# richardbaihe/a3t

Hardware: AMD Instinct MI355X
Metric: mel-frames/sec (train) (higher is better)
Workload: dtype bf16; 1 GPU; VCTK A3T masked-mel train step: 6+6 Conformer blocks d=384 H=2 ff=1536(k3), B=32/GPU, T_mel=1000, T_phn=120, postnet 5x256x5, fwd+bwd+clip+Adam, dropout 0.2/0.2/0.2 + postnet 0.5 (recipe); global_batch=32, parallelism=dp1, params=100799808

## Files before the change

a3t_amd/_lib.py:

```python
import ctypes
import os
from ctypes import POINTER, c_char_p, c_float, c_int, c_int32, c_int64, c_void_p

import torch

HERE = os.path.dirname(os.path.abspath(__file__))
LIB_PATH = os.environ.get("A3T_LIB_PATH") or os.path.join(HERE, "lib", "liba3t_hip.so")

F32, BF16 = 0, 1
BF16X3 = 2
ACT_NONE, ACT_RELU, ACT_TANH, ACT_SWISH = 0, 1, 2, 3
ACC_STORE, ACC_ADD, ACC_ATOMIC, ACC_SOLE = 0, 1, 2, 3


class GemmDesc(ctypes.Structure):
    _fields_ = [
        ("A", c_void_p), ("B", c_void_p), ("C", c_void_p), ("bias", c_void_p), ("R", c_void_p), ("S", c_void_p),
        ("M", c_int32), ("N", c_int32), ("K", c_int32),
        ("a_rs", c_int64), ("a_cs", c_int64),
        ("b_rs", c_int64), ("b_cs", c_int64), ("b_ts", c_int64),
        ("c_rs", c_int64),
        ("batch", c_int32), ("batch_inner", c_int32),
        ("a_bs0", c_int64), ("a_bs1", c_int64), ("b_bs0", c_int64), ("b_bs1", c_int64),
        ("c_bs0", c_int64), ("c_bs1", c_int64),
        ("taps", c_int32), ("pad", c_int32), ("dil", c_int32), ("Tseq", c_int32), ("kshift", c_int32),
        ("alpha", c_float),
        ("act", c_int32), ("accumulate", c_int32), ("splitk", c_int32),
        ("a_dtype", c_int32), ("b_dtype", c_int32), ("c_dtype", c_int32), ("compute", c_int32),
        ("s_dtype", c_int32), ("colsum_slots", c_int32),
        ("colsum", c_void_p), ("colsum_bs1", c_int64), ("colsum_scale", c_float), ("drop_key", ctypes.c_uint32),
        ("drop_p", c_float), ("colsum_ss", c_int32),
        ("keep_out", c_void_p), ("keep_in", c_void_p),
        ("a_signmask", c_int32), ("keep_layout", c_int32),
        ("A2", c_void_p), ("B2", c_void_p), ("b2_cs", c_int64), ("b2_bs0", c_int64), ("b2_bs1", c_int64), ("colsum2", c_void_p),
        ("a2_rs", c_int64), ("a_unaligned", c_int32),
    ]


_P = c_void_p
_SIGS = {
    "a3t_gemm": [POINTER(GemmDesc), _P],
    "a3t_gemm_plan": [POINTER(GemmDesc), c_char_p, c_int],
    "a3t_layernorm_fwd": [_P, _P, _P, _P, c_int, _P, _P, c_int, c_int, c_float, _P],
    "a3t_layernorm_bwd": [_P, c_int, _P, _P, _P, _P, _P, _P, _P, _P, _P, _P, c_float, c_int, c_int, c_float,
                          ctypes.c_uint32, _P],
    "a3t_col_reduce": [_P, c_int, _P, _P, _P, _P, c_int, c_int, c_int64, c_int, _P],
    "a3t_f64_to_f32_add": [_P, _P, c_int, c_float, _P],
    "a3t_bn_act_fwd": [_P, _P, _P, _P, _P, _P, _P, _P, _P, c_int, c_int, c_int, c_float, c_float, c_int, c_int, _P],
    "a3t_bn_act_bwd_a": [_P, c_int, _P, _P, _P, _P, _P, _P, c_int, c_int, c_int, _P],
    "a3t_bn_act_bwd_b": [_P, c_int, _P, _P, _P, _P, _P, _P, _P, _P, _P, c_int, c_int, c_int, c_int, _P],
    "a3t_glu_dwconv_fwd": [_P, c_int, _P, _P, _P, c_int, _P, c_int, c_int, c_int, c_int, _P],
    "a3t_glu_dwconv_bwd": [_P, _P, c_int, _P, c_int, _P, _P, c_int, _P, _P, _P, c_int, c_int, c_int, c_int, _P],
    "a3t_add_pos_bias": [_P, _P, _P, _P, _P, c_int, c_int, c_int, _P],
    "a3t_add_pos_bias_bwd": [_P, _P, _P, c_int, c_int, c_int, _P],
    "a3t_relpos_softmax_fwd": [_P, _P, c_int, _P, _P, c_int, c_int, c_int, c_int, c_int64, c_int64, c_int64, c_float, _P,
                               c_float, ctypes.c_uint32, _P],
    "a3t_relpos_softmax_bwd": [_P, c_int, _P, c_int, _P, _P, c_int, c_int, c_int, c_int, c_int64, c_int64, c_int64, c_float, _P,
                               c_float, c_int64, c_int64, ctypes.c_uint32, _P, _P],
    "a3t_attn_fwd_train": [_P, _P, _P, _P, _P, _P, _P, _P, _P, _P, _P, c_int, c_int, c_int, c_int, c_int64, c_int64, c_int64,
                           c_int64, c_float, c_float, ctypes.c_uint32, _P, _P, _P],
    "a3t_attn_scale_rows": [_P, _P, _P, c_int, c_int, c_int, c_int, _P],
    "a3t_attn_bwd_ds": [_P, _P, _P, _P, _P, _P, _P, c_int, c_int, c_int, c_int, c_int64, c_int64, c_int64, c_int64, c_float,
                        c_float, ctypes.c_uint32, c_int, c_int64, _P],
    "a3t_attn_fwd": [_P, _P, _P, _P, _P, _P, _P, _P, c_int, c_int, c_int, c_int, c_int64, c_int64, c_int64, c_int64,
                     c_float, c_float, ctypes.c_uint32, _P, _P, _P],
    "a3t_pwg_block": [_P, _P, _P, _P, _P, _P, _P, _P, c_int, c_int, c_int, _P],
    "a3t_mask_fill": [_P, _P, _P, _P, c_int, c_int, c_int, _P],
    "a3t_embed_finish_fwd": [_P, _P, _P, _P, _P, _P, _P, c_int, c_int, c_int, c_int, c_float, c_float, ctypes.c_uint32,
                             _P, _P],
    "a3t_embed_finish_bwd": [_P, _P, _P, _P, _P, _P, _P, _P, c_int, c_int, c_int, c_int, c_int, c_int, c_float, c_float,
                             ctypes.c_uint32, _P],
    "a3t_scale": [_P, _P, c_int64, c_float, _P],
    "a3t_axpy": [_P, _P, c_int64, c_float, _P],
    "a3t_attn_bias_fold": [_P, c_int32, c_int32, _P, _P, _P, _P],
    "a3t_scale_dev": [_P, _P, c_int64, _P, _P],
    "a3t_slice_rows": [_P, _P, c_int, c_int, c_int, c_int, c_int, c_int, _P],
    "a3t_concat_rows": [_P, _P, _P, c_int, c_int, c_int, c_int, _P],
    "a3t_concat_rows_ragged": [_P, _P, _P, _P, _P, c_int, c_int, c_int, c_int, c_int64, c_int64, _P],
    "a3t_split_rows": [_P, _P, _P, c_int, c_int, c_int, c_int, _P],
    "a3t_cast_bf16": [_P, _P, c_int64, _P],
    "a3t_cast_bf16_conv_t": [_P, _P, _P, _P, c_int, c_int, c_int, c_int, _P],
    "a3t_split_bf16": [_P, _P, _P, c_int64, _P],
    "a3t_reflect_pad": [_P, _P, c_int, c_int, c_int, c_int, _P],
    "a3t_reflect_pad_ragged": [_P, _P, _P, c_int, c_int, c_int, c_int, _P],
    "a3t_stft_amp": [_P, _P, c_int64, c_int, c_int, _P],
    "a3t_logmel_finish": [_P, _P, c_int, c_int, c_int, _P],
    "a3t_mlm_loss": [_P, _P, _P, _P, _P, _P, _P, _P, c_int, c_int, c_int, c_float, _P],
    "a3t_mlm_loss_scratch_floats": [c_int],
    "a3t_sumsq": [_P, c_int64, _P, _P],
    "a3t_clip_adam": [_P, _P, _P, _P, _P, _P, c_int64, c_float, c_float, c_float, c_float, c_int, c_float, c_float,
                      _P],
    "a3t_clip_adam_noam": [_P, _P, _P, _P, _P, _P, c_int64, _P, c_float, c_float, c_float, c_float, c_float, c_float,
                           c_float, c_float, _P],
    "a3t_sgd_step": [_P, _P, c_int64, c_float, c_float, _P],
    "a3t_pwg_gate": [_P, _P, _P, c_int64, c_int, _P],
    "a3t_pwg_res_skip": [_P, _P, _P, c_int64, c_int, c_int, _P],
    "a3t_pwg_upsample": [_P, _P, _P, c_int64, c_int64, c_int, c_int, _P],
    "a3t_replicate_pad": [_P, _P, c_int64, c_int64, c_int, c_int, _P],
    "a3t_bias_act": [_P, _P, c_int64, c_int, c_int, c_float, _P],
    "a3t_replicate_pad_ragged": [_P, _P, _P, c_int64, c_int64, c_int, c_int, _P],
    "a3t_pwg_upsample_ragged": [_P, _P, _P, _P, c_int, c_int64, c_int64, c_int, c_int, _P],
    "a3t_zero_tail": [_P, _P, c_int, c_int64, c_int64, c_int, _P],
    "a3t_layernorm_fwd_ragged": [_P, _P, _P, _P, _P, _P, _P, c_int, c_int, c_int, c_float, _P],
    "a3t_glu_dwconv_fwd_ragged": [_P, _P, _P, _P, _P, _P, c_int, c_int, c_int, c_int, _P],
    "a3t_relpos_softmax_fwd_ragged": [_P, _P, c_int, _P, _P, c_int, c_int, c_int, c_int, c_int64, c_int64, c_int64, c_float,
                                      _P],
    "a3t_splice_spans": [_P, _P, _P, _P, _P, _P, c_int, c_int, c_int, c_int, _P],
    "a3t_splice_spans_multi": [_P, _P, _P, _P, _P, _P, _P, c_int, c_int, c_int, c_int, c_int, _P],
    "a3t_gather_windows": [_P, _P, _P, c_int, c_int, c_int, c_int, _P],
    "a3t_pwg_block_ragged": [_P, _P, _P, _P, _P, _P, _P, _P, _P, c_int, c_int, c_int, c_int, _P],
    "a3t_pwg_block_f16": [_P, _P, _P, _P, _P, _P, _P, _P, _P, c_int, c_int, c_int, c_int, _P],
    "a3t_cast_f16_sat": [_P, _P, c_int64, _P],
    "a3t_hfg_conv": [_P, _P, _P, _P, _P, _P, c_float, c_int, c_float, _P, c_int, c_int, c_int, c_int, c_int, c_int, _P],
    "a3t_hfg_conv_f16": [_P, _P, _P, _P, _P, _P, c_float, c_int, c_float, _P, c_int, c_int, c_int, c_int, c_int, c_int, _P],
    "a3t_hfg_out": [_P, _P, _P, _P, c_float, _P, c_int, c_int, c_int, c_int, c_int, _P],
    "a3t_leaky_relu": [_P, _P, c_int64, c_float, _P],
    "a3t_mgan_stack": [_P, _P, _P, _P, c_float, _P, c_int, c_int, c_int, c_int, c_int, c_int, _P],
    "a3t_mgan_out": [_P, _P, _P, _P, c_float, c_int, _P, c_int, c_int, c_int, c_int, c_int, c_int, c_int, _P],
    "a3t_pqmf_synthesis": [_P, _P, _P, _P, c_int, c_int, c_int, c_int, c_int, _P],
    "a3t_reflect_pad_rows": [_P, _P, c_int64, c_int64, c_int, c_int, _P],
    "a3t_reflect_pad_rows_ragged": [_P, _P, _P, c_int, c_int64, c_int64, c_int, c_int, _P],
    "a3t_smg_conv": [_P, _P, _P, _P, _P, _P, _P, c_int, c_int, _P, c_int, c_int, c_int, c_int, c_int, c_int, c_int, c_int, c_int,
                     c_int, _P],
    "a3t_smg_stats": [_P, _P, _P, c_float, _P, c_int, c_int, c_int, c_int, _P],
    "a3t_duration_head": [_P, _P, _P, _P, _P, _P, _P, c_int, c_int, c_float, c_float, _P],
    "a3t_l2_normalize": [_P, _P, c_int, c_int, c_float, _P],
    "a3t_gst_conv_bn_relu": [_P, _P, _P, _P, _P, _P, c_int, c_int, c_int, c_int, c_int, c_int, c_int, _P],
    "a3t_gst_gru_stl": [_P, _P, _P, _P, _P, _P, _P, _P, _P, _P, _P, _P, c_int, c_int, c_int, c_int, c_int, c_int, _P],
    "a3t_gst_add_style": [_P, _P, _P, c_int, c_int, c_int, c_int, _P],
    "a3t_fs2_variance_embed": [_P, _P, _P, _P, _P, _P, _P, _P, c_int, c_int, c_int, c_int, c_int, _P],
    "a3t_length_offsets": [_P, _P, c_float, _P, _P, _P, c_int, c_int, _P],
    "a3t_length_expand": [_P, _P, _P, _P, _P, c_int, c_int, c_int, c_int, c_float, _P],
    "a3t_fs2_finish": [_P, _P, _P, _P, _P, _P, _P, c_int, c_int, c_int, _P],
    "a3t_fs2_mvn": [_P, _P, _P, _P, c_int64, c_int, _P],
    "a3t_dropout": [_P, c_int, _P, c_int, c_int64, c_float, ctypes.c_uint32, c_float, _P],
    "a3t_collate_paint": [_P, _P, _P, _P, _P, _P, _P, _P, _P, _P, _P, _P, _P, c_int, c_int, c_int, c_int, c_int, c_int, _P],
    "a3t_segment_colsum": [_P, _P, c_int, c_int, c_int, _P],
    "a3t_gemm_8p_mode": [c_int],
    "a3t_gemm_8p_supported": [c_int, c_int, c_int, c_int, c_int],
    "a3t_gemm_pn_mode": [c_int],
    "a3t_gemm_tt_mode": [c_int],
    "a3t_gemm_tn3_mode": [c_int],
    "a3t_gemm_tn3_group": [_P, c_int, _P],
    "a3t_attn_split_mode": [c_int],
    "a3t_release_workspaces": [],
    "a3t_gemm_pn_supported": [c_int, c_int, c_int, c_int, c_int],
    "a3t_gemm_tt_supported": [c_int, c_int, c_int, c_int],
    "a3t_dropout_bwd_cast": [_P, _P, c_int, _P, c_float, c_int, c_int, c_float, ctypes.c_uint32, _P],
}
EXPORTS = sorted(list(_SIGS) + ["a3t_version", "a3t_gemm_last_kernel", "a3t_gemm_keep_bytes"])

_lib = None


class A3TLibraryError(RuntimeError):
    pass


def load():
    global _lib
    if _lib is not None:
        return _lib
    if not os.path.exists(LIB_PATH):
        raise A3TLibraryError(
            f"{LIB_PATH} is missing: build it with `python -m a3t_amd.build` (hipcc --offload-arch=gfx950). "
            "a3t_amd has no CPU fallback.")
    lib = ctypes.CDLL(LIB_PATH)
    for name, args in _SIGS.items():
        fn = getattr(lib, name)
        fn.argtypes = args
        fn.restype = c_int
    lib.a3t_version.restype = c_char_p
    lib.a3t_version.argtypes = []
    lib.a3t_gemm_last_kernel.restype = c_char_p
    lib.a3t_gemm_last_kernel.argtypes = []
    lib.a3t_gemm_keep_bytes.restype = c_int64
    lib.a3t_gemm_keep_bytes.argtypes = [c_int, c_int]
    _lib = lib
    return lib


def check(rc, what=""):
    if rc != 0:
        raise A3TLibraryError(f"liba3t_hip call failed ({what}): rc={rc}")
```

a3t_amd/conformer.py:

```python
import math
import os
import zlib
from dataclasses import dataclass

import torch

from . import ops
from ._lib import ACC_ADD, ACC_ATOMIC, ACC_STORE, ACT_RELU, ACT_SWISH, BF16, BF16X3, F32
from .config import A3TConfig
from .params import ParamStore
from .schedule import StepSchedule


def legacy_pe_table(c: A3TConfig) -> torch.Tensor:
    d = c.adim
    position = torch.arange(c.max_len - 1, -1, -1.0, dtype=torch.float32).unsqueeze(1)
    div = torch.exp(torch.arange(0, d, 2, dtype=torch.float32) * -(math.log(10000.0) / d))
    pe = torch.zeros(c.max_len, d)
    pe[:, 0::2] = torch.sin(position * div)
    pe[:, 1::2] = torch.cos(position * div)
    return pe


def score_chunks(lengths, heads, max_score_elems):
    order = sorted(range(len(lengths)), key=lambda i: (lengths[i], i))
    out, cur = [], []
    for i in order:
        if cur and (len(cur) + 1) * heads * lengths[i] ** 2 > max_score_elems:
            out.append(cur)
            cur = []
        cur.append(i)
    if cur:
        out.append(cur)
    return out


@dataclass
class EngineOptions:
    side_stream: bool = True
    side2: bool = True
    side_depth: int = 48
    wgrad_group: bool = True
    post_f32_first: bool = True
    attn_bwd_ds: bool = True
    attn_signed: bool = True
    attn_dq_dual: bool = True
    attn_dbd_view: bool = True
    attn_dk_main: bool = True
    fused_attn: str = "auto"
    fused_attn_train: int = 1
    ffn_8p: bool = True
    ffn_keep4: bool = True
    lin_dgrad_t: bool = True
    fuse_ln_dropout: bool = True

    @classmethod
    def from_env(cls, environ=os.environ):
        fa, ft = environ.get("A3T_FUSED_ATTN", "auto"), environ.get("A3T_FUSED_ATTN_TRAIN", "1")
        if fa not in ("auto", "fwd", "0"):
            raise ValueError(f"A3T_FUSED_ATTN={fa!r}: expected auto, fwd or 0 (the flash backward behind '1' left the library in "
                             "round 5, tools/experiments/attn_flash_backward.patch)")
        on = {f: environ.get("A3T_" + f.upper(), "1") != "0" for f in
              ("side_stream", "side2", "wgrad_group", "post_f32_first", "attn_bwd_ds", "attn_signed", "attn_dq_dual",
               "attn_dbd_view", "attn_dk_main", "ffn_8p", "ffn_keep4", "lin_dgrad_t")}
        return cls(side_depth=max(2, int(environ.get("A3T_SIDE_DEPTH", "48"))), fused_attn=fa,
                   fused_attn_train=0 if ft == "0" else 2 if ft == "2" else 1, **on)


COMPUTE_MODES = {"f32": F32, "bf16": BF16, "bf16x3": BF16X3}


class ConformerStack(StepSchedule):
    def __init__(self, cfg: A3TConfig, store: ParamStore, compute: str = "f32", training: bool = True,
                 dropout: bool = False, options: EngineOptions = None):
        self.opt = opt = options if options is not None else EngineOptions.from_env()
        super().__init__(store.device, opt.side_stream, opt.side2, opt.side_depth)
        self.c = cfg
        self.dropping = bool(dropout and training)
        self.step_seed = 0
        self.store = store
        if compute not in COMPUTE_MODES:
            raise ValueError(f"compute={compute!r}: expected one of {', '.join(map(repr, COMPUTE_MODES))}")
        self.compute = compute
        self.bf16 = (compute == "bf16")
        self.adt = torch.bfloat16 if self.bf16 else torch.float32
        self.cmp = COMPUTE_MODES[compute]
        self.training = training
        self.pe = legacy_pe_table(cfg).to(self.dev)
        self.sv = {}
        self.scratch64 = torch.zeros(4 * max(cfg.ff, 3 * cfg.adim, cfg.postnet_chans, 64), dtype=torch.float64,
                                     device=self.dev)
        self.bn_momentum = 0.1
        self._wg_group = 4 if (self.bf16 and self.side is not None and self._depth >= 8 and opt.wgrad_group) else 1
        self._wg_pending, self._wg_slots = [], set()
        self._gm_ready = None
        self.colsum_slots = 16
        self.fused_attn_fwd_only = self.bf16 and opt.fused_attn == "fwd"
        self.fused_attn_auto = self.bf16 and opt.fused_attn == "auto"
        self.fused_attn_train = self.bf16 and opt.fused_attn == "auto" and opt.fused_attn_train != 0
        self.fused_attn_train_min = 1 if opt.fused_attn_train == 2 else 64
        self._fused_now = self._fused_train_now = False
        self.attn_path, self.block_dims = {}, {}
        self._need_grad = training
        self._mode_tag = None
        if self.bf16:
            for n, v in (("adim", cfg.adim), ("ff", cfg.ff), ("idim", cfg.idim), ("odim", cfg.odim),
                         ("dk", cfg.dk), ("postnet_chans", cfg.postnet_chans or 8)):
                if v % 8:
                    raise ValueError(f"compute='bf16' needs {n} % 8 == 0 (16-byte DMA granules), got {v}")
            self.flat16 = torch.zeros(store.total, dtype=torch.bfloat16, device=self.dev)
            self.p16 = {k: self.flat16[o:o + math.prod(s)].view(s) for k, (o, s) in store.offsets.items()}
        self._ffn_plans = {}
        self._lin_plans = {}
        self._wt = {}
        self._P_ahead, self._pos_ev = {}, None
        self._cast_ev = self._wt_ev = None
        dec = [o for k, (o, _) in store.offsets.items() if k.startswith("dec.")]
        self._cast_split = min(dec) if dec else 0

    def _drop(self, p, tag):
        if not self.dropping or p <= 0.0:
            return None
        h = (zlib.crc32(tag.encode()) ^ ((self.step_seed * 0x9E3779B1) & 0xFFFFFFFF)) & 0xFFFFFFFF
        h = ((h ^ (h >> 16)) * 0x85EBCA6B) & 0xFFFFFFFF
        h = ((h ^ (h >> 13)) * 0xC2B2AE35) & 0xFFFFFFFF
        return (float(p), (h ^ (h >> 16)) & 0xFFFFFFFF)

    def _gm(self, g, tag, p, bias_grad, bias_scale):
        dr = self._drop(p, tag)
        if dr is None:
            return (self._g16(g) if self.bf16 else g)
        gm = self.ws.get(self._t("tmp.gm"), tuple(g.shape), self.adt)
        if self._gm_ready == tag:
            self._gm_ready = None
            return gm
        ops.dropout_bwd_cast(g, gm, dr[0], dr[1], colsum=bias_grad, colsum_scale=bias_scale)
        return gm

    def W(self, name):
        return self.p16[name] if self.bf16 else self.store.p[name]

    def refresh_weights(self):
        self._cast_ev = self._wt_ev = None
        if not self.bf16:
            return
        split = self._cast_split if self.side is not None else 0
        flat, flat16 = self.store.flat, self.flat16
        wt = list(self._wt.values()) if self._need_grad else []

        def transposed():
            for src_off, dst_off, _, tflat, shp in wt:
                ops.cast_bf16_conv_t(flat, tflat, src_off, dst_off, *shp)
        if split <= 0:
            ops.cast_bf16(flat, flat16)
            transposed()
            return
        ops.cast_bf16(flat[:split], flat16[:split])
        self._cast_ev = self._side(lambda: ops.cast_bf16(flat[split:], flat16[split:]), want_event="cast")
        if wt:
            self._wt_ev = self._side(transposed, want_event="wt")

    def _wait_cast(self, which):
        ev = getattr(self, which, None)
        if ev is not None:
            ev.wait_on(torch.cuda.current_stream())
            setattr(self, which, None)

    def _setup_wt(self, suf, shape):
        stored = (tuple(shape), (shape[0], shape[2])) if shape[1] == 1 else (tuple(shape),)
        names = [k for k in self.store.offsets if k.endswith("." + suf) and tuple(self.store.offsets[k][1]) in stored]
        if not names:
            return
        n = math.prod(shape)
        flat = torch.zeros(n * len(names), dtype=torch.bfloat16, device=self.dev)
        src = torch.tensor([self.store.offsets[k][0] for k in names], dtype=torch.int64, device=self.dev)
        dst = torch.arange(len(names), dtype=torch.int64, device=self.dev) * n
        views = {k: flat[i * n:(i + 1) * n].view(shape[2], shape[1], shape[0]) for i, k in enumerate(names)}
        self._wt[suf] = (src, dst, views, flat, tuple(shape))
        ops.cast_bf16_conv_t(self.store.flat, flat, src, dst, *shape)

    def _ffn_plan(self, M):
        key = (M, self._need_grad, self._mode_tag, self.opt.ffn_8p, self.opt.ffn_keep4)
        if key not in self._ffn_plans:
            c = self.c
            keep = d1 = d2 = keep4 = False
            if self._need_grad and self.bf16 and self.dev.type == "cuda" and self.opt.ffn_8p:
                k = c.ff_kernel
                drop = ops.G8_DROP if (self.dropping and c.dropout_rate > 0) else 0
                keep = ops.gemm_8p_supported(M, c.ff, k * c.adim, k, ops.G8_BIAS_ACT | drop | ops.G8_KEEP_OUT) and \
                    ops.gemm_8p_supported(M, c.ff, k * c.adim, k, ops.G8_KEEP_IN | ops.G8_COLSUM)
                d1 = ops.gemm_8p_supported(M, c.adim, k * c.ff, k, 0) or ops.gemm_pn_supported(M, c.adim, k * c.ff, k, 0)
                d2 = (not keep) and \
                    ops.gemm_pn_supported(M, c.ff, k * c.adim, k, ops.G8_SMASK | ops.G8_COLSUM)
                keep4 = (not keep) and self.opt.ffn_keep4 and c.ff % 8 == 0 and \
                    ops.gemm_pn_supported(M, c.ff, k * c.adim, k, ops.G8_KEEP_IN | ops.G8_COLSUM)
                d2 = d2 or keep4
                if (keep or d2) and "w2" not in self._wt:
                    self._setup_wt("w2", (c.adim, k, c.ff))
                if d1 and "w1" not in self._wt:
                    self._setup_wt("w1", (c.ff, k, c.adim))
                keep, d1, d2 = keep and "w2" in self._wt, d1 and "w1" in self._wt, d2 and "w2" in self._wt
                keep4 = keep4 and d2
            self._ffn_plans[key] = (keep, d1, d2, keep4)
        return self._ffn_plans[key]

    def _lin_dgrad(self, dy, name, dx):
        suf = name.rsplit(".", 1)[1]
        M = dy.shape[0]
        key = (suf, M, dx.dtype, self._mode_tag, self.opt.lin_dgrad_t)
        if key not in self._lin_plans:
            use = False
            if self.bf16 and self.dev.type == "cuda" and self.opt.lin_dgrad_t:
                n_out, n_in = self.store.offsets[name][1]
                use = ops.gemm_pn_supported(M, n_in, n_out, 1, ops.G8_F32_OR_RES if dx.dtype == torch.float32 else 0)
                if use and suf not in self._wt:
                    self._setup_wt(suf, (n_out, 1, n_in))
                use = use and suf in self._wt and name in self._wt[suf][2]
            self._lin_plans[key] = use
        if self._lin_plans[key]:
            wt = self._wt[suf][2][name]
            ops.linear_fwd(dy, wt.view(wt.shape[0], wt.shape[2]), dx, compute=self.cmp)
        else:
            ops.linear_bwd_data(dy, self.W(name), dx, compute=self.cmp)

    def _act(self, name, shape):
        return self.ws.get(name, shape, self.adt)

    def _ln_fwd(self, tag, x, pre, eps=1e-12, out_dtype=None, lens=None, T=0):
        p = self.store.p
        M, D = x.shape
        y = self.ws.get(tag + ".y", (M, D), out_dtype or self.adt)
        mean = self.ws.get(tag + ".mean", (M,))
        rstd = self.ws.get(tag + ".rstd", (M,))
        if lens is not None:
            ops.layernorm_fwd_ragged(x, p[pre + ".g"], p[pre + ".b"], y, mean, rstd, lens, M // T, T, eps)
        else:
            ops.layernorm_fwd(x, p[pre + ".g"], p[pre + ".b"], y, mean, rstd, eps)
        self.sv[tag] = (x, y, mean, rstd)
        return y

    def _ln_bwd(self, tag, dy, pre, dres, dx, dx16=None, nb=None, nxt=None):
        p, g = self.store.p, self.store.g
        x, _, mean, rstd = self.sv[tag]
        dropping = self.dropping and self.c.dropout_rate > 0
        if dropping and self.bf16 and self.opt.fuse_ln_dropout and nb is not None and nxt is not None and x.shape[1] % 128 == 0:
            dr = self._drop(self.c.dropout_rate, nxt)
            nx = (self._par + 1) % self._depth
            gm = self.ws.get(f"tmp.gm.{nx}", tuple(dx.shape), self.adt)
            ev = self._side_ev[nx]
            if ev is not None:
                ev.wait_on(torch.cuda.current_stream())
                self._side_ev[nx] = None
            ops.layernorm_bwd(dy, x, p[pre + ".g"], mean, rstd, dres, dx, g[pre + ".g"], g[pre + ".b"], dx16=gm,
                              dxsum=nb[0], dxsum_scale=nb[1], drop=dr)
            self._gm_ready = nxt
            return
        if dropping and nxt is not None:
            nb = None
        fuse = self.bf16 and nb is not None
        ops.layernorm_bwd(dy, x, p[pre + ".g"], mean, rstd, dres, dx, g[pre + ".g"], g[pre + ".b"], dx16=dx16,
                          dxsum=nb[0] if fuse else None, dxsum_scale=nb[1] if fuse else 1.0)
        if nb is not None and not fuse:
            self._bias_grad(dx, nb[0], nb[1])

    def _bias_grad(self, dy, gb, scale=1.0):
        ops.bias_grad(dy, gb, self.scratch64, scale)

    def _g16(self, g):
        return self.ws.get("grad.x16", tuple(g.shape), torch.bfloat16) if self.bf16 else None

    def _lin_wgrad(self, dy, x, dW):
        if self._wg_group > 1:
            self._wg_pending.append((dy, x, dW, 1.0))
            self._wg_slots.add(self._par)
            if len(self._wg_pending) >= self._wg_group:
                self._wg_flush()
            return
        self._side(lambda: ops.linear_bwd_weight(dy, x, dW, compute=self.cmp))

    def _wg_flush(self):
        items, self._wg_pending = self._wg_pending, []
        slots, self._wg_slots = self._wg_slots, set()
        if items:
            cmp = self.cmp
            self._side(lambda: ops.linear_bwd_weight_group(items, compute=cmp))
            if self.side is not None:
                for sl in slots:
                    ev = self._owned_event(("slot", sl))
                    ev.record(self.side)
                    self._side_ev[sl] = ev

    def _pre_ln(self, ga, g, g16):
        if ga is g or ga is g16:
            self._wg_flush()
        if self.side is not None and (ga is g or ga is g16):
            torch.cuda.current_stream().wait_stream(self.side)

    def _ffn_fwd(self, tag, pre, x, T, lens=None):
        p, c = self.store.p, self.c
        M = x.shape[0]
        pad = (c.ff_kernel - 1) // 2
        if lens is not None and pad == 0:
            lens = None
        y = self._ln_fwd(tag + ".ln", x, pre + ".ln", lens=lens, T=T)
        h = self._act(tag + ".h", (M, c.ff))
        keep, lay = None, 0
        if self._ffn_plan(M)[0]:
            keep = self.ws.get(tag + ".keep", (ops.gemm_keep_bytes(M, c.ff),), torch.uint8)
        elif self._ffn_plan(M)[3]:
            keep, lay = self.ws.get(tag + ".keep4", (M * c.ff // 4,), torch.uint8), 1
        ops.conv_fwd(y, self.W(pre + ".w1"), h, T, pad, bias=p[pre + ".b1"], act=ACT_RELU, compute=self.cmp,
                     drop=self._drop(c.dropout_rate, tag + ".h"), keep_out=keep, keep_layout=lay)
        if lens is not None:
            ops.zero_tail(h, lens, 1, M // T, T)
        xo = self.ws.get(tag + ".xo", (M, c.adim))
        ops.conv_fwd(h, self.W(pre + ".w2"), xo, T, pad, bias=p[pre + ".b2"], R=x, alpha=0.5, compute=self.cmp,
                     drop=self._drop(c.dropout_rate, tag + ".o"))
        self.sv[tag] = (y, h, keep, lay)
        return xo

    def _ffn_bwd(self, tag, pre, g, T, nb=None, nxt=None):
        p, gr, c = self.store.p, self.store.g, self.c
        y, h, keep, lay = self.sv[tag]
        M = g.shape[0]
        pad = (c.ff_kernel - 1) // 2
        self._sub_begin()
        g16 = self._g16(g)
        ga = self._gm(g, tag + ".o", c.dropout_rate, gr[pre + ".b2"], 0.5)
        self._side(lambda: ops.conv_bwd_weight(ga, h, gr[pre + ".w2"], T, pad, alpha=0.5, compute=self.cmp))
        dh = self._act(self._t("tmp.dh"), (M, c.ff))
        hd = self._drop(c.dropout_rate, tag + ".h")
        a_dh = 0.5 / (1.0 - hd[0]) if hd else 0.5
        if keep is not None:
            ops.conv_fwd(ga, self._wt["w2"][2][pre + ".w2"], dh, T, c.ff_kernel - 1 - pad, alpha=a_dh, compute=self.cmp,
                         keep_in=keep, keep_layout=lay, colsum=gr[pre + ".b1"])
        elif self._ffn_plan(M)[2]:
            ops.conv_fwd(ga, self._wt["w2"][2][pre + ".w2"], dh, T, c.ff_kernel - 1 - pad, alpha=a_dh, compute=self.cmp,
                         S=h, colsum=gr[pre + ".b1"])
        else:
            ops.conv_bwd_data(ga, self.W(pre + ".w2"), dh, T, pad, S=h, alpha=a_dh,
                              compute=self.cmp, colsum=gr[pre + ".b1"] if self.bf16 else None)
        self._side(lambda: ops.conv_bwd_weight(dh, y, gr[pre + ".w1"], T, pad, compute=self.cmp))
        dy = self._act("tmp.dy", (M, c.adim))
        if self._ffn_plan(M)[1]:
            ops.conv_fwd(dh, self._wt["w1"][2][pre + ".w1"], dy, T, c.ff_kernel - 1 - pad, compute=self.cmp)
        else:
            ops.conv_bwd_data(dh, self.W(pre + ".w1"), dy, T, pad, compute=self.cmp)
        if not self.bf16:
            self._bias_grad(dh, gr[pre + ".b1"])
        self._pre_ln(ga, g, g16)
        self._ln_bwd(tag + ".ln", dy, pre + ".ln", g, g, g16, nb, nxt)
        self._sub_end()
        return g

    def _mha_fwd(self, tag, pre, x, pos, keymask, B, T, lens=None, pos_rows=None):
        p, c = self.store.p, self.c
        d, dk = c.adim, c.dk
        M = B * T
        cmp = self.cmp
        y = self._ln_fwd(tag + ".ln", x, pre + ".ln")
        qkv = self._act(tag + ".qkv", (M, 3 * d))
        ops.linear_fwd(y, self.W(pre + ".wqkv"), qkv, bias=p[pre + ".bqkv"], compute=cmp)
        ragged = lens is not None
        fused = (self._fused_now or self._fused_train_now) and ops.attn_fused_supported(dk, T) and not ragged
        pbias = (p[pre + ".u"], p[pre + ".v"])
        qu = qv = None
        if not fused:
            qu = self._act(tag + ".qu", (M, d))
            qv = self._act(tag + ".qv", (M, d))
            ops.add_pos_bias(qkv, pbias[0], pbias[1], qu, qv)
        P = None if ragged else self._P_ahead.get(tag)
        if P is not None:
            ev = self._pos_ev.get(tag[:3]) if self._pos_ev else None
            if ev is not None:
                ev.wait_on(torch.cuda.current_stream())
                self._pos_ev[tag[:3]] = None
        elif pos_rows is not None:
            Pt = self._act(tag + ".Pt", (pos.shape[0], d))
            ops.linear_fwd(pos, self.W(pre + ".wpos"), Pt, compute=cmp)
            P = self._act(tag + ".Prow", (M, d))
            ops.concat_rows_ragged(Pt, Pt, P, pos_rows[0], pos_rows[1], B, pos_rows[2], pos_rows[3], d, 0, 0)
        else:
            P = self._act(tag + ".P", (T, d))
            ops.linear_fwd(pos, self.W(pre + ".wpos"), P, compute=cmp)
        route = "fwd" if (self._fused_now and fused) else "train" if (self._fused_train_now and fused) else "mat"
        self.attn_path[tag[:-4]] = route
        self.block_dims[tag[:-4]] = (B, T)
        for k in (".fused", ".rs", ".signed"):
            self.sv.pop(tag + k, None)
        ctx = self._act(tag + ".ctx", (M, d))
        q = (qu, qv, qkv, P, keymask, ctx)
        if route == "mat":
            kept = self._attn_fwd_mat(tag, q, B, T, lens, pos_rows is not None)
        else:
            kept = (self._attn_fwd_only if route == "fwd" else self._attn_fwd_train)(tag, q, pbias, B, T)
        xo = self.ws.get(tag + ".xo", (M, d))
        ops.linear_fwd(ctx, self.W(pre + ".wo"), xo, bias=p[pre + ".bo"], R=x, compute=cmp,
                       drop=self._drop(c.dropout_rate, tag + ".o"))
        self.sv[tag] = None if kept is None else (y, qkv, qu, qv, P, kept[0], ctx, pos, kept[1])
        return xo

    def _attn_fwd_only(self, tag, q, pbias, B, T):
        c = self.c
        lse = self.ws.get(tag + ".lse", (B, c.heads, T))
        ops.attn_fwd(*q, lse, B, c.heads, T, 1.0 / math.sqrt(c.dk), drop=self._drop(c.attention_dropout_rate, tag + ".att") or (0.0, 0),
                     pos_bias=pbias if q[0] is None else None)
        self.sv[tag + ".fused"] = True

    def _attn_fwd_train(self, tag, q, pbias, B, T):
        c, H = self.c, self.c.heads
        adr = self._drop(c.attention_dropout_rate, tag + ".att")
        probs = self._act(tag + ".probs", (B, H, T, T))
        signed = bool(adr) and self.bf16 and self.opt.attn_bwd_ds and self.opt.attn_signed and T <= 2048
        pdrop = self._act(tag + ".pdrop", (B, H, T, T)) if adr and not signed else None
        lse = self.ws.get(tag + ".lse", (B, H, T))
        rs = self.ws.get(tag + ".rs", (B, H, T))
        ops.attn_fwd_train(*q, lse, probs, pdrop, rs, B, H, T, 1.0 / math.sqrt(c.dk), drop=adr or (0.0, 0),
                           pos_bias=pbias if q[0] is None else None)
        self.sv[tag + ".signed"] = signed
        self.sv[tag + ".rs"] = rs
        return probs, pdrop

    def _attn_fwd_mat(self, tag, q, B, T, lens, pos_per_row):
        c, H, d, dk, cmp = self.c, self.c.heads, self.c.adim, self.c.dk, self.cmp
        qu, qv, qkv, P, keymask, ctx = q
        sdt = torch.bfloat16 if self.bf16 else torch.float32
        ac = self.ws.get("tmp.ac", (B, H, T, T), sdt)
        bd = self.ws.get("tmp.bd", (B, H, T, T), sdt)
        kk = qkv.view(-1)[d:]
        vv = qkv.view(-1)[2 * d:]
        ops.gemm(qu, kk, ac, T, T, dk, d, 1, 3 * d, 1, T, batch=B * H, batch_inner=H, a_bs=(T * d, dk),
                 b_bs=(T * 3 * d, dk), c_bs=(H * T * T, T * T), compute=cmp)
        ops.gemm(qv, P, bd, T, T, dk, d, 1, d, 1, T, batch=B * H, batch_inner=H, a_bs=(T * d, dk),
                 b_bs=(T * d if pos_per_row else 0, dk), c_bs=(H * T * T, T * T), compute=cmp)
        probs = self._act(tag + ".probs", (B, H, T, T))
        adr = self._drop(c.attention_dropout_rate, tag + ".att")
        pdrop = self._act(tag + ".pdrop", (B, H, T, T)) if adr else None
        if lens is not None:
            ops.relpos_softmax_fwd_ragged(ac, bd, lens, probs, B, H, T, 1.0 / math.sqrt(dk))
        else:
            ops.relpos_softmax_fwd(ac, bd, keymask, probs, B, H, T, 1.0 / math.sqrt(dk), probs_drop=pdrop,
                                   drop=adr or (0.0, 0))
        ops.gemm(pdrop if adr else probs, vv, ctx, T, dk, T, T, 1, 1, 3 * d, d, batch=B * H, batch_inner=H,
                 a_bs=(H * T * T, T * T), b_bs=(T * 3 * d, dk), c_bs=(T * d, dk), compute=cmp)
        return None if lens is not None else (probs, pdrop)

    def _mha_bwd(self, tag, pre, g, B, T, nb=None, nxt=None):
        p, gr, c = self.store.p, self.store.g, self.c
        d, H, dk = c.adim, c.heads, c.dk
        M = B * T
        cmp = self.cmp
        y, qkv, qu, qv, P, probs, ctx, pos, pdrop = self.sv[tag]
        scale = 1.0 / math.sqrt(dk)
        self._sub_begin()
        g16 = self._g16(g)
        ga = self._gm(g, tag + ".o", c.dropout_rate, gr[pre + ".bo"], 1.0)
        self._lin_wgrad(ga, ctx, gr[pre + ".wo"])
        dctx = self._act("tmp.dctx", (M, d))
        self._lin_dgrad(ga, pre + ".wo", dctx)
        kk = qkv.view(-1)[d:]
        vv = qkv.view(-1)[2 * d:]
        dqkv = self._act(self._t("tmp.dqkv"), (M, 3 * d))
        dkk = dqkv.view(-1)[d:]
        dvv = dqkv.view(-1)[2 * d:]
        sdt = torch.bfloat16 if self.bf16 else torch.float32
        rs = self.sv.get(tag + ".rs")
        dctx_v = dctx
        if rs is not None:
            dctx_v = self._act(self._t("tmp.dctxs"), (M, d))
        signed = bool(self.sv.get(tag + ".signed"))
        adr = self._drop(c.attention_dropout_rate, tag + ".att") if (pdrop is not None or signed) else None
        regen = self.bf16 and adr is not None and T % 8 == 0 and T <= 2048
        ds_fused = (rs is not None and self.bf16 and self.opt.attn_bwd_ds and (adr is None or regen) and dk % 32 == 0 and dk <= 192
                    and dk != 160 and T % 8 == 0)
        zb = (H * T * T, T * T)
        assert ds_fused or not signed
        if not ds_fused:
            dpr = self.ws.get("tmp.ac", (B, H, T, T), sdt)
            ops.gemm(dctx, vv, dpr, T, T, dk, d, 1, 3 * d, 1, T, batch=B * H, batch_inner=H, a_bs=(T * d, dk),
                     b_bs=(T * 3 * d, dk), c_bs=zb, compute=cmp)
        fz = self.bf16
        gbq = gr[pre + ".bqkv"]
        S = self.colsum_slots
        sl = self._arena_slot("bwd32", tag + ".bsl", S * 4 * d) if fz else None
        csk = dict(colsum_bs1=dk, colsum_slots=S, colsum_ss=4 * d)
        make_q = qu is None
        if make_q:
            qu = self._act("tmp.qu", (M, d))
            qv = self._act(self._t("tmp.qv"), (M, d))

        def dv_gemm():
            if rs is not None:
                ops.attn_scale_rows(dctx, rs, dctx_v, B, H, T)
            ops.gemm(pdrop if pdrop is not None else probs, dctx_v, dvv, T, dk, T, 1, T, 1, d, 3 * d,
                     batch=B * H, batch_inner=H, a_bs=zb, b_bs=(T * d, dk), c_bs=(T * 3 * d, dk),
                     compute=cmp, colsum=sl[3 * d:] if fz else None, a_signmask=signed,
                     alpha=1.0 / (1.0 - adr[0]) if signed else 1.0, **csk)
            if make_q:
                ops.add_pos_bias(qkv, p[pre + ".u"], p[pre + ".v"], qu, qv)
        qv_ready = self._side(dv_gemm, want_event=make_q, urgent=True)
        zbd = zb
        dual = ds_fused and fz and self.opt.attn_dq_dual and ops.gemm_tt_supported(T, dk, T, B * H)
        dview = ds_fused and fz and self.opt.attn_dbd_view
        if dview:
            bsv = T + T * T
            flat = self.ws.get(self._t("tmp.dsv"), (B * H * bsv,), torch.bfloat16, zero_once=True)
            ds, dbd = flat[T:], flat[1:]
            zbd = (H * bsv, bsv)
        elif self.bf16:
            ds = self.ws.get("tmp.ds16", (B, H, T, T), torch.bfloat16)
            dbd = self.ws.get(self._t("tmp.dbd16"), (B, H, T, T), torch.bfloat16)
        else:
            ds = dpr
            dbd = self.ws.get(self._t("tmp.dbd"), (B, H, T, T), sdt)
        if ds_fused:
            ops.attn_bwd_ds(dctx, ctx, qkv, probs, rs, ds, None if dview else dbd, B, H, T, scale, drop=adr or (0.0, 0),
                            signed_probs=signed, ds_bs=zbd[1] if dview else 0)
        else:
            ops.relpos_softmax_bwd(probs, dpr, ds, dbd, B, H, T, scale, probs_drop=None if regen else pdrop,
                                   drop_p=adr[0] if adr else 0.0, drop_key=adr[1] if regen else 0, rowscale=rs)
        def pos_weight_grad():
            if qv_ready is not None and self.side is not None:
                qv_ready.wait_on(self.side)
            dP = self._arena_slot("bwd32", tag + ".dP", T * d).view(T, d)
            ops.gemm(dbd, qv, dP, T, dk, T, 1, T + 1 if dview else T, 1, d, d, batch=B * H, batch_inner=H, a_bs=zbd, b_bs=(T * d, dk),
                     c_bs=(0, dk), acc=ACC_ATOMIC, compute=cmp, a_view=dview)
            if self.bf16:
                dP16 = self.ws.get("tmp.dP16", (T, d), torch.bfloat16)
                ops.cast_bf16(dP, dP16)
                dP = dP16
            ops.linear_bwd_weight(dP, pos, gr[pre + ".wpos"], compute=cmp)
        self._side(pos_weight_grad)
        dq_acc = fz
        dqu = dqkv if dq_acc else self._act("tmp.dqu", (M, d))
        dqv = dqkv if dq_acc else self._act("tmp.dqv", (M, d))
        ldq, cbq = (3 * d, (T * 3 * d, dk)) if dq_acc else (d, (T * d, dk))
        if dual:
            ops.gemm(ds, kk, dqkv, T, dk, T, T, 1, 1, 3 * d, ldq, batch=B * H, batch_inner=H, a_bs=zbd,
                     b_bs=(T * 3 * d, dk), c_bs=cbq, compute=cmp, colsum=sl,
                     second=(dbd, P, d, (0, dk), sl[d:]) + ((T + 1,) if dview else ()), **csk)
        else:
            ops.gemm(ds, kk, dqu, T, dk, T, T, 1, 1, 3 * d, ldq, batch=B * H, batch_inner=H, a_bs=zbd,
                     b_bs=(T * 3 * d, dk), c_bs=cbq, compute=cmp, colsum=sl if fz else None, **csk)
        dk_fn = lambda: ops.gemm(ds, qu, dkk, T, dk, T, 1, T, 1, d, 3 * d, batch=B * H, batch_inner=H,
                                 a_bs=zbd, b_bs=(T * d, dk), c_bs=(T * 3 * d, dk), compute=cmp,
                                 colsum=sl[2 * d:] if fz else None, **csk)
        if self.opt.attn_dk_main and dual and self.side is not None and make_q and qv_ready is not None:
            qv_ready.wait_on(torch.cuda.current_stream())
            dk_fn()
            dk_done = None
        else:
            dk_done = self._side(dk_fn, want_event=True, urgent=True)
        if not dual:
            ops.gemm(dbd, P, dqv, T, dk, T, T + 1 if dview else T, 1, 1, d, ldq, batch=B * H, batch_inner=H, a_bs=zbd, b_bs=(0, dk),
                     c_bs=cbq, acc=ACC_ADD if dq_acc else ACC_STORE, compute=cmp, colsum=sl[d:] if fz else None, a_view=dview, **csk)
        if not dq_acc:
            ops.add_pos_bias_bwd(dqu, dqv, dqkv)
        if dk_done is not None:
            dk_done.wait_on(torch.cuda.current_stream())
        if fz:
            self._side(
                lambda: ops.attn_bias_fold(sl, S, d, gr[pre + ".u"], gr[pre + ".v"], gbq))
        else:
            self._bias_grad(dqu, gr[pre + ".u"])
            self._bias_grad(dqv, gr[pre + ".v"])
            self._bias_grad(dqkv, gbq)
        self._lin_wgrad(dqkv, y, gr[pre + ".wqkv"])
        dy = self._act("tmp.dy", (M, d))
        self._lin_dgrad(dqkv, pre + ".wqkv", dy)
        self._pre_ln(ga, g, g16)
        self._ln_bwd(tag + ".ln", dy, pre + ".ln", g, g, g16, nb, nxt)
        self._sub_end()
        return g

    def _bn_fwd(self, tag, z, pre, bufpre, act, out):
        p, b = self.store.p, self.store.buf
        M, C = z.shape
        stats = self._arena_slot("fwd64", tag + ".stats", 2 * C)
        if self.training:
            ops.col_reduce(z, stats[:C], stats[C:], mode=1)
        mean = self.ws.get(tag + ".bnmean", (C,))
        rstd = self.ws.get(tag + ".bnrstd", (C,))
        ops.bn_act_fwd(z, stats, p[pre + ".g"], p[pre + ".b"], b[bufpre + ".rm"], b[bufpre + ".rv"], mean, rstd, out,
                       1e-5, self.bn_momentum if self.training else 0.0, self.training, act)
        if self.training:
            self.store.nbt[bufpre] = self.store.nbt.get(bufpre, 0) + 1
        self.sv[tag + ".bn"] = (z, mean, rstd)

    def _bn_bwd(self, tag, dy, pre, act, dz):
        p, gr = self.store.p, self.store.g
        z, mean, rstd = self.sv[tag + ".bn"]
        M, C = z.shape
        sums = self._arena_slot("bwd64", tag + ".bnsums", 2 * C)
        ops.bn_act_bwd(dy, z, mean, rstd, p[pre + ".g"], p[pre + ".b"], sums, dz, gr[pre + ".g"], gr[pre + ".b"],
                       self.training, act, zero=False)

    def _conv_fwd(self, tag, pre, x, T, lens=None):
        p, c = self.store.p, self.c
        M, d = x.shape
        cmp = self.cmp
        y = self._ln_fwd(tag + ".ln", x, pre + ".ln")
        g2 = self._act(tag + ".g", (M, 2 * d))
        ops.linear_fwd(y, self.W(pre + ".pw1"), g2, bias=p[pre + ".pb1"], compute=cmp)
        glu = self._act(tag + ".glu", (M, d))
        z = self.ws.get(tag + ".z", (M, d))
        if lens is not None:
            ops.glu_dwconv_fwd_ragged(g2, p[pre + ".dw"], p[pre + ".db"], glu, z, lens, M // T, T)
        else:
            ops.glu_dwconv_fwd(g2, p[pre + ".dw"], p[pre + ".db"], glu, z, T)
        s = self._act(tag + ".s", (M, d))
        self._bn_fwd(tag, z, pre + ".bn", pre + ".bn", ACT_SWISH, s)
        xo = self.ws.get(tag + ".xo", (M, d))
        ops.linear_fwd(s, self.W(pre + ".pw2"), xo, bias=p[pre + ".pb2"], R=x, compute=cmp,
                       drop=self._drop(c.dropout_rate, tag + ".o"))
        self.sv[tag] = (y, g2, glu, s)
        return xo

    def _conv_bwd(self, tag, pre, g, T, nb=None, nxt=None):
        p, gr, c = self.store.p, self.store.g, self.c
        M, d = g.shape
        cmp = self.cmp
        y, g2, glu, s = self.sv[tag]
        self._sub_begin()
        g16 = self._g16(g)
        ga = self._gm(g, tag + ".o", c.dropout_rate, gr[pre + ".pb2"], 1.0)
        self._lin_wgrad(ga, s, gr[pre + ".pw2"])
        ds = self.ws.get("tmp.ds", (M, d))
        self._lin_dgrad(ga, pre + ".pw2", ds)
        dz = self.ws.get("tmp.dz", (M, d))
        self._bn_bwd(tag, ds, pre + ".bn", ACT_SWISH, dz)
        dg = self._act(self._t("tmp.dg"), (M, 2 * d))
        ops.glu_dwconv_bwd(dz, g2, glu, p[pre + ".dw"], dg, gr[pre + ".dw"], gr[pre + ".db"], T,
                           dgsum=gr[pre + ".pb1"])
        self._lin_wgrad(dg, y, gr[pre + ".pw1"])
        dy = self._act("tmp.dy", (M, d))
        self._lin_dgrad(dg, pre + ".pw1", dy)
        self._pre_ln(ga, g, g16)
        self._ln_bwd(tag + ".ln", dy, pre + ".ln", g, g, g16, nb, nxt)
        self._sub_end()
        return g

    def _check_ragged(self, lens, B):
        if self.bf16 or self.training or self._need_grad:
            raise ValueError("lens: ragged rows need an engine in fp32 compute, eval mode, forward only "
                             f"(compute={self.compute}: 'f32' and 'bf16x3' both count, training={self.training}, "
                             f"need_grad={self._need_grad})")
        if lens.dtype != torch.int32 or lens.numel() != B or lens.device.type != self.dev.type:
            raise ValueError(f"lens must be an int32 tensor of {B} entries on {self.dev}")

    def block_fwd(self, pre, x, pos, keymask, B, T, lens=None, pos_rows=None):
        if lens is not None:
            self._check_ragged(lens, B)
        x = self._ffn_fwd(pre + ".ffm", pre + ".ffm", x, T, lens)
        x = self._mha_fwd(pre + ".mha", pre + ".mha", x, pos, keymask, B, T, lens, pos_rows)
        x = self._conv_fwd(pre + ".cnv", pre + ".cnv", x, T, lens)
        x = self._ffn_fwd(pre + ".ff", pre + ".ff", x, T, lens)
        return self._ln_fwd(pre + ".fin", x, pre + ".fin.ln", out_dtype=torch.float32)

    def block_bwd(self, pre, g, B, T):
        gr = self.store.g
        self._ln_bwd(pre + ".fin", g, pre + ".fin.ln", None, g, self._g16(g), (gr[pre + ".ff.b2"], 0.5), pre + ".ff.o")
        self._ffn_bwd(pre + ".ff", pre + ".ff", g, T, (gr[pre + ".cnv.pb2"], 1.0), pre + ".cnv.o")
        self._conv_bwd(pre + ".cnv", pre + ".cnv", g, T, (gr[pre + ".mha.bo"], 1.0), pre + ".mha.o")
        self._mha_bwd(pre + ".mha", pre + ".mha", g, B, T, (gr[pre + ".ffm.b2"], 0.5), pre + ".ffm.o")
        self._ffn_bwd(pre + ".ffm", pre + ".ffm", g, T, None)
        return g

    def _attn_choice(self, B, T, need_grad):
        nblk = B * self.c.heads * ((T + 127) // 128)
        fused_now = (self.fused_attn_fwd_only and not need_grad) or \
            (self.fused_attn_auto and not need_grad and nblk >= 64)
        fused_train_now = self.fused_attn_train and need_grad and not fused_now and \
            self.fused_attn_train_min <= nblk <= 65536 and T <= 2048
        return fused_now, fused_train_now
```

a3t_amd/csrc/convmod_attn.hip:

```cpp
#include <hip/hip_runtime.h>
#include <stdint.h>
#include "../../include/a3t_hip.h"
#include "dtype_io.h"

#define WAVE 64
__device__ __forceinline__ float sigm(float v) { return 1.f / (1.f + __expf(-v)); }
__device__ __forceinline__ float bf2f_(unsigned int h) { return __uint_as_float(h << 16); }
__device__ __forceinline__ float wsum(float v) {
#pragma unroll
    for (int o = 32; o > 0; o >>= 1) v += __shfl_xor(v, o, WAVE);
    return v;
}
__device__ __forceinline__ float wmax(float v) {
#pragma unroll
    for (int o = 32; o > 0; o >>= 1) v = fmaxf(v, __shfl_xor(v, o, WAVE));
    return v;
}

#define DW_TT 64
#define DW_KMAX 31

template <int KT, bool RAGGED>
__global__ __launch_bounds__(256) void glu_dwconv_fwd_kernel(const void* __restrict__ g, int g_dt,
                                                             const float* __restrict__ wdw,
                                                             const float* __restrict__ bdw, void* __restrict__ glu,
                                                             int glu_dt, float* __restrict__ z, int C, int K, int Tseq,
                                                             int tiles_t, const int32_t* __restrict__ lens) {
    __shared__ float win[DW_TT + DW_KMAX - 1][64];
    const int tx = threadIdx.x & 63, ty = threadIdx.x >> 6;
    const int c = blockIdx.x * 64 + tx;
    const int b = blockIdx.y / tiles_t, t0 = (blockIdx.y % tiles_t) * DW_TT;
    const int pad = (K - 1) / 2;
    const int64_t mbase = (int64_t)b * Tseq;
    int n = Tseq;
    if constexpr (RAGGED) {
        g_dt = glu_dt = A3T_F32;
        n = ragged_len(lens, b, Tseq);
        if (t0 >= n) {
            if (c < C)
                for (int r = ty; r < DW_TT && t0 + r < Tseq; r += 4) {
                    ((float*)glu)[(mbase + t0 + r) * (int64_t)C + c] = 0.f;
                    z[(mbase + t0 + r) * (int64_t)C + c] = 0.f;
                }
            return;
        }
    }
    const int rows = DW_TT + K - 1;
    for (int rb = ty; rb < rows; rb += 32) {
        float ga[8], gb[8];
#pragma unroll
        for (int u = 0; u < 8; ++u) {
            const int r = rb + 4 * u, t = t0 - pad + r;
            const bool ok = (c < C) && (r < rows) && (t >= 0) && (t < n);
            const int64_t gi = ok ? (mbase + t) * (int64_t)(2 * C) + c : 0;
            ga[u] = ldx(g, g_dt, gi);
            gb[u] = ldx(g, g_dt, gi + (ok ? C : 0));
        }
#pragma unroll
        for (int u = 0; u < 8; ++u) {
            const int r = rb + 4 * u, t = t0 - pad + r;
            const bool ok = (c < C) && (r < rows) && (t >= 0) && (t < n);
            const float v = ok ? ga[u] * sigm(gb[u]) : 0.f;
            const bool st = RAGGED ? (c < C) && (t < Tseq) : ok;
            if (st && r >= pad && r < pad + DW_TT) stx(glu, glu_dt, (mbase + t) * (int64_t)C + c, v);
            if (r < rows) win[r][tx] = v;
        }
    }
    __syncthreads();
    if (c >= C) return;
    float w[KT];
#pragma unroll
    for (int k = 0; k < KT; ++k) w[k] = (k < K) ? wdw[(int64_t)c * K + k] : 0.f;
    const float bias = bdw[c];
    if (K == KT) {
        for (int r0 = ty * 4; r0 < DW_TT; r0 += 16) {
            float v[KT + 3];
#pragma unroll
            for (int j = 0; j < KT + 3; ++j) v[j] = win[r0 + j][tx];
#pragma unroll
            for (int tt = 0; tt < 4; ++tt) {
                float acc = bias;
#pragma unroll
                for (int k = 0; k < KT; ++k) acc += w[k] * v[tt + k];
                int t = t0 + r0 + tt;
                if (t < Tseq) z[(mbase + t) * (int64_t)C + c] = (!RAGGED || t < n) ? acc : 0.f;
            }
        }
        return;
    }
    for (int r = ty; r < DW_TT; r += 4) {
        int t = t0 + r;
        if (t >= Tseq) break;
        float acc = bias;
#pragma unroll
        for (int k = 0; k < KT; ++k)
            if (k < K) acc += w[k] * win[r + k][tx];
        z[(mbase + t) * (int64_t)C + c] = (!RAGGED || t < n) ? acc : 0.f;
    }
}

int a3t_glu_dwconv_fwd_vec(const void* g, const float* wdw, const float* bdw, void* glu, float* z, int M, int C, int K,
                           int Tseq, hipStream_t stream);
int a3t_glu_dwconv_bwd_vec(const float* dz, const void* g, const void* glu, const float* wdw, void* dg, float* dwdw,
                           float* dbdw, float* dg_colsum, int M, int C, int K, int Tseq, hipStream_t stream);
static inline bool dw_al16(const void* p) { return ((uintptr_t)p & 15) == 0; }

template <bool RAGGED>
static int glu_dwconv_fwd_launch(const void* g, int g_dtype, const float* wdw, const float* bdw, void* glu, int glu_dtype,
                                 float* z, int B, int C, int K, int Tseq, const int32_t* lens, hipStream_t stream) {
    const int tiles_t = (Tseq + DW_TT - 1) / DW_TT;
    dim3 grid((C + 63) / 64, B * tiles_t);
#define CALL(KT)                                                                                                         \
    hipLaunchKernelGGL((glu_dwconv_fwd_kernel<KT, RAGGED>), grid, dim3(256), 0, stream, g, g_dtype, wdw, bdw, glu, glu_dtype, \
                       z, C, K, Tseq, tiles_t, lens)
    if (K <= 7) CALL(7);
    else if (K <= 15) CALL(15);
    else CALL(DW_KMAX);
#undef CALL
    return (int)hipGetLastError();
}

extern "C" int a3t_glu_dwconv_fwd(const void* g, int g_dtype, const float* wdw, const float* bdw, void* glu,
                                  int glu_dtype, float* z, int M, int C, int K, int Tseq, void* stream) {
    if (K > DW_KMAX || K <= 0 || (K & 1) == 0 || Tseq <= 0 || M <= 0 || C <= 0 || M % Tseq) return A3T_EINVAL;
    if ((int64_t)(M / Tseq) * ((Tseq + DW_TT - 1) / DW_TT) > 65535) return A3T_EINVAL;
    if (g_dtype == A3T_BF16 && glu_dtype == A3T_BF16 && C % 64 == 0 && dw_al16(g) && dw_al16(glu) && dw_al16(z))
        return a3t_glu_dwconv_fwd_vec(g, wdw, bdw, glu, z, M, C, K, Tseq, (hipStream_t)stream);
    return glu_dwconv_fwd_launch<false>(g, g_dtype, wdw, bdw, glu, glu_dtype, z, M / Tseq, C, K, Tseq, nullptr,
                                        (hipStream_t)stream);
}

extern "C" int a3t_glu_dwconv_fwd_ragged(const float* g, const float* wdw, const float* bdw, float* glu, float* z,
                                         const int32_t* lens, int B, int Tseq, int C, int K, void* stream) {
    if (K > DW_KMAX || K <= 0 || (K & 1) == 0 || Tseq <= 0 || B <= 0 || C <= 0 || !lens) return A3T_EINVAL;
    if ((int64_t)B * ((Tseq + DW_TT - 1) / DW_TT) > 65535) return A3T_EINVAL;
    return glu_dwconv_fwd_launch<true>(g, A3T_F32, wdw, bdw, glu, A3T_F32, z, B, C, K, Tseq, lens, (hipStream_t)stream);
}

template <int KT>
__global__ __launch_bounds__(256, 3) void glu_dwconv_bwd_kernel(const float* __restrict__ dz, const void* __restrict__ g,
                                                             int g_dt, const void* __restrict__ glu, int glu_dt,
                                                             const float* __restrict__ wdw, void* __restrict__ dg,
                                                             int dg_dt, float* dwdw, float* dbdw, float* dgsum, int C,
                                                             int K, int Tseq, int tiles_t, int tiles_per_block,
                                                             int chunks) {
    __shared__ float wdz[DW_TT + DW_KMAX - 1][64];
    __shared__ float wgl[DW_TT + DW_KMAX - 1][64];
    __shared__ float red[4][64];
    const int tx = threadIdx.x & 63, ty = threadIdx.x >> 6;
    const int c = blockIdx.x * 64 + tx;
    const int b = blockIdx.y / chunks, tile0 = (blockIdx.y % chunks) * tiles_per_block;
    const int pad = (K - 1) / 2;
    const int64_t mbase = (int64_t)b * Tseq;
    const int rows = DW_TT + K - 1;
    float w[KT], dw[KT];
#pragma unroll
    for (int k = 0; k < KT; ++k) {
        w[k] = (k < K && c < C) ? wdw[(int64_t)c * K + k] : 0.f;
        dw[k] = 0.f;
    }
    float db = 0.f, sga = 0.f, sgb = 0.f;
    for (int tile = tile0; tile < min(tiles_t, tile0 + tiles_per_block); ++tile) {
        const int t0 = tile * DW_TT;
        float gan[4], gbn[4];
        auto prefetch_g = [&](int i) {
#pragma unroll
            for (int tt = 0; tt < 4; ++tt) {
                const int t = t0 + ty * 4 + 16 * i + tt;
                gan[tt] = gbn[tt] = 0.f;
                if (c < C && t < Tseq) {
                    const int64_t gi = (mbase + t) * (int64_t)(2 * C);
                    gan[tt] = ldx(g, g_dt, gi + c);
                    gbn[tt] = ldx(g, g_dt, gi + C + c);
                }
            }
        };
        if (K == KT) prefetch_g(0);
        __syncthreads();
        for (int rb = ty; rb < rows; rb += 32) {
            float a[8], q[8];
#pragma unroll
            for (int u = 0; u < 8; ++u) {
                const int r = rb + 4 * u, t = t0 - pad + r;
                const bool ok = (c < C) && (r < rows) && (t >= 0) && (t < Tseq);
                const int64_t idx = ok ? (mbase + t) * (int64_t)C + c : 0;
                a[u] = dz[idx];
                q[u] = ldx(glu, glu_dt, idx);
                a[u] = ok ? a[u] : 0.f;
                q[u] = ok ? q[u] : 0.f;
            }
#pragma unroll
            for (int u = 0; u < 8; ++u) {
                const int r = rb + 4 * u;
                if (r < rows) wdz[r][tx] = a[u], wgl[r][tx] = q[u];
            }
        }
        __syncthreads();
        if (c < C && K == KT) {
#pragma unroll 1
            for (int i = 0; i < 4; ++i) {
                const int r0 = ty * 4 + 16 * i;
                float ga[4], gb[4];
#pragma unroll
                for (int tt = 0; tt < 4; ++tt) ga[tt] = gan[tt], gb[tt] = gbn[tt];
                if (i < 3) prefetch_g(i + 1);
                float acc[4], dzt[4];
                {
                    float u[KT + 3];
#pragma unroll
                    for (int j = 0; j < KT + 3; ++j) u[j] = wdz[r0 + j][tx];
#pragma unroll
                    for (int tt = 0; tt < 4; ++tt) {
                        float a = 0.f;
#pragma unroll
                        for (int k = 0; k < KT; ++k) a += w[k] * u[tt + KT - 1 - k];
                        acc[tt] = a;
                        dzt[tt] = u[tt + (KT - 1) / 2];
                    }
                }
                __builtin_amdgcn_sched_barrier(0);
                {
                    float q[KT + 3];
#pragma unroll
                    for (int j = 0; j < KT + 3; ++j) q[j] = wgl[r0 + j][tx];
#pragma unroll
                    for (int tt = 0; tt < 4; ++tt) {
#pragma unroll
                        for (int k = 0; k < KT; ++k) dw[k] += dzt[tt] * q[tt + k];
                        db += dzt[tt];
                    }
                }
#pragma unroll
                for (int tt = 0; tt < 4; ++tt) {
                    const int t = t0 + r0 + tt;
                    if (t < Tseq) {
                        const int64_t gi = (mbase + t) * (int64_t)(2 * C);
                        const float sb = sigm(gb[tt]);
                        const float da = acc[tt] * sb, dbb = acc[tt] * ga[tt] * sb * (1.f - sb);
                        stx(dg, dg_dt, gi + c, da);
                        stx(dg, dg_dt, gi + C + c, dbb);
                        sga += da, sgb += dbb;
                    }
                }
            }
        } else if (c < C) {
            for (int r = ty; r < DW_TT; r += 4) {
                int t = t0 + r;
                if (t >= Tseq) break;
                float acc = 0.f;
#pragma unroll
                for (int k = 0; k < KT; ++k)
                    if (k < K) acc += w[k] * wdz[r + 2 * pad - k][tx];
                const int64_t gi = (mbase + t) * (int64_t)(2 * C);
                float ga = ldx(g, g_dt, gi + c), sb = sigm(ldx(g, g_dt, gi + C + c));
                const float da = acc * sb, dbb = acc * ga * sb * (1.f - sb);
                stx(dg, dg_dt, gi + c, da);
                stx(dg, dg_dt, gi + C + c, dbb);
                sga += da, sgb += dbb;
                float dzt = wdz[r + pad][tx];
                db += dzt;
#pragma unroll
                for (int k = 0; k < KT; ++k)
                    if (k < K) dw[k] += dzt * wgl[r + k][tx];
            }
        }
    }
#pragma unroll
    for (int k = 0; k < KT; ++k) {
        if (k >= K) break;
        __syncthreads();
        red[ty][tx] = dw[k];
        __syncthreads();
        if (ty == 0 && c < C) atomicAdd(&dwdw[(int64_t)c * K + k], red[0][tx] + red[1][tx] + red[2][tx] + red[3][tx]);
    }
    __syncthreads();
    red[ty][tx] = db;
    __syncthreads();
    if (ty == 0 && c < C) atomicAdd(&dbdw[c], red[0][tx] + red[1][tx] + red[2][tx] + red[3][tx]);
    if (dgsum) {
        __syncthreads();
        red[ty][tx] = sga;
        __syncthreads();
        if (ty == 0 && c < C) atomicAdd(&dgsum[c], red[0][tx] + red[1][tx] + red[2][tx] + red[3][tx]);
        __syncthreads();
        red[ty][tx] = sgb;
        __syncthreads();
        if (ty == 0 && c < C) atomicAdd(&dgsum[C + c], red[0][tx] + red[1][tx] + red[2][tx] + red[3][tx]);
    }
}

extern "C" int a3t_glu_dwconv_bwd(const float* dz, const void* g, int g_dtype, const void* glu, int glu_dtype,
                                  const float* wdw, void* dg, int dg_dtype, float* dwdw, float* dbdw, float* dg_colsum,
                                  int M, int C, int K, int Tseq, void* stream) {
    if (K > DW_KMAX || K <= 0 || (K & 1) == 0 || Tseq <= 0 || M <= 0 || C <= 0 || M % Tseq) return A3T_EINVAL;
    if (g_dtype == A3T_BF16 && glu_dtype == A3T_BF16 && dg_dtype == A3T_BF16 && C % 64 == 0 && dw_al16(g) &&
        dw_al16(glu) && dw_al16(dg) && dw_al16(dz))
        return a3t_glu_dwconv_bwd_vec(dz, g, glu, wdw, dg, dwdw, dbdw, dg_colsum, M, C, K, Tseq, (hipStream_t)stream);
    int B = M / Tseq, tiles_t = (Tseq + DW_TT - 1) / DW_TT;
    int cb = (C + 63) / 64;
    int chunks = 1;
    while (cb * B * chunks < 1024 && chunks < tiles_t) ++chunks;
    int tpb = (tiles_t + chunks - 1) / chunks;
    chunks = (tiles_t + tpb - 1) / tpb;
    if ((int64_t)B * chunks > 65535) return A3T_EINVAL;
    dim3 grid(cb, B * chunks);
#define DWB(KT)                                                                                                       \
    hipLaunchKernelGGL(glu_dwconv_bwd_kernel<KT>, grid, dim3(256), 0, (hipStream_t)stream, dz, g, g_dtype, glu, glu_dtype, \
                       wdw, dg, dg_dtype, dwdw, dbdw, dg_colsum, C, K, Tseq, tiles_t, tpb, chunks)
    if (K <= 7)
        DWB(7);
    else if (K <= 15)
        DWB(15);
    else
        DWB(DW_KMAX);
#undef DWB
    return (int)hipGetLastError();
}

__global__ void add_pos_bias_kernel(const void* __restrict__ qkv, const float* __restrict__ bu,
                                    const float* __restrict__ bv, void* __restrict__ qu, void* __restrict__ qv,
                                    int dt, int64_t n, int d) {
    for (int64_t i = (int64_t)blockIdx.x * blockDim.x + threadIdx.x; i < n; i += (int64_t)gridDim.x * blockDim.x) {
        int64_t m = i / d;
        int c = (int)(i - m * d);
        float q = ldx(qkv, dt, m * 3 * d + c);
        stx(qu, dt, i, q + bu[c]);
        stx(qv, dt, i, q + bv[c]);
    }
}
__device__ __forceinline__ void apb_unpack8(const uint4& u, float* f) {
    f[0] = bf2f_(u.x & 0xffff), f[1] = bf2f_(u.x >> 16), f[2] = bf2f_(u.y & 0xffff), f[3] = bf2f_(u.y >> 16);
    f[4] = bf2f_(u.z & 0xffff), f[5] = bf2f_(u.z >> 16), f[6] = bf2f_(u.w & 0xffff), f[7] = bf2f_(u.w >> 16);
}
__device__ __forceinline__ uint4 apb_pack8(const float* f) {
    uint4 u;
    u.x = io_pack2(f[0], f[1]), u.y = io_pack2(f[2], f[3]);
    u.z = io_pack2(f[4], f[5]), u.w = io_pack2(f[6], f[7]);
    return u;
}
__global__ void add_pos_bias_bf16_kernel(const unsigned short* __restrict__ qkv, const float* __restrict__ bu,
                                         const float* __restrict__ bv, unsigned short* __restrict__ qu,
                                         unsigned short* __restrict__ qv, int64_t n8, int d8) {
    for (int64_t i = (int64_t)blockIdx.x * blockDim.x + threadIdx.x; i < n8; i += (int64_t)gridDim.x * blockDim.x) {
        const int64_t m = i / d8;
        const int c = (int)(i - m * d8) * 8;
        float q[8], o[8];
        apb_unpack8(*(const uint4*)(qkv + m * 3 * d8 * 8 + c), q);
        const float4 u0 = *(const float4*)(bu + c), u1 = *(const float4*)(bu + c + 4);
        const float4 v0 = *(const float4*)(bv + c), v1 = *(const float4*)(bv + c + 4);
        const float uu[8] = {u0.x, u0.y, u0.z, u0.w, u1.x, u1.y, u1.z, u1.w};
        const float vv[8] = {v0.x, v0.y, v0.z, v0.w, v1.x, v1.y, v1.z, v1.w};
#pragma unroll
        for (int e = 0; e < 8; ++e) o[e] = q[e] + uu[e];
        *(uint4*)(qu + i * 8) = apb_pack8(o);
#pragma unroll
        for (int e = 0; e < 8; ++e) o[e] = q[e] + vv[e];
        *(uint4*)(qv + i * 8) = apb_pack8(o);
    }
}
static inline bool apb_al16(const void* p) { return ((uintptr_t)p & 15) == 0; }
extern "C" int a3t_add_pos_bias(const void* qkv, const float* bias_u, const float* bias_v, void* qu, void* qv,
                                int dtype, int M, int d, void* stream) {
    int64_t n = (int64_t)M * d;
    if (dtype == A3T_BF16 && d % 8 == 0 && apb_al16(qkv) && apb_al16(qu) && apb_al16(qv) && apb_al16(bias_u) &&
        apb_al16(bias_v)) {
        int64_t n8 = n / 8;
        int blocks = (int)((n8 + 255) / 256);
        if (blocks > 4096) blocks = 4096;
        hipLaunchKernelGGL(add_pos_bias_bf16_kernel, dim3(blocks), dim3(256), 0, (hipStream_t)stream,
                           (const unsigned short*)qkv, bias_u, bias_v, (unsigned short*)qu, (unsigned short*)qv, n8, d / 8);
        return (int)hipGetLastError();
    }
    int blocks = (int)((n + 255) / 256);
    if (blocks > 4096) blocks = 4096;
    hipLaunchKernelGGL(add_pos_bias_kernel, dim3(blocks), dim3(256), 0, (hipStream_t)stream, qkv, bias_u, bias_v, qu,
                       qv, dtype, n, d);
    return (int)hipGetLastError();
}
__global__ void add_pos_bias_bwd_kernel(const void* __restrict__ dqu, const void* __restrict__ dqv,
                                        void* __restrict__ dqkv, int dt, int64_t n, int d) {
    for (int64_t i = (int64_t)blockIdx.x * blockDim.x + threadIdx.x; i < n; i += (int64_t)gridDim.x * blockDim.x) {
        int64_t m = i / d;
        int c = (int)(i - m * d);
        stx(dqkv, dt, m * 3 * d + c, ldx(dqu, dt, i) + ldx(dqv, dt, i));
    }
}
__global__ void add_pos_bias_bwd_bf16_kernel(const unsigned short* __restrict__ dqu, const unsigned short* __restrict__ dqv,
                                             unsigned short* __restrict__ dqkv, int64_t n8, int d8) {
    for (int64_t i = (int64_t)blockIdx.x * blockDim.x + threadIdx.x; i < n8; i += (int64_t)gridDim.x * blockDim.x) {
        const int64_t m = i / d8;
        const int c = (int)(i - m * d8) * 8;
        float a[8], b[8], o[8];
        apb_unpack8(*(const uint4*)(dqu + i * 8), a);
        apb_unpack8(*(const uint4*)(dqv + i * 8), b);
#pragma unroll
        for (int e = 0; e < 8; ++e) o[e] = a[e] + b[e];
        *(uint4*)(dqkv + m * 3 * d8 * 8 + c) = apb_pack8(o);
    }
}
extern "C" int a3t_add_pos_bias_bwd(const void* dqu, const void* dqv, void* dqkv, int dtype, int M, int d,
                                    void* stream) {
    int64_t n = (int64_t)M * d;
    if (dtype == A3T_BF16 && d % 8 == 0 && apb_al16(dqu) && apb_al16(dqv) && apb_al16(dqkv)) {
        int64_t n8 = n / 8;
        int blocks = (int)((n8 + 255) / 256);
        if (blocks > 4096) blocks = 4096;
        hipLaunchKernelGGL(add_pos_bias_bwd_bf16_kernel, dim3(blocks), dim3(256), 0, (hipStream_t)stream,
                           (const unsigned short*)dqu, (const unsigned short*)dqv, (unsigned short*)dqkv, n8, d / 8);
        return (int)hipGetLastError();
    }
    int blocks = (int)((n + 255) / 256);
    if (blocks > 4096) blocks = 4096;
    hipLaunchKernelGGL(add_pos_bias_bwd_kernel, dim3(blocks), dim3(256), 0, (hipStream_t)stream, dqu, dqv, dqkv, dtype,
                       n, d);
    return (int)hipGetLastError();
}

__device__ __forceinline__ float bd_shift(const void* __restrict__ BDz, int dt, int T, int n, int i, int j) {
    if (j <= i) return ldx(BDz, dt, (int64_t)i * T + (n - 1 - i + j));
    if (j == i + 1) return 0.f;
    return ldx(BDz, dt, (int64_t)(i + 1) * T + (j - i - 2));
}

template <int NV, bool RAGGED>
__global__ __launch_bounds__(256) void relpos_softmax_fwd_kernel(const void* __restrict__ ac,
                                                                 const void* __restrict__ bd, int s_dt,
                                                                 const uint8_t* __restrict__ keymask,
                                                                 void* __restrict__ probs, int p_dt, int H, int T,
                                                                 int64_t ac_bs, int64_t bd_bs, int64_t p_bs,
                                                                 float scale, int64_t nrows, void* __restrict__ pdrop,
                                                                 unsigned int thr, float inv, unsigned int key,
                                                                 const int32_t* __restrict__ lens) {
    const int lane = threadIdx.x & 63;
    const int64_t row = (int64_t)blockIdx.x * 4 + (threadIdx.x >> 6);
    if (row >= nrows) return;
    const int64_t zz = row / T;
    const int i = (int)(row - zz * T);
    const int b = (int)(zz / H);
    int n = T;
    if constexpr (RAGGED) {
        s_dt = p_dt = A3T_F32;
        pdrop = nullptr;
        n = ragged_len(lens, b, T);
        if (i >= n) {
            for (int j = lane; j < T; j += 64) ((float*)probs)[zz * p_bs + (int64_t)i * T + j] = 0.f;
            return;
        }
    }
    const int64_t ao = zz * ac_bs + (int64_t)i * T;
    const void* bz = (s_dt == A3T_BF16) ? (const void*)((const unsigned short*)bd + zz * bd_bs)
                                        : (const void*)((const float*)bd + zz * bd_bs);
    const uint8_t* mk = keymask + (int64_t)b * T;
    auto valid = [&](const int j) -> bool {
        if constexpr (RAGGED) return j < n;
        else return mk[j];
    };
    const int64_t po = zz * p_bs + (int64_t)i * T;
    const float NEG = -3.4028235e38f;
    if (NV > 0) {
        float v[NV > 0 ? NV : 1];
        float mx = NEG;
#pragma unroll
        for (int q = 0; q < NV; ++q) {
            int j = lane + q * 64;
            v[q] = NEG;
            if (j < T && valid(j)) v[q] = (ldx(ac, s_dt, ao + j) + bd_shift(bz, s_dt, T, n, i, j)) * scale;
            mx = fmaxf(mx, v[q]);
        }
        mx = wmax(mx);
        float s = 0.f;
#pragma unroll
        for (int q = 0; q < NV; ++q) {
            v[q] = (v[q] > NEG) ? expf(v[q] - mx) : 0.f;
            s += v[q];
        }
        s = wsum(s);
        const float inv_s = s > 0.f ? 1.f / s : 0.f;
#pragma unroll
        for (int q = 0; q < NV; ++q) {
            int j = lane + q * 64;
            if (j < T) {
                const float pj = v[q] * inv_s;
                stx(probs, p_dt, po + j, pj);
                if (pdrop) stx(pdrop, p_dt, po + j, rng_keep(key, (unsigned int)(po + j), thr) ? pj * inv : 0.f);
            }
        }
        return;
    }
    float mx = NEG;
    int any = 0;
    for (int j = lane; j < T; j += 64)
        if (valid(j)) {
            mx = fmaxf(mx, (ldx(ac, s_dt, ao + j) + bd_shift(bz, s_dt, T, n, i, j)) * scale);
            any = 1;
        }
    mx = wmax(mx);
    any = __any(any);
    if (!any) {
        for (int j = lane; j < T; j += 64) {
            stx(probs, p_dt, po + j, 0.f);
            if (pdrop) stx(pdrop, p_dt, po + j, 0.f);
        }
        return;
    }
    float s = 0.f;
    for (int j = lane; j < T; j += 64)
        if (valid(j)) s += expf((ldx(ac, s_dt, ao + j) + bd_shift(bz, s_dt, T, n, i, j)) * scale - mx);
    s = wsum(s);
    const float inv_s = 1.f / s;
    for (int j = lane; j < T; j += 64) {
        const float pj = valid(j) ? expf((ldx(ac, s_dt, ao + j) + bd_shift(bz, s_dt, T, n, i, j)) * scale - mx) * inv_s : 0.f;
        stx(probs, p_dt, po + j, pj);
        if (pdrop) stx(pdrop, p_dt, po + j, rng_keep(key, (unsigned int)(po + j), thr) ? pj * inv : 0.f);
    }
}

__device__ __forceinline__ void unpack8(const uint4& u, float* f) {
    f[0] = bf2f_(u.x & 0xffff), f[1] = bf2f_(u.x >> 16), f[2] = bf2f_(u.y & 0xffff), f[3] = bf2f_(u.y >> 16);
    f[4] = bf2f_(u.z & 0xffff), f[5] = bf2f_(u.z >> 16), f[6] = bf2f_(u.w & 0xffff), f[7] = bf2f_(u.w >> 16);
}
__device__ __forceinline__ uint4 pack8(const float* f) {
    uint4 u;
    u.x = io_pack2(f[0], f[1]), u.y = io_pack2(f[2], f[3]);
    u.z = io_pack2(f[4], f[5]), u.w = io_pack2(f[6], f[7]);
    return u;
}

template <int NC>
__global__ __launch_bounds__(256) void relpos_softmax_fwd_bf16_kernel(
    const unsigned short* __restrict__ ac, const unsigned short* __restrict__ bd, const uint8_t* __restrict__ keymask,
    unsigned short* __restrict__ probs, int H, int T, int64_t ac_bs, int64_t bd_bs, int64_t p_bs, float scale,
    int64_t nrows, unsigned short* __restrict__ pdrop, unsigned int thr, float inv, unsigned int key) {
    const int lane = threadIdx.x & 63;
    const int64_t row = (int64_t)blockIdx.x * 4 + (threadIdx.x >> 6);
    if (row >= nrows) return;
    const int64_t zz = row / T;
    const int i = (int)(row - zz * T);
    const int b = (int)(zz / H);
    const unsigned short* ar = ac + zz * ac_bs + (int64_t)i * T;
    const unsigned short* b0 = bd + zz * bd_bs + (int64_t)i * T + (T - 1 - i);
    const unsigned short* b1 = bd + zz * bd_bs + (int64_t)(i + 1) * T - i - 2;
    const uint8_t* mk = keymask + (int64_t)b * T;
    const int64_t po = zz * p_bs + (int64_t)i * T;
    const float NEG = -3.4028235e38f;
    const int nch = T >> 3;
    float v[NC][8];
    float mx = NEG;
#pragma unroll
    for (int q = 0; q < NC; ++q) {
        const int c = lane + q * 64, j0 = c * 8;
#pragma unroll
        for (int e = 0; e < 8; ++e) v[q][e] = NEG;
        if (c < nch) {
            float a[8];
            unpack8(*(const uint4*)(ar + j0), a);
            const uint2 m2 = *(const uint2*)(mk + j0);
            float bv[8];
            if (j0 + 7 <= i) {
#pragma unroll
                for (int e = 0; e < 8; ++e) bv[e] = bf2f_(b0[j0 + e]);
            } else if (j0 >= i + 2) {
#pragma unroll
                for (int e = 0; e < 8; ++e) bv[e] = bf2f_(b1[j0 + e]);
            } else {
#pragma unroll
                for (int e = 0; e < 8; ++e) {
                    const int j = j0 + e;
                    bv[e] = (j <= i) ? bf2f_(b0[j]) : (j == i + 1 ? 0.f : bf2f_(b1[j]));
                }
            }
#pragma unroll
            for (int e = 0; e < 8; ++e) {
                const unsigned int mb = ((e < 4 ? m2.x : m2.y) >> (8 * (e & 3))) & 0xff;
                if (mb) v[q][e] = (a[e] + bv[e]) * scale;
                mx = fmaxf(mx, v[q][e]);
            }
        }
    }
    mx = wmax(mx);
    float s = 0.f;
#pragma unroll
    for (int q = 0; q < NC; ++q)
#pragma unroll
        for (int e = 0; e < 8; ++e) {
            v[q][e] = (v[q][e] > NEG) ? __expf(v[q][e] - mx) : 0.f;
            s += v[q][e];
        }
    s = wsum(s);
    const float inv_s = s > 0.f ? 1.f / s : 0.f;
#pragma unroll
    for (int q = 0; q < NC; ++q) {
        const int c = lane + q * 64, j0 = c * 8;
        if (c < nch) {
            float o[8];
#pragma unroll
            for (int e = 0; e < 8; ++e) o[e] = v[q][e] * inv_s;
            *(uint4*)(probs + po + j0) = pack8(o);
            if (pdrop) {
#pragma unroll
                for (int e = 0; e < 8; e += 4) {
                    bool kp[4];
                    rng_keep4(key, (unsigned int)(po + j0 + e), thr, kp);
#pragma unroll
                    for (int u = 0; u < 4; ++u) o[e + u] = kp[u] ? o[e + u] * inv : 0.f;
                }
                *(uint4*)(pdrop + po + j0) = pack8(o);
            }
        }
    }
}

#define SM_DISPATCH(T, CALL)               \
    do {                                   \
        if ((T) <= 128) { CALL(2); }       \
        else if ((T) <= 256) { CALL(4); }  \
        else if ((T) <= 512) { CALL(8); }  \
        else if ((T) <= 1152) { CALL(18); } \
        else if ((T) <= 2048) { CALL(32); } \
        else { CALL(0); }                  \
    } while (0)
#define SM_DISPATCH_VEC(T, CALL)            \
    do {                                    \
        if ((T) <= 512) { CALL(1); }        \
        else if ((T) <= 1024) { CALL(2); }  \
        else if ((T) <= 1536) { CALL(3); }  \
        else { CALL(4); }                   \
    } while (0)
static inline bool sm_al16(const void* p) { return ((uintptr_t)p & 15) == 0; }

template <bool RAGGED>
static int relpos_softmax_fwd_launch(const void* ac, const void* bd, int scores_dtype, const uint8_t* keymask, void* probs,
                                     int probs_dtype, int H, int T, int64_t ac_bs, int64_t bd_bs, int64_t p_bs, float scale,
                                     int64_t nrows, void* probs_drop, unsigned int thr, float dinv, uint32_t drop_key,
                                     const int32_t* lens, hipStream_t stream) {
#define CALL(NV)                                                                                                       \
    hipLaunchKernelGGL((relpos_softmax_fwd_kernel<NV, RAGGED>), dim3((unsigned)((nrows + 3) / 4)), dim3(256), 0, stream, ac, \
                       bd, scores_dtype, keymask, probs, probs_dtype, H, T, ac_bs, bd_bs, p_bs, scale, nrows, probs_drop,  \
                       thr, dinv, drop_key, lens)
    SM_DISPATCH(T, CALL);
#undef CALL
    return (int)hipGetLastError();
}

extern "C" int a3t_relpos_softmax_fwd(const void* ac, const void* bd, int scores_dtype, const uint8_t* keymask,
                                      void* probs, int probs_dtype, int B, int H, int T, int64_t ac_bs, int64_t bd_bs,
                                      int64_t p_bs, float scale, void* probs_drop, float drop_p, uint32_t drop_key,
                                      void* stream) {
    int64_t nrows = (int64_t)B * H * T;
    if (drop_p < 0.f || drop_p >= 1.f) return A3T_EINVAL;
    if (drop_p == 0.f) probs_drop = nullptr;
    const unsigned int thr = (unsigned int)((double)drop_p * 4294967296.0);
    const float dinv = 1.f / (1.f - drop_p);
    if (scores_dtype == A3T_BF16 && probs_dtype == A3T_BF16 && T % 8 == 0 && T <= 2048 && ac_bs % 8 == 0 &&
        p_bs % 8 == 0 && sm_al16(ac) && sm_al16(probs) && sm_al16(keymask) && (!probs_drop || sm_al16(probs_drop))) {
#define CALLV(NC)                                                                                                     \
    hipLaunchKernelGGL(relpos_softmax_fwd_bf16_kernel<NC>, dim3((unsigned)((nrows + 3) / 4)), dim3(256), 0,           \
                       (hipStream_t)stream, (const unsigned short*)ac, (const unsigned short*)bd, keymask,            \
                       (unsigned short*)probs, H, T, ac_bs, bd_bs, p_bs, scale, nrows, (unsigned short*)probs_drop, \
                       thr, dinv, drop_key)
        SM_DISPATCH_VEC(T, CALLV);
#undef CALLV
        return (int)hipGetLastError();
    }
    return relpos_softmax_fwd_launch<false>(ac, bd, scores_dtype, keymask, probs, probs_dtype, H, T, ac_bs, bd_bs, p_bs, scale,
                                            nrows, probs_drop, thr, dinv, drop_key, nullptr, (hipStream_t)stream);
}
// ... 189 lines not shown
```

a3t_amd/csrc/gemm.hip:

```cpp
#include <hip/hip_runtime.h>
#include <stdint.h>
#include "../../include/a3t_hip.h"

typedef float f32x16 __attribute__((ext_vector_type(16)));
typedef __bf16 bf16x8 __attribute__((ext_vector_type(8)));

#include "gemm_common.h"

#include <stdio.h>
#include <stdlib.h>
static thread_local char g_last_kernel[128] = "";
void a3t_note_kernel(const char* name) { snprintf(g_last_kernel, sizeof(g_last_kernel), "%s", name); }
extern "C" const char* a3t_gemm_last_kernel(void) { return g_last_kernel; }

template <bool AK, bool BKC, bool VEC>
__global__ __launch_bounds__(256) void gemm_f32_kernel(GP p) {
    constexpr int BM = 128, BN = 128, BK = 16, LD = 132;
    __shared__ __attribute__((aligned(16))) float smem[4 * BK * LD];
    float(*As)[BK][LD] = (float(*)[BK][LD])smem;
    float(*Bs)[BK][LD] = (float(*)[BK][LD])(smem + 2 * BK * LD);

    const int tid = threadIdx.x, lane = tid & 63, w = tid >> 6;
    const int tn = blockIdx.x % p.tiles_n, tm = blockIdx.x / p.tiles_n;
    const int ks = blockIdx.y % p.splitk, bz = blockIdx.y / p.splitk;
// ... 511 lines not shown
    store_tiles(0);
    __syncthreads();
    int buf = 0;
    for (int kt = kt0; kt < kt1; ++kt) {
        const bool more = (kt + 1 < kt1);
        if (more) load_tiles((kt + 1) * BK);
#pragma unroll
        for (int kk = 0; kk < BK / 16; ++kk) {
            bf16x8 ah[2], al[2], bh[2], bl[2];
#pragma unroll
            for (int i = 0; i < 2; ++i) {
                ah[i] = *(const bf16x8*)&Ts[buf][0][wm + i * 32 + lr][kk * 16 + lk * 8];
                al[i] = *(const bf16x8*)&Ts[buf][1][wm + i * 32 + lr][kk * 16 + lk * 8];
                bh[i] = *(const bf16x8*)&Ts[buf][2][wn + i * 32 + lr][kk * 16 + lk * 8];
                bl[i] = *(const bf16x8*)&Ts[buf][3][wn + i * 32 + lr][kk * 16 + lk * 8];
            }
#pragma unroll
            for (int i = 0; i < 2; ++i)
#pragma unroll
                for (int j = 0; j < 2; ++j) acc[i][j] = __builtin_amdgcn_mfma_f32_32x32x16_bf16(al[i], bh[j], acc[i][j], 0, 0, 0);
#pragma unroll
            for (int i = 0; i < 2; ++i)
#pragma unroll
                for (int j = 0; j < 2; ++j) acc[i][j] = __builtin_amdgcn_mfma_f32_32x32x16_bf16(ah[i], bl[j], acc[i][j], 0, 0, 0);
#pragma unroll
            for (int i = 0; i < 2; ++i)
#pragma unroll
                for (int j = 0; j < 2; ++j) acc[i][j] = __builtin_amdgcn_mfma_f32_32x32x16_bf16(ah[i], bh[j], acc[i][j], 0, 0, 0);
        }
        if (more) store_tiles(buf ^ 1);
        __syncthreads();
        buf ^= 1;
    }
#pragma unroll
    for (int i = 0; i < 2; ++i)
#pragma unroll
        for (int j = 0; j < 2; ++j)
#pragma unroll
            for (int r = 0; r < 16; ++r) {
                int row = tm * BM + wm + i * 32 + (r & 3) + 8 * (r >> 2) + 4 * lk;
                int col = tn * BN + wn + j * 32 + lr;
                epilogue_store(p, zoff, row, col, acc[i][j][r], ks);
            }
}

static int sw_mode(const char* e) { return e ? atoi(e) : 2; }
static int sw_stages(const char* e) { return e ? (e[0] == '1' ? 1 : 2) : 0; }
static int sw_wn3(const char* e) { return e ? (e[0] == '0' ? 0 : 2) : 1; }
static const struct {
    const char* env;
    int (*read)(const char*);
} k_switch[] = {{"A3T_GEMM_8P", sw_mode},     {"A3T_GEMM_PN", sw_mode},         {"A3T_GEMM_TT", sw_mode}, {"A3T_GEMM_8P_TN", sw_mode},
                {"A3T_GEMM_8P_TN3", sw_mode}, {"A3T_GEMM_STAGES", sw_stages}, {"A3T_GEMM_WN3", sw_wn3}};
static int g_switch[] = {-1, -1, -1, -1, -1, -1, -1};
int gemm_switch(int s) {
    if (g_switch[s] < 0) g_switch[s] = k_switch[s].read(getenv(k_switch[s].env));
    return g_switch[s];
}
int gemm_switch_set(int s, int v) {
    const int old = gemm_switch(s);
    g_switch[s] = v;
    return old;
}
extern "C" int a3t_gemm_8p_mode(int mode) { return gemm_switch_set(SW_8P, mode); }
extern "C" int a3t_gemm_pn_mode(int mode) { return gemm_switch_set(SW_PN, mode); }
extern "C" int a3t_gemm_tt_mode(int mode) { return gemm_switch_set(SW_TT, mode); }
extern "C" int a3t_gemm_tn3_mode(int mode) { return gemm_switch_set(SW_8P_TN3, mode); }

GP gemm_rep(int M, int N, int K, int taps, int flags, int keep_layout) {
    static float dummy[4] __attribute__((aligned(16)));
    GP p = {};
    p.M = M, p.N = N, p.K = K, p.taps = taps < 1 ? 1 : taps, p.Kc = K / p.taps, p.b_ts = p.Kc;
    p.a_rs = p.Kc, p.a_cs = 1, p.b_rs = K, p.b_cs = 1, p.c_rs = N, p.splitk = 1, p.accumulate = A3T_ACC_STORE;
    p.Tseq = 1, p.colsum_slots = 1, p.c_dtype = (flags & 16) ? A3T_F32 : A3T_BF16;
    if (flags & 1) p.bias = dummy, p.act = A3T_ACT_RELU;
    if (flags & 2) p.drop_inv = 1.25f;
    if (flags & 4) p.keep_out = (unsigned char*)dummy;
    if (flags & 8) p.keep_in = (const unsigned char*)dummy, p.keep_layout = keep_layout;
    if (flags & 32) p.colsum = dummy;
    if (flags & 64) p.S = dummy, p.s_dtype = A3T_BF16;
    return p;
}

static inline bool al(const void* p, int b) { return ((uintptr_t)p % b) == 0; }
static inline bool m4(int64_t v, int m) { return (v % m) == 0; }

static bool glds_routes(GP& p, int batch, bool AK, bool BKC, GemmPlan* pl) {
    const bool aview = (p.a_unaligned & 1) != 0;
    bool ok = (aview || al(p.A, 16)) && al(p.B, 16) && m4(p.a_bs0, 8) && m4(p.a_bs1, 8) && m4(p.b_bs0, 8) && m4(p.b_bs1, 8);
    if (AK || BKC) ok = ok && m4(p.Kc, 8);
    if (AK)
        ok = ok && (aview || m4(p.a_rs, 8)) && m4(p.K, 8);
    else
        ok = ok && (aview || m4(p.a_cs, 8)) && m4(p.M, 8);
    if (BKC)
        ok = ok && m4(p.b_rs, 8) && m4(p.K, 8) && m4(p.b_ts, 8);
    else
        ok = ok && m4(p.b_cs, 8) && m4(p.b_ts, 8) && m4(p.N, 8);
    if (!AK && p.taps > 1) ok = ok && ((p.N / p.taps) % 128 == 0) && (p.N % p.taps == 0) && p.Tseq > 0;
    if (!ok || (p.colsum && p.accumulate == A3T_ACC_ATOMIC)) return false;
    const int epi_vec = (p.N % 4 == 0) && (p.c_rs % 4 == 0) && (p.c_bs0 % 4 == 0) && (p.c_bs1 % 4 == 0) && al(p.C, 16) &&
                        (!p.R || al(p.R, 16)) && (!p.S || al(p.S, 8)) && (!p.bias || al(p.bias, 16));
    if (p.colsum && !epi_vec) return false;
    const bool keep = p.keep_in || p.keep_out;
    const bool keep_rm = p.keep_layout == 1 && keep;
    if (keep_rm && (!epi_vec || p.c_rs != p.N || batch != 1 || p.splitk != 1 || p.accumulate != A3T_ACC_STORE || p.N % 8 ||
                    (p.keep_out && p.R) || (p.keep_in && p.S)))
        return false;
    if (p.a_signmask && (AK || BKC || p.taps > 1 || p.kshift_mode)) return false;
    p.epi_vec = epi_vec;
    const int ly = (AK && BKC) ? L_NT : (AK ? L_NN : L_TN);
    if (!(p.keep_out || (p.keep_in && !keep_rm) || p.a_signmask || p.A2 || aview) && pn_plan(p, batch, ly, pl)) return true;
    if (!p.a_signmask && !keep_rm && !p.A2 && !aview) {
        if (g8_plan(p, batch, ly, pl)) return true;
        if (keep) return false;
    }
    if (!BKC && !keep && !aview && tt_plan(p, batch, AK ? L_NN : L_TN, pl)) return true;
    if (p.A2) return false;
    glds_plan(p, batch, ly, pl);
    return true;
}

static bool staged_aligned(const GP& p, bool AK, bool BKC) {
    bool ok = al(p.A, 16) && al(p.B, 16);
    if (AK)
        ok = ok && m4(p.a_rs, 8) && m4(p.K, 8) && m4(p.Kc, 8) && m4(p.a_bs0, 8) && m4(p.a_bs1, 8);
    else
        ok = ok && m4(p.a_cs, 4) && m4(p.a_bs0, 4) && m4(p.a_bs1, 4);
    if (BKC)
        ok = ok && m4(p.b_rs, 8) && m4(p.K, 8) && m4(p.Kc, 8) && m4(p.b_ts, 8) && m4(p.b_bs0, 8) && m4(p.b_bs1, 8);
    else
        ok = ok && m4(p.b_cs, 4) && m4(p.b_ts, 4) && m4(p.b_bs0, 4) && m4(p.b_bs1, 4);
    return ok;
}

static int gemm_plan(const a3t_gemm_desc* d, GP* gp, GemmPlan* pl) {
    if (!d || !d->A || !d->B || !d->C || d->M <= 0 || d->N <= 0 || d->K <= 0) return A3T_EINVAL;
    GP& p = *gp;
    p = GP{};
    *pl = GemmPlan{};
    p.A = d->A, p.B = d->B, p.C = d->C, p.bias = d->bias, p.R = d->R, p.S = d->S;
    p.M = d->M, p.N = d->N, p.K = d->K;
    p.taps = d->taps < 1 ? 1 : d->taps;
    const bool wgrad_fused = (d->taps > 1 && d->a_cs != 1);
    if (!wgrad_fused && (p.K % p.taps)) return A3T_EINVAL;
    p.Kc = wgrad_fused ? p.K : p.K / p.taps;
    p.a_rs = d->a_rs, p.a_cs = d->a_cs, p.b_rs = d->b_rs, p.b_cs = d->b_cs, p.b_ts = d->b_ts, p.c_rs = d->c_rs;
    int batch = d->batch < 1 ? 1 : d->batch;
    p.batch_inner = d->batch_inner < 1 ? 1 : d->batch_inner;
    p.a_bs0 = d->a_bs0, p.a_bs1 = d->a_bs1, p.b_bs0 = d->b_bs0, p.b_bs1 = d->b_bs1;
    p.c_bs0 = d->c_bs0, p.c_bs1 = d->c_bs1;
    p.pad = d->pad, p.dil = d->dil < 1 ? 1 : d->dil, p.Tseq = d->Tseq, p.kshift = d->kshift;
    p.kshift_mode = (p.taps == 1 && d->Tseq > 0) ? 1 : 0;
    if (p.taps > 1 && p.Tseq <= 0) return A3T_EINVAL;
    p.alpha = d->alpha, p.act = d->act, p.accumulate = d->accumulate;
    p.sole_writer = 0;
    if (p.accumulate == A3T_ACC_SOLE) p.accumulate = A3T_ACC_ATOMIC, p.sole_writer = 1;
    p.splitk = d->splitk < 1 ? 1 : d->splitk;
    if (p.splitk > 1 && p.accumulate != A3T_ACC_ATOMIC) return A3T_EINVAL;
    if (p.splitk > 1 && p.act != A3T_ACT_NONE) return A3T_EINVAL;
    p.c_dtype = d->c_dtype;
    p.s_dtype = d->s_dtype;
    p.colsum = d->colsum, p.colsum_bs1 = d->colsum_bs1, p.colsum_scale = d->colsum_scale;
    p.colsum_slots = d->colsum_slots > 1 ? d->colsum_slots : 1, p.colsum_ss = d->colsum_ss;
    if (d->drop_p < 0.f || d->drop_p >= 1.f) return A3T_EINVAL;
    p.drop_key = d->drop_key;
    p.drop_thr = (unsigned int)((double)d->drop_p * 4294967296.0);
    p.drop_inv = d->drop_p > 0.f ? 1.f / (1.f - d->drop_p) : 0.f;
    p.keep_out = (unsigned char*)d->keep_out, p.keep_in = (const unsigned char*)d->keep_in;
    p.a_signmask = d->a_signmask ? 1 : 0;
    p.A2 = d->A2, p.B2 = d->B2, p.b2_cs = d->b2_cs, p.b2_bs0 = d->b2_bs0, p.b2_bs1 = d->b2_bs1, p.colsum2 = d->colsum2;
    p.a2_rs = d->a2_rs, p.a_unaligned = d->a_unaligned;
    if ((p.A2 == nullptr) != (p.B2 == nullptr) || (!p.A2 && (p.colsum2 || p.a2_rs || (p.a_unaligned & 2))) || (p.a_unaligned & ~3)) return A3T_EINVAL;
    if ((p.a_unaligned & 1) && (d->compute != A3T_BF16 || d->a_dtype != A3T_BF16 || d->b_dtype != A3T_BF16 || p.taps > 1 || d->Tseq > 0 ||
                                ((uintptr_t)p.A & 1)))
        return A3T_EINVAL;
    p.keep_layout = (p.keep_out || p.keep_in) ? d->keep_layout : 0;
    if (p.keep_layout != 0 && p.keep_layout != 1) return A3T_EINVAL;
    const bool keep = p.keep_out || p.keep_in;
    if (keep && (d->compute != A3T_BF16 || d->a_dtype != A3T_BF16 || d->b_dtype != A3T_BF16)) return A3T_EINVAL;
    if (p.c_dtype == A3T_BF16 && p.accumulate != A3T_ACC_STORE && (p.accumulate != A3T_ACC_ADD || p.splitk > 1)) return A3T_EINVAL;
    const bool AK = (d->a_cs == 1), BKC = (d->b_cs == 1);
    if (!AK && d->a_rs != 1) return A3T_EINVAL;
    if (!BKC && d->b_rs != 1) return A3T_EINVAL;
    p.tiles_n = (p.N + 127) / 128;
    if (p.taps > 1 && !AK) {
        if (d->compute != A3T_BF16 || d->a_dtype != A3T_BF16 || d->b_dtype != A3T_BF16 || d->b_cs == 1 || p.a_signmask || p.A2) return A3T_EINVAL;
        return glds_routes(p, batch, false, false, pl) ? 0 : A3T_EINVAL;
    }
    if (!AK && BKC) return A3T_EINVAL;
    const int tiles_m = (p.M + 127) / 128;
    const dim3 grid((unsigned)(p.tiles_n * tiles_m), (unsigned)(batch * p.splitk));

    if (d->compute == A3T_F32 || d->compute == A3T_BF16X3) {
        if (d->a_dtype != A3T_F32 || d->b_dtype != A3T_F32 || d->colsum || p.a_signmask || p.A2) return A3T_EINVAL;
        if (d->compute == A3T_BF16X3 && staged_aligned(p, AK, BKC)) {
            pl->route = GR_BF16X3, pl->ak = AK, pl->bkc = BKC, pl->grid = grid;
            snprintf(pl->name, sizeof(pl->name), "gemm_bf16x3_kernel<%s, %s>", tf(AK), tf(BKC));
            return 0;
        }
        bool vec = al(p.A, 16) && al(p.B, 16) && m4(p.a_bs0, 4) && m4(p.a_bs1, 4) && m4(p.b_bs0, 4) && m4(p.b_bs1, 4);
        if (AK)
            vec = vec && m4(p.a_rs, 4) && m4(p.K, 4) && m4(p.Kc, 4);
        else
            vec = vec && m4(p.a_cs, 4);
        if (BKC)
            vec = vec && m4(p.b_rs, 4) && m4(p.K, 4) && m4(p.Kc, 4) && m4(p.b_ts, 4);
        else
            vec = vec && m4(p.b_cs, 4) && m4(p.b_ts, 4);
        pl->route = GR_F32, pl->ak = AK, pl->bkc = BKC, pl->vec = vec, pl->grid = grid;
        snprintf(pl->name, sizeof(pl->name), "gemm_f32_kernel<%s, %s, %s>", tf(AK), tf(BKC), tf(vec));
        return 0;
    }
    if (d->compute != A3T_BF16) return A3T_EINVAL;
    if (d->a_dtype == A3T_BF16 && d->b_dtype == A3T_BF16 && glds_routes(p, batch, AK, BKC, pl)) return 0;
    if (keep || p.a_signmask || p.A2 || p.a_unaligned) return A3T_EINVAL;
    if (d->colsum) return A3T_EINVAL;
    if (!staged_aligned(p, AK, BKC)) return A3T_EINVAL;
    pl->route = GR_BF16_LEGACY, pl->ak = AK, pl->bkc = BKC, pl->grid = grid;
    pl->a_f32 = d->a_dtype == A3T_F32, pl->b_f32 = d->b_dtype == A3T_F32;
    snprintf(pl->name, sizeof(pl->name), "gemm_bf16_kernel<%s, %s, %s, %s>", pl->a_f32 ? "float" : "unsigned short",
             pl->b_f32 ? "float" : "unsigned short", tf(AK), tf(BKC));
    return 0;
}

static int f32_launch(const GP& p, const GemmPlan& pl, hipStream_t stream) {
#define LAUNCH_F32(ak, bk)                                                                          \
    do {                                                                                            \
        if (pl.vec)                                                                                 \
            hipLaunchKernelGGL((gemm_f32_kernel<ak, bk, true>), pl.grid, dim3(256), 0, stream, p);  \
        else                                                                                        \
            hipLaunchKernelGGL((gemm_f32_kernel<ak, bk, false>), pl.grid, dim3(256), 0, stream, p); \
    } while (0)
    if (pl.ak && pl.bkc)
        LAUNCH_F32(true, true);
    else if (pl.ak)
        LAUNCH_F32(true, false);
    else
        LAUNCH_F32(false, false);
#undef LAUNCH_F32
    return (int)hipGetLastError();
}

static int legacy_launch(const GP& p, const GemmPlan& pl, hipStream_t stream) {
#define LAUNCH_BF(TA, TB)                                                                                   \
    do {                                                                                                    \
        if (pl.ak && pl.bkc)                                                                                \
            hipLaunchKernelGGL((gemm_bf16_kernel<TA, TB, true, true>), pl.grid, dim3(256), 0, stream, p);   \
        else if (pl.ak)                                                                                     \
            hipLaunchKernelGGL((gemm_bf16_kernel<TA, TB, true, false>), pl.grid, dim3(256), 0, stream, p);  \
        else                                                                                                \
            hipLaunchKernelGGL((gemm_bf16_kernel<TA, TB, false, false>), pl.grid, dim3(256), 0, stream, p); \
    } while (0)
    if (pl.a_f32 && pl.b_f32)
        LAUNCH_BF(float, float);
    else if (pl.a_f32)
        LAUNCH_BF(float, unsigned short);
    else if (pl.b_f32)
        LAUNCH_BF(unsigned short, float);
    else
        LAUNCH_BF(unsigned short, unsigned short);
#undef LAUNCH_BF
    return (int)hipGetLastError();
}

static int x3_launch(const GP& p, const GemmPlan& pl, hipStream_t stream) {
#define LAUNCH_X3(ak, bk)                                                                                                   \
    do {                                                                                                                    \
        const hipError_t opt_in =                                                                                           \
            hipFuncSetAttribute((const void*)gemm_bf16x3_kernel<ak, bk>, hipFuncAttributeMaxDynamicSharedMemorySize, X3_LDS); \
        if (opt_in != hipSuccess) return (int)opt_in;                                                                       \
        hipLaunchKernelGGL((gemm_bf16x3_kernel<ak, bk>), pl.grid, dim3(256), X3_LDS, stream, p);                            \
    } while (0)
    if (pl.ak && pl.bkc)
        LAUNCH_X3(true, true);
    else if (pl.ak)
        LAUNCH_X3(true, false);
    else
        LAUNCH_X3(false, false);
#undef LAUNCH_X3
    return (int)hipGetLastError();
}

extern "C" int a3t_gemm(const a3t_gemm_desc* d, void* stream_) {
    hipStream_t stream = (hipStream_t)stream_;
    GP p;
    GemmPlan pl;
    const int rc = gemm_plan(d, &p, &pl);
    if (rc) return rc;
    int r;
    switch (pl.route) {
        case GR_F32: r = f32_launch(p, pl, stream); break;
        case GR_BF16_LEGACY: r = legacy_launch(p, pl, stream); break;
        case GR_BF16X3: r = x3_launch(p, pl, stream); break;
        case GR_GLDS_128: r = glds_launch(p, pl, stream); break;
        case GR_PN: r = pn_launch(p, pl, stream); break;
        case GR_TT: r = tt_launch(p, pl, stream); break;
        default: r = g8_launch(p, pl, stream); break;
    }
    a3t_note_kernel(pl.name);
    return r;
}

extern "C" int a3t_gemm_plan(const a3t_gemm_desc* d, char* name, int len) {
    GP p;
    GemmPlan pl;
    const int rc = gemm_plan(d, &p, &pl);
    if (!rc && name && len > 0) snprintf(name, (size_t)len, "%s", pl.name);
    return rc;
}
```

a3t_amd/csrc/gemm_bf16_tt.hip:

```cpp
#include <hip/hip_runtime.h>
#include <stdint.h>
#include <stdlib.h>
#include "../../include/a3t_hip.h"
#include "gemm_common.h"
#include "mfma_kit.h"

typedef short s16x4 __attribute__((ext_vector_type(4)));
typedef short s16x8 __attribute__((ext_vector_type(8)));
typedef unsigned short u16;

namespace {
constexpr int TT_MAX_ROWS = 320, TT_BK = 32, TT_STAGES = 4;
constexpr int TT_A_BYTES = TT_MAX_ROWS * TT_BK * 2, TT_B_BYTES = 192 * TT_BK * 2, TT_STAGE = TT_A_BYTES + TT_B_BYTES;
constexpr int TT_LDS = TT_STAGES * TT_STAGE;
}

#ifdef TT_TIMING
__device__ unsigned long long tt_stamps[1024 * 4];
extern "C" int a3t_debug_read_tt(void* dst, size_t bytes) { return (int)hipMemcpyFromSymbol(dst, HIP_SYMBOL(tt_stamps), bytes); }
#define TT_STAMP(k) do { if (tid == 0 && blockIdx.x < 1024) tt_stamps[blockIdx.x * 4 + (k)] = wall_clock64(); } while (0)
#else
#define TT_STAMP(k)
#endif

template <bool ATN, int NJ, bool ASGN = false, bool DUAL = false>
__global__ __launch_bounds__(512, 2) void gemm_bf16_tt_kernel(GP p, int TR) {
    extern __shared__ __attribute__((aligned(16))) unsigned char smem[];
    const int tid = threadIdx.x, lane = tid & 63;
    const int w = __builtin_amdgcn_readfirstlane(tid >> 6);
    const int wr = w >> 2, wc = w & 3;
    TT_STAMP(0);
    const int wi = xcd_contiguous(blockIdx.x, gridDim.x);
    const int tm = wi % p.ntiles, bz = wi / p.ntiles;
    const int z0 = bz / p.batch_inner, z1 = bz % p.batch_inner;
    const u16* A = (const u16*)p.A + z0 * p.a_bs0 + z1 * p.a_bs1;
    const u16* B = (const u16*)p.B + z0 * p.b_bs0 + z1 * p.b_bs1;
    const int64_t zoff = z0 * p.c_bs0 + z1 * p.c_bs1;
    const int m0 = tm * TR;
    const int HR = TR >> 1, nbi = HR >> 4;
    const int nkt = (p.K + TT_BK - 1) / TT_BK;

    const unsigned a_ld = (unsigned)(ATN ? p.a_cs : p.a_rs) * 2u, b_ld = (unsigned)p.b_cs * 2u;
    const unsigned a_ext = ATN ? (unsigned)(p.K - 1) * a_ld + (unsigned)p.M * 2u : (unsigned)(p.M - 1) * a_ld + (unsigned)p.K * 2u;
    const unsigned b_ext = (unsigned)(p.K - 1) * b_ld + (unsigned)p.N * 2u;
    const bool is_a = w < 5;
    const __amdgpu_buffer_rsrc_t rX = __builtin_amdgcn_make_buffer_rsrc((void*)(is_a ? A : B), 0, (int)(is_a ? a_ext : b_ext), 0x00020000);
    const unsigned b2_ld = DUAL ? (unsigned)p.b2_cs * 2u : 0u;
    const void* X2 = DUAL ? (is_a ? (const void*)((const u16*)p.A2 + z0 * p.a_bs0 + z1 * p.a_bs1) : (const void*)((const u16*)p.B2 + z0 * p.b2_bs0 + z1 * p.b2_bs1)) : (const void*)A;
    const unsigned a2_ld = (DUAL && p.a2_rs) ? (unsigned)p.a2_rs * 2u : a_ld;
    const __amdgpu_buffer_rsrc_t rX2 = __builtin_amdgcn_make_buffer_rsrc((void*)X2, 0, (int)(is_a ? (unsigned)(p.M - 1) * a2_ld + (unsigned)p.K * 2u : (unsigned)(p.K - 1) * b2_ld + (unsigned)p.N * 2u), 0x00020000);
    const unsigned lds0 = __builtin_amdgcn_readfirstlane((unsigned)(uintptr_t)LDS_AS(smem));

    unsigned voff[4];
    unsigned voff2[4];
    int kq[4];
    const unsigned ld = is_a ? a_ld : b_ld;
#pragma unroll
    for (int q = 0; q < 4; ++q) {
        if (is_a && !ATN) {
            const int R = (w * 4 + q) * 16 + (lane >> 2);
            const int g = (lane & 3) ^ ((4 - ((lane >> 4) & 3)) & 3);
            const bool ok = R < TR && m0 + R < p.M;
            voff[q] = ok ? (unsigned)(m0 + R) * a_ld + (unsigned)g * 16u : OOB;
            voff2[q] = ok ? (unsigned)(m0 + R) * a2_ld + (unsigned)g * 16u : OOB;
            kq[q] = g * 8;
        } else {
            const int s = is_a ? w * 4 + q : (w - 5) * 4 + q;
            const int r = (s & 3) * 8 + (lane >> 3);
            const int sw = ((r >> 1) & 1) | (((r >> 3) & 1) << 1);
            const int col = (s >> 2) * 64 + (((lane & 7) ^ (sw << 1)) << 3);
            const bool ok = is_a ? (col < TR && m0 + col < p.M) : (col < p.N && col < 64 * NJ);
            voff[q] = ok ? (unsigned)r * ld + (unsigned)((is_a ? m0 : 0) + col) * 2u : OOB;
            voff2[q] = ok ? (unsigned)r * (is_a ? ld : b2_ld) + (unsigned)((is_a ? m0 : 0) + col) * 2u : OOB;
            kq[q] = r;
        }
    }
    const unsigned kstep = (is_a && !ATN) ? 64u : 32u * ld;
    const unsigned kstep2 = (is_a && !ATN) ? 64u : 32u * (is_a ? ld : b2_ld);
    const unsigned dst0 = lds0 + (is_a ? (unsigned)(w * 4) * 1024u : (unsigned)TT_A_BYTES + (unsigned)((w - 5) * 4) * 1024u);
    auto issue = [&](const int kt) __attribute__((always_inline)) {
        const unsigned dst = dst0 + (unsigned)(kt & 3) * (unsigned)TT_STAGE;
        if (DUAL && kt >= nkt) {
            const int k2 = kt - nkt;
            const unsigned so = (unsigned)k2 * kstep2;
            const int krem = p.K - k2 * TT_BK;
#pragma unroll
            for (int q = 0; q < 4; ++q) dma16(rX2, dst + q * 1024, kq[q] < krem ? voff2[q] : OOB, so);
            return;
        }
        const unsigned so = (unsigned)kt * kstep;
        const int krem = p.K - kt * TT_BK;
#pragma unroll
        for (int q = 0; q < 4; ++q) dma16(rX, dst + q * 1024, kq[q] < krem ? voff[q] : OOB, so);
    };

    const int g = lane >> 4, pp = lane & 15;
    const unsigned offkc = (unsigned)pp * 64u + (unsigned)((g ^ ((4 - (pp >> 2)) & 3)) << 4);
    const unsigned swr = (unsigned)((((pp >> 3) & 1) | ((g & 1) << 1)) << 1);
    const unsigned kbyte = (unsigned)(g * 8 + (pp >> 2)) * 128u + (unsigned)(pp & 1) * 8u;
    auto frag_rc = [&](const unsigned char* img, const int c0) __attribute__((always_inline)) -> bf16x8 {
        const unsigned cb = (unsigned)((c0 & 63) >> 3) + (unsigned)((pp >> 1) & 1);
        const unsigned char* a0 = img + (c0 >> 6) * 4096 + kbyte + ((cb ^ swr) << 4);
        s16x4 lo = __builtin_amdgcn_ds_read_tr16_b64_v4i16((__attribute__((address_space(3))) s16x4*)LDS_AS(a0));
        s16x4 hi = __builtin_amdgcn_ds_read_tr16_b64_v4i16((__attribute__((address_space(3))) s16x4*)LDS_AS(a0 + 512));
        s16x8 v = {lo[0], lo[1], lo[2], lo[3], hi[0], hi[1], hi[2], hi[3]};
        return __builtin_bit_cast(bf16x8, v);
    };

    f32x4 acc[10][NJ];
#pragma unroll
    for (int i = 0; i < 10; ++i)
#pragma unroll
        for (int j = 0; j < NJ; ++j) acc[i][j] = f32x4{0.f, 0.f, 0.f, 0.f};

    issue(0), issue(1), issue(2);
    const int rb0 = wr * nbi;
    const int nkt_all = DUAL ? 2 * nkt : nkt;
    float cs1[NJ][4];
#pragma unroll
    for (int j = 0; j < NJ; ++j)
#pragma unroll
        for (int r = 0; r < 4; ++r) cs1[j][r] = 0.f;
    for (int kt = 0; kt < nkt_all; ++kt) {
        WAIT_VM(8);
        BAR();
#ifdef TT_TIMING
        if (kt == 0) TT_STAMP(1);
#endif
        issue(kt + 3);
        const unsigned char* sA = smem + (kt & 3) * TT_STAGE;
        const unsigned char* sB = sA + TT_A_BYTES;
        bf16x8 fb[NJ];
#pragma unroll
        for (int j = 0; j < NJ; ++j) fb[j] = frag_rc(sB, wc * (16 * NJ) + j * 16);
        bf16x8 fa[10];
#pragma unroll
        for (int i = 0; i < 10; ++i) {
            if (ATN)
                fa[i] = ASGN ? a3t_sign_floor(frag_rc(sA, (rb0 + i) * 16), 0) : frag_rc(sA, (rb0 + i) * 16);
            else
                fa[i] = *(const bf16x8*)(sA + (rb0 + i) * 1024 + offkc);
        }
        SB();
#pragma unroll
        for (int i = 0; i < 10; ++i)
#pragma unroll
            for (int j = 0; j < NJ; ++j) acc[i][j] = __builtin_amdgcn_mfma_f32_16x16x32_bf16(fb[j], fa[i], acc[i][j], 0, 0, 0);
        if (DUAL && kt == nkt - 1 && p.colsum) {
#pragma unroll
            for (int i = 0; i < 10; ++i)
                if (i < nbi) {
#pragma unroll
                    for (int j = 0; j < NJ; ++j)
#pragma unroll
                        for (int r = 0; r < 4; ++r) cs1[j][r] += acc[i][j][r];
                }
        }
    }
    WAIT_VM(0);
    __syncthreads();
    TT_STAMP(2);

    const int crow = m0 + rb0 * 16 + pp;
    const int ccol = wc * (16 * NJ) + g * 4;
    u16* Cb = (u16*)p.C + zoff + ccol;
    float cs[NJ][4];
#pragma unroll
    for (int j = 0; j < NJ; ++j)
#pragma unroll
        for (int r = 0; r < 4; ++r) cs[j][r] = 0.f;
    const bool add = p.accumulate != A3T_ACC_STORE;
    const float alpha = p.alpha;
#pragma unroll
    for (int i = 0; i < 10; ++i) {
        const int row = crow + i * 16;
        const bool rok = i < nbi && row < p.M;
        uint2 old[NJ];
        if (add) {
#pragma unroll
            for (int j = 0; j < NJ; ++j)
                old[j] = (rok && ccol + j * 16 < p.N) ? *(const uint2*)(Cb + (int64_t)row * p.c_rs + j * 16) : make_uint2(0u, 0u);
        }
#pragma unroll
        for (int j = 0; j < NJ; ++j) {
            if (!rok || ccol + j * 16 >= p.N) continue;
            float v0 = acc[i][j][0] * alpha, v1 = acc[i][j][1] * alpha, v2 = acc[i][j][2] * alpha, v3 = acc[i][j][3] * alpha;
            cs[j][0] += v0, cs[j][1] += v1, cs[j][2] += v2, cs[j][3] += v3;
            if (add) v0 += bf2f(old[j].x & 0xffff), v1 += bf2f(old[j].x >> 16), v2 += bf2f(old[j].y & 0xffff), v3 += bf2f(old[j].y >> 16);
            uint2 o;
            o.x = io_pack2(v0, v1), o.y = io_pack2(v2, v3);
            *(uint2*)(Cb + (int64_t)row * p.c_rs + j * 16) = o;
        }
    }
    if (p.colsum) {
        float* o = p.colsum + z1 * p.colsum_bs1 + ccol;
        if (p.colsum_slots > 1) o += (int64_t)((tm + z0) % p.colsum_slots) * p.colsum_ss;
#pragma unroll
        for (int j = 0; j < NJ; ++j)
#pragma unroll
            for (int r = 0; r < 4; ++r) {
                const float t = row16_sum(cs[j][r]);
                if (DUAL) {
                    const float t1 = row16_sum(cs1[j][r] * alpha);
                    if (pp == 0 && ccol + j * 16 < p.N) {
                        atomicAdd(o + j * 16 + r, p.colsum_scale * t1);
                        atomicAdd(o + (p.colsum2 - p.colsum) + j * 16 + r, p.colsum_scale * (t - t1));
                    }
                } else if (pp == 0 && ccol + j * 16 < p.N) {
                    atomicAdd(o + j * 16 + r, p.colsum_scale * t);
                }
            }
    }
#ifdef TT_TIMING
    __syncthreads();
    TT_STAMP(3);
#endif
}

template <bool ATN, int NJ, bool ASGN = false, bool DUAL = false>
static void launch_tt(const GP& pv, int TR, int grid, hipStream_t stream) {
    (void)hipFuncSetAttribute((const void*)gemm_bf16_tt_kernel<ATN, NJ, ASGN, DUAL>, hipFuncAttributeMaxDynamicSharedMemorySize, TT_LDS);
    hipLaunchKernelGGL((gemm_bf16_tt_kernel<ATN, NJ, ASGN, DUAL>), dim3(grid), dim3(512), TT_LDS, stream, pv, TR);
}

static bool tt_tiling(int M, int N, int K, int batch, int mode, int& tiles, int& TR) {
    const int cus = device_cus();
    tiles = 0, TR = 0;
    long best = 0;
    for (int t = (M + TT_MAX_ROWS - 1) / TT_MAX_ROWS, n = 0; n < 6; ++t, ++n) {
        const int tr = (((M + t - 1) / t) + 31) / 32 * 32;
        if (tr > TT_MAX_ROWS || (long)tr * (t - 1) >= M) continue;
        const long cost = (((long)t * batch + cus - 1) / cus) * (tr + 64);
        if (!tiles || cost < best) tiles = t, TR = tr, best = cost;
    }
    if (!tiles) return false;
    const long units = (long)tiles * batch;
    if (mode == 2) {
        if (K < 512 || M < 256 || N < 96 || units > cus || units * TR * 4 > (long)M * batch * 5 || units * 10 < cus * 7) return false;
    }
    return true;
}

bool tt_plan(const GP& p, int batch, int ly, GemmPlan* pl) {
    const int mode = gemm_switch(SW_TT);
    if (mode == 0 || (ly != L_NN && ly != L_TN) || p.splitk != 1 || p.accumulate == A3T_ACC_ATOMIC) return false;
    if (p.a_signmask && ly != L_TN) return false;
    if (p.A2) {
        const bool v2 = (p.a_unaligned & 2) != 0;
        const int64_t a2 = p.a2_rs ? p.a2_rs : p.a_rs;
        if (ly != L_NN || p.accumulate != A3T_ACC_STORE || !p.B2 || p.b2_cs % 8 || (p.b2_bs0 | p.b2_bs1) % 8 || ((uintptr_t)p.B2 & 15) ||
            ((uintptr_t)p.A2 & (v2 ? 1 : 15)) || (!v2 && a2 % 8) || a2 < p.K || a2 * 2 * (int64_t)p.M >= (1ll << 31) ||
            p.b2_cs * 2 * (int64_t)p.K >= (1ll << 31) || (p.colsum != nullptr) != (p.colsum2 != nullptr))
            return false;
    }
    if (p.taps > 1 || p.kshift_mode || p.keep_in || p.keep_out || !p.epi_vec) return false;
    if (p.b_rs != 1 || p.N > 192 || p.N % 8 || p.M % 8 || p.K % 8) return false;
    if (ly == L_NN ? (p.a_cs != 1 || p.a_rs % 8) : (p.a_rs != 1 || p.a_cs % 8)) return false;
    if (p.b_cs % 8 || (p.a_bs0 | p.a_bs1 | p.b_bs0 | p.b_bs1) % 8) return false;
    if (p.bias || p.R || p.S || p.act != A3T_ACT_NONE || p.drop_inv > 0.f || p.c_dtype != A3T_BF16) return false;
    const int64_t a_ld = ly == L_NN ? p.a_rs : p.a_cs;
    if (a_ld * 2 * (int64_t)(ly == L_NN ? p.M : p.K) >= (1ll << 31) || p.b_cs * 2 * (int64_t)p.K >= (1ll << 31)) return false;
    int tiles = 0, TR = 0;
    if (!tt_tiling(p.M, p.N, p.K, batch, mode, tiles, TR)) return false;
    pl->route = GR_TT, pl->ly = ly, pl->ntiles = tiles, pl->TR = TR, pl->grid = dim3((unsigned)((long)tiles * batch));
    pl->nj = p.N <= 128 ? 2 : 3;
    pl->atn = ly == L_TN, pl->asgn = pl->atn && p.a_signmask, pl->dual = !pl->atn && p.A2;
    snprintf(pl->name, sizeof(pl->name), "gemm_bf16_tt_kernel<%s, %d, %s, %s>", tf(pl->atn), pl->nj, tf(pl->asgn), tf(pl->dual));
    return true;
}

extern "C" int a3t_gemm_tt_supported(int M, int N, int K, int batch) {
    static float dummy[4] __attribute__((aligned(16)));
    GP p = {};
    p.A = dummy, p.B = dummy, p.C = dummy;
    p.M = M, p.N = N, p.K = K, p.Kc = K, p.taps = 1, p.alpha = 1.f, p.colsum_slots = 1;
    p.a_rs = K, p.a_cs = 1, p.b_rs = 1, p.b_cs = N, p.c_rs = N;
    p.batch_inner = 1, p.a_bs0 = (int64_t)M * K, p.b_bs0 = (int64_t)K * N, p.c_bs0 = (int64_t)M * N;
    p.splitk = 1, p.accumulate = A3T_ACC_STORE, p.c_dtype = A3T_BF16, p.epi_vec = 1;
    GemmPlan pl;
    return tt_plan(p, batch, L_NN, &pl) ? 1 : 0;
}

int tt_launch(const GP& p, const GemmPlan& pl, hipStream_t stream) {
    GP pv = p;
    pv.ntiles = pl.ntiles;
    const int TR = pl.TR, grid = (int)pl.grid.x;
    const bool nj3 = pl.nj == 3;
    if (pl.asgn) {
        if (nj3)
            launch_tt<true, 3, true>(pv, TR, grid, stream);
        else
            launch_tt<true, 2, true>(pv, TR, grid, stream);
    } else if (pl.atn) {
        if (nj3)
            launch_tt<true, 3>(pv, TR, grid, stream);
        else
            launch_tt<true, 2>(pv, TR, grid, stream);
    } else if (pl.dual) {
        if (nj3)
            launch_tt<false, 3, false, true>(pv, TR, grid, stream);
        else
            launch_tt<false, 2, false, true>(pv, TR, grid, stream);
    } else {
        if (nj3)
            launch_tt<false, 3>(pv, TR, grid, stream);
        else
            launch_tt<false, 2>(pv, TR, grid, stream);
    }
    return (int)hipGetLastError();
}
```

a3t_amd/csrc/gemm_common.h:

```cpp
#pragma once
#include <hip/hip_runtime.h>
#include <stdint.h>
#include <stdio.h>
#include "../../include/a3t_hip.h"
#include "dtype_io.h"
#include "device_cus.h"

void a3t_note_kernel(const char* name);

enum { L_NT = 0, L_NN = 1, L_TN = 2 };

struct GP {
    const void* A;
    const void* B;
    void* C;
    const float* bias;
    const float* R;
    const float* S;
    int M, N, K, Kc;
    int64_t a_rs, a_cs, b_rs, b_cs, b_ts, c_rs;
    int batch_inner;
    int64_t a_bs0, a_bs1, b_bs0, b_bs1, c_bs0, c_bs1;
    int taps, pad, dil, Tseq, kshift, kshift_mode;
    float alpha;
    int act, accumulate, splitk, c_dtype, tiles_n, s_dtype, epi_vec;
    int ntiles;
    float* colsum;
    int64_t colsum_bs1;
    float colsum_scale;
    int colsum_slots, colsum_ss;
    unsigned int drop_key, drop_thr;
    float drop_inv;
    unsigned char* keep_out;
    const unsigned char* keep_in;
    unsigned int a_bytes, b_bytes;
    float* slab;
    int sole_writer;
    const void* A2;
    const void* B2;
    int64_t b2_cs, b2_bs0, b2_bs1;
    float* colsum2;
    int64_t a2_rs;
    int a_unaligned;
    int keep_layout;
    int a_signmask;
};

__device__ __forceinline__ unsigned short f2bf(float f) { return io_f2bf(f); }

template <typename V>
__device__ __forceinline__ V a3t_sign_floor(V v, short fl) {
    typedef short s16x8_ __attribute__((ext_vector_type(8)));
    const s16x8_ f = {fl, fl, fl, fl, fl, fl, fl, fl};
    return __builtin_bit_cast(V, __builtin_elementwise_max(__builtin_bit_cast(s16x8_, v), f));
}
__device__ __forceinline__ float bf2f(unsigned short h) { return __uint_as_float(((unsigned int)h) << 16); }

template <typename T>
__device__ __forceinline__ float ldf(const T* p);
template <>
__device__ __forceinline__ float ldf<float>(const float* p) {
    return *p;
}
template <>
__device__ __forceinline__ float ldf<unsigned short>(const unsigned short* p) {
    return bf2f(*p);
}

template <typename T>
__device__ __forceinline__ const T* a_ptr_k(const GP& p, const T* A, int m, int tpos, int kg) {
    if (p.taps > 1) {
        int tap = kg / p.Kc;
        int c = kg - tap * p.Kc;
        int off = (tap - p.pad) * p.dil;
        int tt = tpos + off;
        if (tt < 0 || tt >= p.Tseq) return nullptr;
        return A + (int64_t)(m + off) * p.a_rs + c;
    }
    return A + (int64_t)m * p.a_rs + kg;
}
__device__ __forceinline__ bool b_koff(const GP& p, int k, int64_t& koff) {
    if (p.taps > 1) {
        int tap = k / p.Kc;
        int c = k - tap * p.Kc;
        koff = (int64_t)tap * p.b_ts + (int64_t)c * p.b_cs;
        return true;
    }
    if (p.kshift_mode) {
        int tt = (k % p.Tseq) + p.kshift;
        koff = (int64_t)(k + p.kshift) * p.b_cs;
        return tt >= 0 && tt < p.Tseq;
    }
    koff = (int64_t)k * p.b_cs;
    return true;
}

__device__ __forceinline__ float apply_act(float v, int act) {
    if (act == A3T_ACT_RELU) return fmaxf(v, 0.f);
    if (act == A3T_ACT_TANH) return tanhf(v);
    if (act == A3T_ACT_SWISH) return v / (1.f + __expf(-v));
    return v;
}

__device__ __forceinline__ void epilogue_store(const GP& p, int64_t zoff, int row, int col, float v, int ks) {
    if (row >= p.M || col >= p.N) return;
    int64_t idx = zoff + (int64_t)row * p.c_rs + col;
    if (p.bias && ks == 0) v += p.bias[col];
    v = apply_act(v, p.act);
    if (p.S) {
        float sv = (p.s_dtype == A3T_BF16) ? bf2f(((const unsigned short*)p.S)[idx]) : p.S[idx];
        v = (sv > 0.f) ? v : 0.f;
    }
    if (p.drop_inv > 0.f) v = rng_keep(p.drop_key, (unsigned int)idx, p.drop_thr) ? v * p.drop_inv : 0.f;
    v *= p.alpha;
    if (p.R && ks == 0) v += p.R[idx];
    if (p.c_dtype == A3T_BF16) {
        unsigned short* c = (unsigned short*)p.C + idx;
        *c = f2bf(p.accumulate == A3T_ACC_STORE ? v : v + bf2f(*c));
        return;
    }
    float* C = (float*)p.C;
    if (p.accumulate == A3T_ACC_STORE)
        C[idx] = v;
    else if (p.accumulate == A3T_ACC_ADD)
        C[idx] += v;
    else
#ifdef A3T_EXPERIMENT_NOATOMIC
        C[idx] = v;
#else
        atomicAdd(&C[idx], v);
#endif
}


__device__ __forceinline__ void epilogue_vec4(const GP& p, float4 v, int64_t idx, const float4& bias4, int ks, float4& cs) {
    v.x += bias4.x, v.y += bias4.y, v.z += bias4.z, v.w += bias4.w;
    if (p.act != A3T_ACT_NONE) {
        v.x = apply_act(v.x, p.act), v.y = apply_act(v.y, p.act);
        v.z = apply_act(v.z, p.act), v.w = apply_act(v.w, p.act);
    }
    if (p.S) {
        float4 sv;
        if (p.s_dtype == A3T_BF16) {
            uint2 t = *(const uint2*)((const unsigned short*)p.S + idx);
            sv = make_float4(bf2f(t.x & 0xffff), bf2f(t.x >> 16), bf2f(t.y & 0xffff), bf2f(t.y >> 16));
        } else {
            sv = *(const float4*)(p.S + idx);
        }
        v.x = sv.x > 0.f ? v.x : 0.f, v.y = sv.y > 0.f ? v.y : 0.f;
        v.z = sv.z > 0.f ? v.z : 0.f, v.w = sv.w > 0.f ? v.w : 0.f;
    }
    if (p.keep_layout == 1 && p.keep_in) {
        const unsigned kb = p.keep_in[idx >> 2];
        v.x = (kb & 1u) ? v.x : 0.f, v.y = (kb & 2u) ? v.y : 0.f, v.z = (kb & 4u) ? v.z : 0.f, v.w = (kb & 8u) ? v.w : 0.f;
    }
    if (p.drop_inv > 0.f) {
        const unsigned int i0 = (unsigned int)idx;
        bool kp[4];
        rng_keep4(p.drop_key, i0, p.drop_thr, kp);
        v.x = kp[0] ? v.x * p.drop_inv : 0.f, v.y = kp[1] ? v.y * p.drop_inv : 0.f;
        v.z = kp[2] ? v.z * p.drop_inv : 0.f, v.w = kp[3] ? v.w * p.drop_inv : 0.f;
    }
    v.x *= p.alpha, v.y *= p.alpha, v.z *= p.alpha, v.w *= p.alpha;
    if (p.keep_layout == 1 && p.keep_out)
        p.keep_out[idx >> 2] = (unsigned char)((v.x > 0.f ? 1u : 0u) | (v.y > 0.f ? 2u : 0u) | (v.z > 0.f ? 4u : 0u) | (v.w > 0.f ? 8u : 0u));
    if (p.R && ks == 0) {
        float4 rv = *(const float4*)(p.R + idx);
        v.x += rv.x, v.y += rv.y, v.z += rv.z, v.w += rv.w;
    }
    cs.x += v.x, cs.y += v.y, cs.z += v.z, cs.w += v.w;
    if (p.c_dtype == A3T_BF16) {
        uint2* c = (uint2*)((unsigned short*)p.C + idx);
        if (p.accumulate != A3T_ACC_STORE) {
            const uint2 t = *c;
            v.x += bf2f(t.x & 0xffff), v.y += bf2f(t.x >> 16), v.z += bf2f(t.y & 0xffff), v.w += bf2f(t.y >> 16);
        }
        uint2 o;
        o.x = io_pack2(v.x, v.y);
        o.y = io_pack2(v.z, v.w);
        *c = o;
    } else {
        float* C = (float*)p.C + idx;
        if (p.accumulate == A3T_ACC_STORE) {
            *(float4*)C = v;
        } else {
            float4 o = *(const float4*)C;
            o.x += v.x, o.y += v.y, o.z += v.z, o.w += v.w;
            *(float4*)C = o;
        }
    }
}
template <int LR = 16>
__device__ __forceinline__ void colsum_flush(const GP& p, float4 cs, int lane, bool col_ok, int z1, int col, int spread = 0) {
#pragma unroll
    for (int o = LR; o < 64; o <<= 1) {
        cs.x += __shfl_xor(cs.x, o, 64), cs.y += __shfl_xor(cs.y, o, 64);
        cs.z += __shfl_xor(cs.z, o, 64), cs.w += __shfl_xor(cs.w, o, 64);
    }
    if (lane < LR && col_ok) {
        float* o = p.colsum + z1 * p.colsum_bs1 + col;
        if (p.colsum_slots > 1) o += (int64_t)(spread % p.colsum_slots) * p.colsum_ss;
        atomicAdd(o + 0, p.colsum_scale * cs.x), atomicAdd(o + 1, p.colsum_scale * cs.y);
        atomicAdd(o + 2, p.colsum_scale * cs.z), atomicAdd(o + 3, p.colsum_scale * cs.w);
    }
}

enum GemmRoute { GR_F32, GR_BF16_LEGACY, GR_GLDS_128, GR_PN, GR_G8, GR_G8_TN, GR_G8_TN3, GR_TT, GR_BF16X3 };
struct GemmPlan {
    GemmRoute route;
    bool ak, bkc, vec;
    bool a_f32, b_f32;
    int ly, stages, wn, conv;
    bool cv;
    int nj;
    bool atn, asgn, dual;
    dim3 grid;
    int tiles_n, ntiles, splits, folds, TR;
    size_t slab_floats;
    char name[96];
};

enum GemmSwitch { SW_8P, SW_PN, SW_TT, SW_8P_TN, SW_8P_TN3, SW_STAGES, SW_WN3 };
int gemm_switch(int s);
int gemm_switch_set(int s, int v);
GP gemm_rep(int M, int N, int K, int taps, int flags, int keep_layout);
static inline const char* tf(bool b) { return b ? "true" : "false"; }

void glds_plan(const GP& p, int batch, int ly, GemmPlan* pl);
int glds_launch(const GP& p, const GemmPlan& pl, hipStream_t stream);
bool pn_plan(const GP& p, int batch, int ly, GemmPlan* pl);
int pn_launch(const GP& p, const GemmPlan& pl, hipStream_t stream);
bool g8_plan(const GP& p, int batch, int ly, GemmPlan* pl);
int g8_launch(const GP& p, const GemmPlan& pl, hipStream_t stream);
bool g8_tn_plan(const GP& p, int batch, GemmPlan* pl);
int g8_tn_launch(const GP& p, const GemmPlan& pl, hipStream_t stream);
bool tt_plan(const GP& p, int batch, int ly, GemmPlan* pl);
int tt_launch(const GP& p, const GemmPlan& pl, hipStream_t stream);
```

a3t_amd/csrc/mfma_kit.h:

```cpp
#pragma once
#include <hip/hip_runtime.h>
#include <stdint.h>

typedef __bf16 bf16x8 __attribute__((ext_vector_type(8)));
typedef float f32x4 __attribute__((ext_vector_type(4)));

#define LDS_AS(p) ((__attribute__((address_space(3))) void*)(p))
#define SB() __builtin_amdgcn_sched_barrier(0)
#define BAR()                                   \
    do {                                        \
        SB();                                   \
        asm volatile("s_barrier" ::: "memory"); \
        SB();                                   \
    } while (0)
#define WAIT_VM(n) asm volatile("s_waitcnt vmcnt(" #n ")" ::: "memory")
#define WAIT_LGKM(n) asm volatile("s_waitcnt lgkmcnt(" #n ")" ::: "memory")

constexpr unsigned OOB = 0x80000000u;

#if defined(__HIP_DEVICE_COMPILE__) && !defined(__gfx950__)
#error "buffer_load_dwordx4 ... lds (16-byte LDS-DMA) exists on gfx950 only: build with --offload-arch=gfx950"
#endif
__device__ __forceinline__ void dma16(const __amdgpu_buffer_rsrc_t& r, unsigned lds_addr, unsigned voff, unsigned soff) {
    asm volatile("s_mov_b32 m0, %0\n\ts_nop 0\n\tbuffer_load_dwordx4 %1, %2, %3 offen lds" ::"s"(lds_addr), "v"(voff), "s"(r), "s"(soff) : "memory");
}

__device__ __forceinline__ float row16_sum(float v) {
    v += __builtin_bit_cast(float, __builtin_amdgcn_update_dpp(0, __builtin_bit_cast(int, v), 0xB1, 0xf, 0xf, true));
    v += __builtin_bit_cast(float, __builtin_amdgcn_update_dpp(0, __builtin_bit_cast(int, v), 0x4E, 0xf, 0xf, true));
    v += __builtin_bit_cast(float, __builtin_amdgcn_update_dpp(0, __builtin_bit_cast(int, v), 0x141, 0xf, 0xf, true));
    v += __builtin_bit_cast(float, __builtin_amdgcn_update_dpp(0, __builtin_bit_cast(int, v), 0x140, 0xf, 0xf, true));
    return v;
}

__device__ __forceinline__ int xcd_contiguous(int wi, int nwg) {
    const int q = nwg >> 3, r = nwg & 7, xcd = wi & 7;
    return (xcd < r ? xcd * (q + 1) : r * (q + 1) + (xcd - r) * q) + (wi >> 3);
}
```

a3t_amd/ops.py:

```python
import ctypes
import os

import torch

from . import _lib as L
from ._lib import ACC_ADD, ACC_ATOMIC, ACC_SOLE, ACC_STORE, ACT_NONE, ACT_RELU, ACT_SWISH, ACT_TANH, BF16, F32

__all__ = ["gemm", "gemm_plan", "linear_fwd", "linear_bwd_data", "linear_bwd_weight", "conv_fwd", "conv_bwd_data",
           "conv_bwd_weight"]


PROFILE = None


def _stream():
    return ctypes.c_void_p(torch.cuda.current_stream().cuda_stream)


def _ptr(t):
    if t is None:
        return None
    return ctypes.c_void_p(t.data_ptr())


def _dt(t):
    if t.dtype == torch.float32:
        return F32
    if t.dtype == torch.bfloat16:
        return BF16
    raise TypeError(f"unsupported dtype {t.dtype}")


def _gemm_desc(A, B, C, M, N, K, a_rs, a_cs, b_rs, b_cs, c_rs, *, b_ts=0, bias=None, R=None, S=None, batch=1,
               batch_inner=1, a_bs=(0, 0), b_bs=(0, 0), c_bs=(0, 0), taps=1, pad=0, dil=1, Tseq=0, kshift=0, alpha=1.0,
               act=ACT_NONE, acc=ACC_STORE, splitk=1, compute=F32, colsum=None, colsum_bs1=0, colsum_scale=1.0,
               drop=None, colsum_slots=1, colsum_ss=0, keep_out=None, keep_in=None, a_signmask=False, keep_layout=0, second=None,
               a_view=False):
    d = L.GemmDesc()
    d.A, d.B, d.C = A.data_ptr(), B.data_ptr(), C.data_ptr()
    d.bias = bias.data_ptr() if bias is not None else None
    d.R = R.data_ptr() if R is not None else None
    d.S = S.data_ptr() if S is not None else None
    d.M, d.N, d.K = M, N, K
    d.a_rs, d.a_cs, d.b_rs, d.b_cs, d.b_ts, d.c_rs = a_rs, a_cs, b_rs, b_cs, b_ts, c_rs
    d.batch, d.batch_inner = batch, batch_inner
    d.a_bs0, d.a_bs1 = a_bs
    d.b_bs0, d.b_bs1 = b_bs
    d.c_bs0, d.c_bs1 = c_bs
    d.taps, d.pad, d.dil, d.Tseq, d.kshift = taps, pad, dil, Tseq, kshift
    d.alpha, d.act, d.accumulate, d.splitk = alpha, act, acc, splitk
    d.a_dtype, d.b_dtype, d.c_dtype, d.compute = _dt(A), _dt(B), _dt(C), compute
    d.s_dtype = _dt(S) if S is not None else F32
    d.colsum = colsum.data_ptr() if colsum is not None else None
    d.colsum_bs1, d.colsum_scale = colsum_bs1, colsum_scale
    d.colsum_slots, d.colsum_ss = colsum_slots, colsum_ss
    d.drop_p, d.drop_key = (drop if drop is not None else (0.0, 0))
    d.keep_out = keep_out.data_ptr() if keep_out is not None else None
    d.keep_in = keep_in.data_ptr() if keep_in is not None else None
    d.a_signmask = 1 if a_signmask else 0
    d.keep_layout = keep_layout
    d.a_unaligned = 1 if a_view else 0
    if second is not None:
        A2, B2, b2_cs, b2_bs, cs2 = second[:5]
        d.A2, d.B2, d.b2_cs = A2.data_ptr(), B2.data_ptr(), b2_cs
        d.b2_bs0, d.b2_bs1 = b2_bs
        d.colsum2 = cs2.data_ptr() if cs2 is not None else None
        if len(second) > 5:
            d.a2_rs = second[5]
            d.a_unaligned |= 2
    return d


def gemm(*args, **kw):
    lib = L.load()
    d = _gemm_desc(*args, **kw)
    if PROFILE is not None:
        e0, e1 = torch.cuda.Event(enable_timing=True), torch.cuda.Event(enable_timing=True)
        e0.record()
        L.check(lib.a3t_gemm(ctypes.byref(d), _stream()), "a3t_gemm")
        e1.record()
        PROFILE.append((lib.a3t_gemm_last_kernel().decode(), (4.0 if d.A2 else 2.0) * d.M * d.N * d.K * d.batch, e0, e1,
                        (d.M, d.N, d.K, d.batch, d.taps, d.splitk)))
        return
    L.check(lib.a3t_gemm(ctypes.byref(d), _stream()), "a3t_gemm")


def gemm_plan(*args, **kw):
    name = ctypes.create_string_buffer(128)
    rc = L.load().a3t_gemm_plan(ctypes.byref(_gemm_desc(*args, **kw)), name, len(name))
    return name.value.decode() if rc == 0 else None


_SPLITK_TARGET = 1000


def _splitk_for(n_tiles, K, ktile=64):
    target = _SPLITK_TARGET if n_tiles >= 64 else 440
    s = max(1, target // max(n_tiles, 1))
    s = min(s, max(1, K // (ktile * 8)))
    return int(s)


def linear_fwd(x, W, out, bias=None, R=None, alpha=1.0, act=ACT_NONE, compute=F32, drop=None):
    M, K = x.shape
    N = W.shape[0]
    gemm(x, W, out, M, N, K, K, 1, K, 1, N, bias=bias, R=R, alpha=alpha, act=act, compute=compute, drop=drop)


def linear_bwd_data(dy, W, dx, S=None, alpha=1.0, acc=ACC_STORE, compute=F32, colsum=None):
    M, N = dy.shape
    K = W.shape[1]
    gemm(dy, W, dx, M, K, N, N, 1, 1, K, K, S=S, alpha=alpha, acc=acc, compute=compute, colsum=colsum)


def linear_bwd_weight(dy, x, dW, alpha=1.0, compute=F32):
    M, N = dy.shape
    K = x.shape[1]
    tiles = ((N + 127) // 128) * ((K + 127) // 128)
    gemm(dy, x, dW, N, K, M, 1, N, 1, K, K, alpha=alpha, acc=ACC_SOLE, splitk=_splitk_for(tiles, M),
         compute=compute)


def linear_bwd_weight_group(items, compute=F32):
    if compute == BF16 and len(items) > 1 and len(items) <= 8:
        lib = L.load()
        arr = (L.GemmDesc * len(items))()
        for d, (dy, x, dW, alpha) in zip(arr, items):
            M, N = dy.shape
            K = x.shape[1]
            d.A, d.B, d.C = dy.data_ptr(), x.data_ptr(), dW.data_ptr()
            d.M, d.N, d.K = N, K, M
            d.a_rs, d.a_cs, d.b_rs, d.b_cs, d.b_ts, d.c_rs = 1, N, 1, K, 0, K
            d.batch, d.batch_inner, d.taps, d.dil = 1, 1, 1, 1
            d.alpha, d.act, d.accumulate, d.splitk = alpha, ACT_NONE, ACC_SOLE, 1
            d.a_dtype, d.b_dtype, d.c_dtype, d.compute, d.s_dtype = _dt(dy), _dt(x), _dt(dW), compute, F32
            d.colsum_slots = 1
        if PROFILE is not None:
            e0, e1 = torch.cuda.Event(enable_timing=True), torch.cuda.Event(enable_timing=True)
            e0.record()
        rc = lib.a3t_gemm_tn3_group(ctypes.cast(arr, ctypes.c_void_p), len(items), _stream())
        if rc == 0:
            if PROFILE is not None:
                e1.record()
                tok, cin = items[0][0].shape[0], items[0][1].shape[1]
                cout = sum(dy.shape[1] for dy, _, _, _ in items)
                PROFILE.append((lib.a3t_gemm_last_kernel().decode() + f" x{len(items)} grouped", 2.0 * tok * cout * cin, e0, e1,
                                (cout, cin, tok, 1, 1, 1)))
            return True
        if rc != -1:
            L.check(rc, "a3t_gemm_tn3_group")
    for dy, x, dW, alpha in items:
        linear_bwd_weight(dy, x, dW, alpha=alpha, compute=compute)
    return False


def conv_fwd(x, Wk, out, Tseq, pad, dil=1, bias=None, R=None, alpha=1.0, act=ACT_NONE, compute=F32, drop=None,
             keep_out=None, keep_in=None, colsum=None, S=None, keep_layout=0):
    M, Cin = x.shape
    N, taps, _ = Wk.shape
    gemm(x, Wk, out, M, N, taps * Cin, Cin, 1, taps * Cin, 1, N, b_ts=Cin, bias=bias, R=R, taps=taps, pad=pad,
         dil=dil, Tseq=Tseq, alpha=alpha, act=act, compute=compute, drop=drop, keep_out=keep_out, keep_in=keep_in,
         colsum=colsum, S=S, keep_layout=keep_layout)


G8_BIAS_ACT, G8_DROP, G8_KEEP_OUT, G8_KEEP_IN, G8_F32_OR_RES, G8_COLSUM, G8_SMASK = 1, 2, 4, 8, 16, 32, 64


def gemm_8p_supported(M, N, K, taps=1, flags=0):
    return bool(L.load().a3t_gemm_8p_supported(int(M), int(N), int(K), int(taps), int(flags)))


def gemm_pn_supported(M, N, K, taps=1, flags=0):
    return bool(L.load().a3t_gemm_pn_supported(int(M), int(N), int(K), int(taps), int(flags)))


def gemm_tt_supported(M, N, K, batch):
    return bool(L.load().a3t_gemm_tt_supported(int(M), int(N), int(K), int(batch)))


def gemm_mode_tag():
    lib = L.load()
    m8 = lib.a3t_gemm_8p_mode(2)
    lib.a3t_gemm_8p_mode(m8)
    mp = lib.a3t_gemm_pn_mode(2)
    lib.a3t_gemm_pn_mode(mp)
    return (m8, mp)


def collate_paint(fs, fe, alen, sel, mspan, nms, flen, tlen, masked, speech_mask, text_mask, sp, tp, sega_emb):
    B, P = fs.shape
    Tm, Tp, S = masked.shape[1], text_mask.shape[1], mspan.shape[1]
    L.check(L.load().a3t_collate_paint(_ptr(fs), _ptr(fe), _ptr(alen), _ptr(sel), _ptr(mspan), _ptr(nms), _ptr(flen), _ptr(tlen),
                                       _ptr(masked), _ptr(speech_mask), _ptr(text_mask), _ptr(sp), _ptr(tp), B, Tm, Tp, P, S,
                                       int(bool(sega_emb)), _stream()), "collate_paint")


def segment_colsum(x, out, B, T):
    L.check(L.load().a3t_segment_colsum(_ptr(x), _ptr(out), B, T, x.shape[1], _stream()), "segment_colsum")


def gemm_keep_bytes(M, N):
    return int(L.load().a3t_gemm_keep_bytes(int(M), int(N)))


def conv_bwd_data(dy, Wk, dx, Tseq, pad, dil=1, S=None, alpha=1.0, compute=F32, colsum=None):
    M, N = dy.shape
    _, taps, Cin = Wk.shape
    Wv = Wk.view(-1)[(taps - 1) * Cin:]
    gemm(dy, Wv, dx, M, Cin, taps * N, N, 1, 1, taps * Cin, Cin, b_ts=-Cin, S=S, taps=taps, pad=taps - 1 - pad,
         dil=dil, Tseq=Tseq, alpha=alpha, compute=compute, colsum=colsum)


def conv_bwd_weight(dy, x, dWk, Tseq, pad, dil=1, alpha=1.0, compute=F32):
    M, N = dy.shape
    Cin = x.shape[1]
    taps = dWk.shape[1]
    if compute == BF16 and dy.dtype == torch.bfloat16 and x.dtype == torch.bfloat16 and Cin % 128 == 0 \
            and N % 8 == 0 and taps > 1:
        tiles = ((N + 127) // 128) * (taps * Cin // 128)
        gemm(dy, x, dWk, N, taps * Cin, M, 1, N, 1, Cin, taps * Cin, taps=taps, pad=pad, dil=dil, Tseq=Tseq,
             alpha=alpha, acc=ACC_SOLE, splitk=_splitk_for(tiles, M), compute=compute)
        return
    tiles = ((N + 127) // 128) * ((Cin + 127) // 128)
    sk = _splitk_for(tiles, M)
    flat = dWk.view(-1)
    for tap in range(taps):
        gemm(dy, x, flat[tap * Cin:], N, Cin, M, 1, N, 1, Cin, taps * Cin, Tseq=Tseq, kshift=(tap - pad) * dil,
             alpha=alpha, acc=ACC_ATOMIC, splitk=sk, compute=compute)


def _dto(t):
    return _dt(t) if t is not None else F32


def layernorm_fwd(x, g, b, y, mean, rstd, eps):
    M, D = x.shape
    L.check(L.load().a3t_layernorm_fwd(_ptr(x), _ptr(g), _ptr(b), _ptr(y), _dt(y), _ptr(mean), _ptr(rstd), M, D, eps,
                                       _stream()), "ln_fwd")


def layernorm_bwd(dy, x, g, mean, rstd, dres, dx, dg, db, dx16=None, dxsum=None, dxsum_scale=1.0, drop=(0.0, 0)):
    M, D = x.shape
    L.check(L.load().a3t_layernorm_bwd(_ptr(dy), _dt(dy), _ptr(x), _ptr(g), _ptr(mean), _ptr(rstd), _ptr(dres),
                                       _ptr(dx), _ptr(dx16), _ptr(dg), _ptr(db), _ptr(dxsum), dxsum_scale, M, D,
                                       drop[0], drop[1], _stream()), "ln_bwd")


def col_reduce(x, out0, out1=None, y=None, rowmask=None, mode=0, ld=None):
    M, C = x.shape
    L.check(L.load().a3t_col_reduce(_ptr(x), _dt(x), _ptr(y), _ptr(rowmask), _ptr(out0), _ptr(out1), M, C,
                                    ld if ld is not None else x.stride(0), mode, _stream()), "col_reduce")


def f64_to_f32_add(src, dst, scale=1.0):
    L.check(L.load().a3t_f64_to_f32_add(_ptr(src), _ptr(dst), dst.numel(), scale, _stream()), "f64_to_f32_add")


def bias_grad(dy, dbias, scratch64, scale=1.0):
    n = dy.shape[1]
    s = scratch64[:n]
    s.zero_()
    col_reduce(dy, s, mode=0)
    f64_to_f32_add(s, dbias, scale)


def bn_act_fwd(z, stats, g, b, rmean, rvar, mean_out, rstd_out, y, eps, momentum, training, act):
    M, C = z.shape
    L.check(L.load().a3t_bn_act_fwd(_ptr(z), _ptr(stats), _ptr(g), _ptr(b), _ptr(rmean), _ptr(rvar), _ptr(mean_out),
                                    _ptr(rstd_out), _ptr(y), _dt(y), M, C, eps, momentum, int(training), act,
                                    _stream()), "bn_act_fwd")


def bn_act_bwd(dy, z, mean, rstd, g, b, sums, dz, dg, db, training, act, zero=True):
    M, C = z.shape
    lib = L.load()
    if zero:
        sums.zero_()
    L.check(lib.a3t_bn_act_bwd_a(_ptr(dy), _dt(dy), _ptr(z), _ptr(mean), _ptr(rstd), _ptr(g), _ptr(b), _ptr(sums), M, C,
                                 act, _stream()), "bn_bwd_a")
    L.check(lib.a3t_bn_act_bwd_b(_ptr(dy), _dt(dy), _ptr(z), _ptr(mean), _ptr(rstd), _ptr(g), _ptr(b), _ptr(sums),
                                 _ptr(dz), _ptr(dg), _ptr(db), M, C, int(training), act, _stream()), "bn_bwd_b")


def glu_dwconv_fwd(g, wdw, bdw, glu, z, Tseq):
    M, C = glu.shape
    L.check(L.load().a3t_glu_dwconv_fwd(_ptr(g), _dt(g), _ptr(wdw), _ptr(bdw), _ptr(glu), _dt(glu), _ptr(z), M, C,
                                        wdw.shape[1], Tseq, _stream()), "glu_dwconv_fwd")


def glu_dwconv_bwd(dz, g, glu, wdw, dg, dwdw, dbdw, Tseq, dgsum=None):
    M, C = glu.shape
    L.check(L.load().a3t_glu_dwconv_bwd(_ptr(dz), _ptr(g), _dt(g), _ptr(glu), _dt(glu), _ptr(wdw), _ptr(dg), _dt(dg),
                                        _ptr(dwdw), _ptr(dbdw), _ptr(dgsum), M, C, wdw.shape[1], Tseq, _stream()),
            "glu_dwconv_bwd")


def add_pos_bias(qkv, u, v, qu, qv):
    M, d = qu.shape
    L.check(L.load().a3t_add_pos_bias(_ptr(qkv), _ptr(u), _ptr(v), _ptr(qu), _ptr(qv), _dt(qkv), M, d, _stream()),
            "pos_bias")


def add_pos_bias_bwd(dqu, dqv, dqkv):
    M, d = dqu.shape
    L.check(L.load().a3t_add_pos_bias_bwd(_ptr(dqu), _ptr(dqv), _ptr(dqkv), _dt(dqu), M, d, _stream()),
            "pos_bias_bwd")


def relpos_softmax_fwd(ac, bd, keymask, probs, B, H, T, scale, probs_drop=None, drop=(0.0, 0)):
    L.check(L.load().a3t_relpos_softmax_fwd(_ptr(ac), _ptr(bd), _dt(ac), _ptr(keymask), _ptr(probs), _dt(probs), B, H, T,
                                            T * T, T * T, T * T, scale, _ptr(probs_drop), drop[0], drop[1],
                                            _stream()), "softmax_fwd")


def relpos_softmax_bwd(probs, dprobs, ds, dbd, B, H, T, scale, probs_drop=None, drop_p=0.0, dbd_head_major=False,
                       drop_key=0, rowscale=None):
    bsb, bsh = (T * T, B * T * T) if dbd_head_major else (0, 0)
    L.check(L.load().a3t_relpos_softmax_bwd(_ptr(probs), _dt(probs), _ptr(dprobs), _dt(dprobs), _ptr(ds), _ptr(dbd), _dt(dbd), B, H,
                                            T, T * T, T * T, T * T, scale, _ptr(probs_drop), drop_p, bsb, bsh, drop_key,
                                            _ptr(rowscale), _stream()), "softmax_bwd")


def attn_fused_supported(dk, T):
    return dk % 32 == 0 and dk <= 192 and dk != 160 and T % 8 == 0 and 8 <= T <= 4096


def _attn_q_operands(qu, qv, qkv, pos_bias):
    d = qkv.shape[1] // 3
    if pos_bias is None:
        return _ptr(qu), _ptr(qv), d, None, None
    return _ptr(qkv), _ptr(qkv), 3 * d, _ptr(pos_bias[0]), _ptr(pos_bias[1])


def attn_fwd(qu, qv, qkv, P, keymask, ctx, lse, B, H, T, scale, drop=(0.0, 0), pos_bias=None):
    d = qkv.shape[1] // 3
    dk = d // H
    kk = qkv.view(-1)[d:]
    vv = qkv.view(-1)[2 * d:]
    pqu, pqv, ldq, pbu, pbv = _attn_q_operands(qu, qv, qkv, pos_bias)
    L.check(L.load().a3t_attn_fwd(pqu, pqv, _ptr(kk), _ptr(vv), _ptr(P), _ptr(keymask), _ptr(ctx), _ptr(lse),
                                  B, H, T, dk, ldq, 3 * d, d, d, scale, drop[0], drop[1], pbu, pbv, _stream()), "attn_fwd")


def attn_fwd_train(qu, qv, qkv, P, keymask, ctx, lse, probs, probs_drop, rowscale, B, H, T, scale, drop=(0.0, 0), pos_bias=None):
    d = qkv.shape[1] // 3
    dk = d // H
    kk = qkv.view(-1)[d:]
    vv = qkv.view(-1)[2 * d:]
    pqu, pqv, ldq, pbu, pbv = _attn_q_operands(qu, qv, qkv, pos_bias)
    e0 = None
    if PROFILE is not None:
        e0, e1 = torch.cuda.Event(enable_timing=True), torch.cuda.Event(enable_timing=True)
        e0.record()
    L.check(L.load().a3t_attn_fwd_train(pqu, pqv, _ptr(kk), _ptr(vv), _ptr(P), _ptr(keymask), _ptr(ctx), _ptr(lse),
                                        _ptr(probs), _ptr(probs_drop), _ptr(rowscale), B, H, T, dk, ldq, 3 * d, d, d, scale,
                                        drop[0], drop[1], pbu, pbv, _stream()), "attn_fwd_train")
    if e0 is not None:
        e1.record()
        PROFILE.append((f"attn_fwd32_kernel<{dk // 32}, {'true' if drop[0] > 0 else 'false'}, true, false, false, {'true' if (drop[0] > 0 and probs_drop is None) else 'false'}>", 3 * 2.0 * B * H * T * T * dk, e0, e1,
                        (T, T, dk, B * H, 1, 1)))


def attn_scale_rows(x, rowscale, y, B, H, T):
    d = x.shape[1]
    L.check(L.load().a3t_attn_scale_rows(_ptr(x), _ptr(rowscale), _ptr(y), B, H, T, d // H, _stream()), "attn_scale_rows")


def attn_bwd_ds(dctx, ctx, qkv, probs, rowscale, ds, dbd, B, H, T, scale, drop=(0.0, 0), dbd_head_major=False, signed_probs=False,
                ds_bs=0):
    d = dctx.shape[1]
    v = qkv.view(-1)[2 * d:]
    bsb, bsh = ((T * T, B * T * T) if dbd_head_major else (0, 0))
    L.check(L.load().a3t_attn_bwd_ds(_ptr(dctx), _ptr(ctx), _ptr(v), _ptr(probs), _ptr(rowscale), _ptr(ds), _ptr(dbd), B, H, T,
                                     d // H, d, 3 * d, bsb, bsh, scale, drop[0], drop[1], 1 if signed_probs else 0, ds_bs, _stream()), "attn_bwd_ds")


def mask_fill(speech, masked, mask_feature, out):
    M, C = out.shape
    L.check(L.load().a3t_mask_fill(_ptr(speech), _ptr(masked), _ptr(mask_feature), _ptr(out), _dt(out), M, C,
                                   _stream()), "mask_fill")


def embed_finish_fwd(e, emb, seg, text, spos, tpos, xs, B, Tm, Tp, D, xscale, drop=(0.0, 0), spk=None):
    L.check(L.load().a3t_embed_finish_fwd(_ptr(e), _ptr(emb), _ptr(seg), _ptr(text), _ptr(spos), _ptr(tpos), _ptr(xs),
                                          B, Tm, Tp, D, xscale, drop[0], drop[1], _ptr(spk), _stream()), "embed_fwd")


def embed_finish_bwd(dxs, e, text, spos, tpos, de, demb, dseg, B, Tm, Tp, D, V, nseg, xscale, drop=(0.0, 0)):
    L.check(L.load().a3t_embed_finish_bwd(_ptr(dxs), _ptr(e), _ptr(text), _ptr(spos), _ptr(tpos), _ptr(de),
                                          _ptr(demb), _ptr(dseg), B, Tm, Tp, D, V, nseg, xscale, drop[0], drop[1],
                                          _stream()), "embed_bwd")


def scale(x, y, s):
    L.check(L.load().a3t_scale(_ptr(x), _ptr(y), x.numel(), s, _stream()), "scale")


def scale_dev(x, y, s):
    L.check(L.load().a3t_scale_dev(_ptr(x), _ptr(y), x.numel(), _ptr(s), _stream()), "scale_dev")


def axpy(x, y, a=1.0):
    L.check(L.load().a3t_axpy(_ptr(x), _ptr(y), x.numel(), a, _stream()), "axpy")


def attn_bias_fold(slots, S, d, gu, gv, gbqkv):
    L.check(L.load().a3t_attn_bias_fold(_ptr(slots), S, d, _ptr(gu), _ptr(gv), _ptr(gbqkv), _stream()), "attn_bias_fold")


def cast_bf16(x, y):
    L.check(L.load().a3t_cast_bf16(_ptr(x), _ptr(y), x.numel(), _stream()), "cast_bf16")


def cast_bf16_conv_t(src_flat, dst, src_off, dst_off, N, taps, C):
    L.check(L.load().a3t_cast_bf16_conv_t(_ptr(src_flat), _ptr(dst), _ptr(src_off), _ptr(dst_off), src_off.numel(), N, taps, C,
                                          _stream()), "cast_bf16_conv_t")


def split_bf16(x, hi, lo):
    L.check(L.load().a3t_split_bf16(_ptr(x), _ptr(hi), _ptr(lo), x.numel(), _stream()), "split_bf16")


def slice_rows(x, y, B, T, Tm, D, reverse_add=False):
    L.check(L.load().a3t_slice_rows(_ptr(x), _ptr(y), _dt(y), B, T, Tm, D, int(reverse_add), _stream()), "slice_rows")


def concat_rows(speech, text, xs, B, Tm, Tp, D):
    L.check(L.load().a3t_concat_rows(_ptr(speech), _ptr(text), _ptr(xs), B, Tm, Tp, D, _stream()), "concat_rows")


def concat_rows_ragged(speech, text, xs, slens, tlens, B, Tm, Tp, D, speech_bs=None, text_bs=None):
    L.check(L.load().a3t_concat_rows_ragged(_ptr(speech), _ptr(text), _ptr(xs), _ptr(_i32(slens, "slens")),
                                            _ptr(_i32(tlens, "tlens")), B, Tm, Tp, D, Tm * D if speech_bs is None else speech_bs,
                                            Tp * D if text_bs is None else text_bs, _stream()), "concat_rows_ragged")


def split_rows(dxs, dspeech, dtext, B, Tm, Tp, D):
    L.check(L.load().a3t_split_rows(_ptr(dxs), _ptr(dspeech), _ptr(dtext), B, Tm, Tp, D, _stream()), "split_rows")


def reflect_pad(x, out, pad):
    B, N = x.shape
    L.check(L.load().a3t_reflect_pad(_ptr(x), _ptr(out), B, N, pad, out.shape[1], _stream()), "reflect_pad")


def reflect_pad_ragged(x, out, pad, lens, host_lens):
    B, N = x.shape
    host_lens = [int(n) for n in host_lens]
    if len(host_lens) != B or lens.numel() != B:
        raise ValueError(f"reflect_pad_ragged: {B} rows, {len(host_lens)} host lengths, {lens.numel()} device lengths")
    for b, n in enumerate(host_lens):
        if n <= pad or n > N:
            raise ValueError(f"reflect_pad_ragged: row {b} has {n} samples; reflection by {pad} needs {pad} < n <= {N}")
    L.check(L.load().a3t_reflect_pad_ragged(_ptr(x), _ptr(out), _ptr(_i32(lens, "lens")), B, N, pad, out.shape[1], _stream()),
            "reflect_pad_ragged")


def stft_amp(S, amp, nbins):
    L.check(L.load().a3t_stft_amp(_ptr(S), _ptr(amp), amp.shape[0], nbins, amp.shape[1], _stream()), "stft_amp")


def logmel_finish(mel, olens, B, F, C):
    L.check(L.load().a3t_logmel_finish(_ptr(mel), _ptr(olens), B, F, C, _stream()), "logmel_finish")


def mlm_loss(before, after, target, masked, loss_out, d_before, d_after, scratch, l2=False, gscale=1.0):
    M, C = before.shape
    L.check(L.load().a3t_mlm_loss(_ptr(before), _ptr(after), _ptr(target), _ptr(masked), _ptr(loss_out),
                                  _ptr(d_before), _ptr(d_after), _ptr(scratch), M, C, int(l2), gscale, _stream()),
            "mlm_loss")


def loss_scratch_floats(M):
    return L.load().a3t_mlm_loss_scratch_floats(M)


def sumsq(g, partial):
    L.check(L.load().a3t_sumsq(_ptr(g), g.numel(), _ptr(partial), _stream()), "sumsq")


def clip_adam(p, g, m, v, partial, norm_out, lr, step, clip=1.0, gscale=1.0, betas=(0.9, 0.999), eps=1e-8):
    L.check(L.load().a3t_clip_adam(_ptr(p), _ptr(g), _ptr(m), _ptr(v), _ptr(partial), _ptr(norm_out), p.numel(), lr,
                                   betas[0], betas[1], eps, step, clip, gscale, _stream()), "clip_adam")


def clip_adam_noam(p, g, m, v, partial, norm_out, state, base_lr, model_size, warmup, clip=1.0, gscale=1.0,
                   betas=(0.9, 0.999), eps=1e-8):
    L.check(L.load().a3t_clip_adam_noam(_ptr(p), _ptr(g), _ptr(m), _ptr(v), _ptr(partial), _ptr(norm_out), p.numel(),
                                        _ptr(state), base_lr, float(model_size), float(warmup), betas[0], betas[1], eps,
                                        clip, gscale, _stream()), "clip_adam_noam")


def sgd_step(p, g, lr, gscale=1.0):
    if p.dtype != torch.float32 or g.dtype != torch.float32 or p.numel() != g.numel() or not (p.is_contiguous() and g.is_contiguous()):
        raise ValueError("sgd_step: p and g must be contiguous fp32 buffers of one size")
    L.check(L.load().a3t_sgd_step(_ptr(p), _ptr(g), p.numel(), float(lr), float(gscale), _stream()), "sgd_step")


def pwg_gate(y, c, out):
    T, H = out.shape
    L.check(L.load().a3t_pwg_gate(_ptr(y), _ptr(c), _ptr(out), T, H, _stream()), "pwg_gate")


def pwg_res_skip(o, x, skips):
    T, R = x.shape
    L.check(L.load().a3t_pwg_res_skip(_ptr(o), _ptr(x), _ptr(skips), T, R, skips.shape[1], _stream()), "pwg_res_skip")


def _i32(t, what):
    if t.dtype != torch.int32 or not t.is_contiguous():
        raise ValueError(f"{what} must be a contiguous int32 tensor")
    return t


def _rows_lens(what, x, lens):
    B = x.shape[0] if x.dim() == 3 else 1
    if lens is not None and _i32(lens, "lens").numel() != B:
        raise ValueError(f"{what}: {lens.numel()} lengths for {B} rows")
    return (B, *x.shape[-2:])


def pwg_upsample(c, w, out, scale_, lens=None, mul=1):
    B, Tin, C = _rows_lens("pwg_upsample", c, lens)
    if lens is None:
        rc = L.load().a3t_pwg_upsample(_ptr(c), _ptr(w), _ptr(out), B, Tin, C, scale_, _stream())
    else:
        rc = L.load().a3t_pwg_upsample_ragged(_ptr(c), _ptr(w), _ptr(out), _ptr(lens), mul, B, Tin, C, scale_, _stream())
    L.check(rc, "pwg_upsample")


def replicate_pad(x, y, pad, lens=None):
    B, T, C = _rows_lens("replicate_pad", x, lens)
    if lens is None:
        rc = L.load().a3t_replicate_pad(_ptr(x), _ptr(y), B, T, C, pad, _stream())
    else:
        rc = L.load().a3t_replicate_pad_ragged(_ptr(x), _ptr(y), _ptr(lens), B, T, C, pad, _stream())
    L.check(rc, "replicate_pad")


def zero_tail(x, lens, mul, B, T):
    C = x.shape[-1]
    L.check(L.load().a3t_zero_tail(_ptr(x), _ptr(_i32(lens, "lens")), mul, B, T, C, _stream()), "zero_tail")


def _ragged_f32(what, *ts):
    for t in ts:
        if t is not None and (t.dtype != torch.float32 or not t.is_contiguous()):
            raise TypeError(f"{what}: tensors must be contiguous fp32")


def layernorm_fwd_ragged(x, g, b, y, mean, rstd, lens, B, T, eps):
    M, D = x.shape
    _ragged_f32("layernorm_fwd_ragged", x, y, mean, rstd)
    if M != B * T or y.shape != x.shape or lens.numel() != B:
        raise ValueError("layernorm_fwd_ragged: shapes do not fit")
    L.check(L.load().a3t_layernorm_fwd_ragged(_ptr(x), _ptr(g), _ptr(b), _ptr(y), _ptr(mean), _ptr(rstd),
                                              _ptr(_i32(lens, "lens")), B, T, D, eps, _stream()), "ln_fwd_ragged")


def glu_dwconv_fwd_ragged(g, wdw, bdw, glu, z, lens, B, Tseq):
    M, C = glu.shape
    _ragged_f32("glu_dwconv_fwd_ragged", g, glu, z)
    if M != B * Tseq or g.shape != (M, 2 * C) or z.shape != glu.shape or lens.numel() != B:
        raise ValueError("glu_dwconv_fwd_ragged: shapes do not fit")
    L.check(L.load().a3t_glu_dwconv_fwd_ragged(_ptr(g), _ptr(wdw), _ptr(bdw), _ptr(glu), _ptr(z), _ptr(_i32(lens, "lens")),
                                               B, Tseq, C, wdw.shape[1], _stream()), "glu_dwconv_fwd_ragged")


def relpos_softmax_fwd_ragged(ac, bd, lens, probs, B, H, T, scale):
    if min(ac.numel(), bd.numel(), probs.numel()) < B * H * T * T or lens.numel() != B:
        raise ValueError("relpos_softmax_fwd_ragged: shapes do not fit")
    L.check(L.load().a3t_relpos_softmax_fwd_ragged(_ptr(ac), _ptr(bd), _dt(ac), _ptr(_i32(lens, "lens")), _ptr(probs),
                                                   _dt(probs), B, H, T, T * T, T * T, T * T, scale, _stream()),
            "softmax_fwd_ragged")


def _tile_list(what, tiles, B, Tw):
    if tiles is None:
        return None, 0
    if tiles.dim() != 2 or tiles.shape[1] != 4:
        raise ValueError(f"{what}: tiles must be (ntiles, 4), got {tuple(tiles.shape)}")
    if tiles.shape[0] > B * ((Tw + 255) // 256):
        raise ValueError(f"{what}: {tiles.shape[0]} tiles do not fit {B} rows of {Tw} samples")
    _i32(tiles, "tiles")
    if tiles.shape[0] == 0:
        return None, -1
    return _ptr(tiles), tiles.shape[0]


def pwg_block(x, cu, wt0, b0, wt1, b1, g, skips, B, Tw, dil, tiles=None):
    for name, t, C in (("x", x, 64), ("cu", cu, 80), ("g", g, 64), ("skips", skips, 64)):
        if t.dtype != torch.float32 or not t.is_contiguous() or t.numel() != B * Tw * C:
            raise ValueError(f"pwg_block: {name} must be a contiguous fp32 [{B * Tw}][{C}] tensor")
    args = (_ptr(x), _ptr(cu), _ptr(wt0), _ptr(b0), _ptr(wt1), _ptr(b1), _ptr(g), _ptr(skips))
    tp, nt = _tile_list("pwg_block", tiles, B, Tw)
    if tiles is None:
        L.check(L.load().a3t_pwg_block(*args, B, Tw, dil, _stream()), "pwg_block")
    elif nt > 0:
        L.check(L.load().a3t_pwg_block_ragged(*args, tp, nt, B, Tw, dil, _stream()), "pwg_block")


# ... 355 lines not shown
```

include/a3t_hip.h:

```cpp
#ifndef A3T_HIP_H
#define A3T_HIP_H
#include <stdint.h>

#ifdef __cplusplus
extern "C" {
#endif

#define A3T_F32 0
#define A3T_BF16 1
#define A3T_BF16X3 2

#define A3T_EINVAL (-22)

#define A3T_ACT_NONE 0
#define A3T_ACT_RELU 1
#define A3T_ACT_TANH 2
#define A3T_ACT_SWISH 3

#define A3T_ACC_STORE 0
#define A3T_ACC_ADD 1
#define A3T_ACC_ATOMIC 2
#define A3T_ACC_SOLE 3

typedef struct a3t_gemm_desc {
    const void* A;
    const void* B;
    void* C;
    const float* bias;
    const float* R;
    const float* S;
    int32_t M, N, K;
    int64_t a_rs, a_cs;
    int64_t b_rs, b_cs, b_ts;
    int64_t c_rs;
    int32_t batch, batch_inner;
    int64_t a_bs0, a_bs1, b_bs0, b_bs1, c_bs0, c_bs1;
    int32_t taps, pad, dil, Tseq, kshift;
    float alpha;
    int32_t act;
    int32_t accumulate;
    int32_t splitk;
    int32_t a_dtype, b_dtype, c_dtype;
    int32_t compute;
    int32_t s_dtype;
    int32_t colsum_slots;
    float* colsum;
    int64_t colsum_bs1;
    float colsum_scale;
    uint32_t drop_key;
    float drop_p;
    int32_t colsum_ss;
    void* keep_out;
    const void* keep_in;
    int32_t a_signmask;
    int32_t keep_layout;
    const void* A2;
    const void* B2;
    int64_t b2_cs, b2_bs0, b2_bs1;
    float* colsum2;
    int64_t a2_rs;
    int32_t a_unaligned;
} a3t_gemm_desc;

int a3t_gemm(const a3t_gemm_desc* d, void* stream);
int a3t_gemm_plan(const a3t_gemm_desc* d, char* name, int len);
int a3t_gemm_8p_supported(int M, int N, int K, int taps, int flags);
int64_t a3t_gemm_keep_bytes(int M, int N);
int a3t_gemm_pn_supported(int M, int N, int K, int taps, int flags);
int a3t_gemm_tt_supported(int M, int N, int K, int batch);

int a3t_layernorm_fwd(const float* x, const float* gamma, const float* beta, void* y, int y_dtype,
                      float* mean, float* rstd, int M, int D, float eps, void* stream);
int a3t_layernorm_bwd(const void* dy, int dy_dtype, const float* x, const float* gamma, const float* mean,
                      const float* rstd, const float* dres, float* dx, void* dx_bf16, float* dgamma,
                      float* dbeta, float* dx_colsum, float dx_colsum_scale, int M, int D, float drop_p,
                      uint32_t drop_key, void* stream);

int a3t_col_reduce(const void* x, int x_dtype, const float* y, const uint8_t* rowmask, double* out0,
                   double* out1, int M, int C, int64_t ld, int mode, void* stream);
int a3t_f64_to_f32_add(const double* src, float* dst, int n, float scale, void* stream);

int a3t_bn_act_fwd(const float* z, const double* stats, const float* gamma, const float* beta,
                   float* running_mean, float* running_var, float* mean_out, float* rstd_out, void* y,
                   int y_dtype, int M, int C, float eps, float momentum, int training, int act, void* stream);
int a3t_bn_act_bwd_a(const void* dy, int dy_dtype, const float* z, const float* mean, const float* rstd,
                     const float* gamma, const float* beta, double* sums, int M, int C, int act, void* stream);
int a3t_bn_act_bwd_b(const void* dy, int dy_dtype, const float* z, const float* mean, const float* rstd,
                     const float* gamma, const float* beta, const double* sums, float* dz, float* dgamma,
                     float* dbeta, int M, int C, int training, int act, void* stream);

int a3t_glu_dwconv_fwd(const void* g, int g_dtype, const float* wdw, const float* bdw, void* glu,
                       int glu_dtype, float* z, int M, int C, int K, int Tseq, void* stream);
int a3t_glu_dwconv_bwd(const float* dz, const void* g, int g_dtype, const void* glu, int glu_dtype,
                       const float* wdw, void* dg, int dg_dtype, float* dwdw, float* dbdw, float* dg_colsum,
                       int M, int C, int K, int Tseq, void* stream);

int a3t_add_pos_bias(const void* qkv, const float* bias_u, const float* bias_v, void* qu, void* qv, int dtype,
                     int M, int d, void* stream);
int a3t_add_pos_bias_bwd(const void* dqu, const void* dqv, void* dqkv, int dtype, int M, int d, void* stream);
int a3t_relpos_softmax_fwd(const void* ac, const void* bd, int scores_dtype, const uint8_t* keymask, void* probs,
                           int probs_dtype, int B, int H, int T, int64_t ac_bs, int64_t bd_bs, int64_t p_bs,
                           float scale, void* probs_drop, float drop_p, uint32_t drop_key, void* stream);
int a3t_relpos_softmax_bwd(const void* probs, int probs_dtype, const void* dprobs, int dprobs_dtype, void* ds,
                           void* dbd, int out_dtype, int B, int H, int T, int64_t p_bs, int64_t dp_bs, int64_t o_bs,
                           float scale, const void* probs_drop, float drop_p, int64_t dbd_bs_b, int64_t dbd_bs_h,
                           uint32_t drop_key, const float* rowscale, void* stream);

int a3t_attn_fwd(const void* qu, const void* qv, const void* k, const void* v, const void* pos, const uint8_t* keymask,
                 void* ctx, float* lse, int B, int H, int T, int dk, int64_t ldq, int64_t ldkv, int64_t ldp, int64_t ldo,
                 float scale, float drop_p, uint32_t drop_key, const float* bias_u, const float* bias_v, void* stream);

int a3t_attn_fwd_train(const void* qu, const void* qv, const void* k, const void* v, const void* pos,
                       const uint8_t* keymask, void* ctx, float* lse, void* probs, void* probs_drop, float* rowscale,
                       int B, int H, int T, int dk, int64_t ldq, int64_t ldkv, int64_t ldp, int64_t ldo, float scale,
                       float drop_p, uint32_t drop_key, const float* bias_u, const float* bias_v, void* stream);
int a3t_attn_scale_rows(const void* x, const float* rowscale, void* y, int B, int H, int T, int dk, void* stream);
int a3t_attn_bwd_ds(const void* dctx, const void* ctx, const void* v, const void* probs, const float* rowscale, void* ds,
                    void* dbd, int B, int H, int T, int dk, int64_t ldo, int64_t ldkv, int64_t dbd_bsb, int64_t dbd_bsh,
                    float scale, float drop_p, uint32_t drop_key, int signed_probs, int64_t ds_bs, void* stream);

int a3t_mask_fill(const float* speech, const uint8_t* masked, const float* mask_feature, void* out,
                  int out_dtype, int M, int C, void* stream);
int a3t_embed_finish_fwd(const float* e, const float* emb, const float* seg, const int64_t* text,
                         const int64_t* spos, const int64_t* tpos, float* xs, int B, int Tm, int Tp, int D,
                         float xscale, float drop_p, uint32_t drop_key, const float* spk, void* stream);
int a3t_embed_finish_bwd(const float* dxs, const float* e, const int64_t* text, const int64_t* spos,
                         const int64_t* tpos, float* de, float* demb, float* dseg, int B, int Tm, int Tp,
                         int D, int V, int nseg, float xscale, float drop_p, uint32_t drop_key, void* stream);
int a3t_scale(const float* x, float* y, int64_t n, float s, void* stream);
int a3t_axpy(const float* x, float* y, int64_t n, float a, void* stream);
int a3t_attn_bias_fold(const float* slots, int S, int d, float* gu, float* gv, float* gbqkv, void* stream);
int a3t_scale_dev(const float* x, float* y, int64_t n, const float* s, void* stream);
int a3t_slice_rows(const float* x, void* y, int y_dtype, int B, int T, int Tm, int D, int reverse_add,
                   void* stream);
int a3t_concat_rows(const float* speech, const float* text, float* xs, int B, int Tm, int Tp, int D, void* stream);
int a3t_split_rows(const float* dxs, float* dspeech, float* dtext, int B, int Tm, int Tp, int D, void* stream);
int a3t_concat_rows_ragged(const float* speech, const float* text, float* xs, const int32_t* slens, const int32_t* tlens, int B,
                           int Tm, int Tp, int D, int64_t speech_bs, int64_t text_bs, void* stream);
int a3t_cast_bf16(const float* x, void* y, int64_t n, void* stream);
int a3t_cast_bf16_conv_t(const float* src, void* dst, const int64_t* src_off, const int64_t* dst_off, int count, int N,
                         int taps, int C, void* stream);
int a3t_split_bf16(const float* x, void* hi, void* lo, int64_t n, void* stream);

int a3t_reflect_pad(const float* x, float* out, int B, int N, int pad, int ld, void* stream);
int a3t_reflect_pad_ragged(const float* x, float* out, const int32_t* lens, int B, int N, int pad, int ld, void* stream);
int a3t_stft_amp(const float* S, float* amp, int64_t rows, int nbins, int ld, void* stream);
int a3t_logmel_finish(float* mel, const int64_t* olens, int B, int F, int C, void* stream);

int a3t_mlm_loss(const float* before, const float* after, const float* target, const uint8_t* masked,
                 float* loss_out, float* d_before, float* d_after, float* scratch, int M, int C, int l2,
                 float gscale, void* stream);
int a3t_mlm_loss_scratch_floats(int M);

int a3t_sumsq(const float* g, int64_t n, double* partial , void* stream);
int a3t_clip_adam(float* p, const float* g, float* m, float* v, const double* partial, float* norm_out,
                  int64_t n, float lr, float beta1, float beta2, float eps, int step, float clip,
                  float gscale, void* stream);

int a3t_clip_adam_noam(float* p, const float* g, float* m, float* v, const double* partial, float* norm_out, int64_t n,
                       int32_t* state, float base_lr, float model_size, float warmup, float beta1, float beta2,
                       float eps, float clip, float gscale, void* stream);

int a3t_sgd_step(float* p, const float* g, int64_t n, float lr, float gscale, void* stream);

int a3t_pwg_gate(const float* y, const float* c, float* out, int64_t T, int H, void* stream);
int a3t_pwg_res_skip(const float* o, float* x, float* skips, int64_t T, int R, int S, void* stream);
int a3t_pwg_upsample(const float* c, const float* w, float* out, int64_t B, int64_t Tin, int C, int scale,
                     void* stream);
int a3t_replicate_pad(const float* x, float* y, int64_t B, int64_t T, int C, int pad, void* stream);
int a3t_bias_act(float* x, const float* bias, int64_t M, int C, int act, float scale, void* stream);
int a3t_replicate_pad_ragged(const float* x, float* y, const int32_t* lens, int64_t B, int64_t T, int C, int pad,
                             void* stream);
int a3t_pwg_upsample_ragged(const float* c, const float* w, float* out, const int32_t* lens, int mul, int64_t B,
                            int64_t Tin, int C, int scale, void* stream);
int a3t_zero_tail(float* x, const int32_t* lens, int mul, int64_t B, int64_t T, int C, void* stream);
int a3t_layernorm_fwd_ragged(const float* x, const float* gamma, const float* beta, float* y, float* mean, float* rstd,
                             const int32_t* lens, int B, int T, int D, float eps, void* stream);
int a3t_glu_dwconv_fwd_ragged(const float* g, const float* wdw, const float* bdw, float* glu, float* z, const int32_t* lens,
                              int B, int Tseq, int C, int K, void* stream);
int a3t_relpos_softmax_fwd_ragged(const void* ac, const void* bd, int scores_dtype, const int32_t* lens, void* probs,
                                  int probs_dtype, int B, int H, int T, int64_t ac_bs, int64_t bd_bs, int64_t p_bs,
                                  float scale, void* stream);
int a3t_splice_spans(const float* after, const float* speech, const uint8_t* speech_mask, const int32_t* spans, float* out,
                     int32_t* lens, int B, int Tin, int Tout, int C, void* stream);
int a3t_splice_spans_multi(const float* after, const float* speech, const uint8_t* speech_mask, const int32_t* spans,
                           const int32_t* nspans, float* out, int32_t* lens, int B, int Tin, int Tout, int C, int S,
                           void* stream);
int a3t_gather_windows(const float* src, const int32_t* table, float* dst, int R, int T, int Wmax, int C, void* stream);

int a3t_duration_head(const float* z, const float* gamma, const float* beta, const float* w, const float* bias,
                      float* logd, int64_t* frames, int M, int C, float eps, float offset, void* stream);
int a3t_l2_normalize(const float* x, float* y, int B, int n, float eps, void* stream);

int a3t_gst_conv_bn_relu(const float* x, const float* w, const float* scale, const float* shift, float* y,
                         const int32_t* lens, int B, int Tin, int Fin, int Cin, int Cout, int k, int s, void* stream);
int a3t_gst_gru_stl(const float* gi, const float* w_hh, const float* b_hh, const int32_t* lens, const float* w_q,
                    const float* b_q, const float* k_tok, const float* v_tok, const float* w_out, const float* b_out,
                    float* ref_embs, float* style, int B, int T, int H, int d, int heads, int tokens, void* stream);
int a3t_gst_add_style(float* hs, const float* style, const int32_t* rows, int B, int T, int d, int S, void* stream);

int a3t_fs2_variance_embed(float* hs, const float* pitch, const float* energy, const float* wp, const float* bp,
                           const float* we, const float* be, const int32_t* lens, int B, int T, int d, int kp, int ke,
                           void* stream);
int a3t_length_offsets(const int64_t* frames, const int32_t* lens, float alpha, int32_t* offsets, int32_t* frame_lens,
                       int64_t* scaled, int B, int T, void* stream);
int a3t_length_expand(const float* hs, const int32_t* offsets, const int32_t* lens, const int32_t* frame_lens, float* out,
                      int B, int T, int Fp, int d, float scale, void* stream);
int a3t_fs2_finish(const float* before, const float* post, const float* mean, const float* std_, float* after, float* denorm,
                   const int32_t* lens, int B, int F, int C, void* stream);
int a3t_fs2_mvn(const float* x, const float* mean, const float* std_, float* y, int64_t M, int C, void* stream);

int a3t_dropout(const void* x, int x_dtype, void* y, int y_dtype, int64_t n, float p, uint32_t key, float scale,
                void* stream);
int a3t_dropout_bwd_cast(const float* g, void* gm, int gm_dtype, float* colsum, float colsum_scale, int M, int C,
                         float p, uint32_t key, void* stream);

int a3t_pwg_block(float* x, const float* cu, const float* wt0, const float* b0, const float* wt1, const float* b1,
                  float* g, float* skips, int B, int Tw, int dil, void* stream);
int a3t_pwg_block_ragged(float* x, const float* cu, const float* wt0, const float* b0, const float* wt1, const float* b1,
                         float* g, float* skips, const int32_t* tiles, int ntiles, int B, int Tw, int dil, void* stream);
int a3t_pwg_block_f16(const float* x_in, float* x_out, const void* cu16, const void* w0h, const float* b0, const void* w1h,
                      const float* b1, float* skips, const int32_t* tiles, int ntiles, int B, int Tw, int dil, void* stream);
int a3t_cast_f16_sat(const float* src, void* dst, int64_t n, void* stream);

int a3t_hfg_conv(const float* x, const float* wt, const float* bias, const float* R, float* y, float* acc, float alpha,
                 int acc_add, float slope, const int32_t* tiles, int ntiles, int B, int Tw, int C, int taps, int dil,
                 void* stream);
int a3t_hfg_conv_f16(const float* x, const void* wf, const float* bias, const float* R, float* y, float* acc, float alpha,
                     int acc_add, float slope, const int32_t* tiles, int ntiles, int B, int Tw, int C, int taps, int dil,
                     void* stream);
int a3t_hfg_out(const float* x, const float* w, const float* bias, float* y, float slope, const int32_t* tiles, int ntiles,
                int B, int Tw, int C, int K, void* stream);
int a3t_leaky_relu(const float* x, float* y, int64_t n, float slope, void* stream);

int a3t_mgan_stack(const float* x, const float* w, const float* bias, float* y, float slope, const int32_t* tiles, int ntiles,
                   int wmin, int B, int Tw, int C, int dil, void* stream);
int a3t_mgan_out(const float* x, const float* w, const float* bias, float* y, float slope, int act_tanh, const int32_t* tiles,
                 int ntiles, int wmin, int B, int Tw, int C, int O, int K, void* stream);
int a3t_pqmf_synthesis(const float* x, const float* h, float* y, const int32_t* tiles, int ntiles, int B, int Ts, int S,
                       int taps, void* stream);
int a3t_reflect_pad_rows(const float* x, float* y, int64_t B, int64_t T, int C, int pad, void* stream);
int a3t_reflect_pad_rows_ragged(const float* x, float* y, const int32_t* lens, int mul, int64_t B, int64_t T, int C, int pad,
                                void* stream);

int a3t_smg_conv(const float* x, const float* wt, const float* bias, const float* m, const float* stats, const float* R, float* y,
                 int mode, int sigmoid, const int32_t* tiles, int ntiles, int B, int Tw, int Cin, int Cout, int taps, int dil,
                 int up, int ux, int ur, void* stream);
int a3t_smg_stats(const float* x, float* part, float* stats, float eps, const int32_t* tiles, int ntiles, int B, int Tw, int C,
                  void* stream);

int a3t_collate_paint(const int* fs, const int* fe, const int* alen, const uint8_t* sel, const int* mspan, const int* nms,
                      const int* flen, const int* tlen, uint8_t* masked, uint8_t* speech_mask, uint8_t* text_mask,
                      int64_t* sp, int64_t* tp, int B, int Tm, int Tp, int P, int S, int sega_emb, void* stream);
int a3t_segment_colsum(const float* x, float* out, int B, int T, int C, void* stream);

const char* a3t_version(void);
const char* a3t_gemm_last_kernel(void);
int a3t_gemm_8p_mode(int mode);
int a3t_gemm_pn_mode(int mode);
int a3t_gemm_tt_mode(int mode);
int a3t_gemm_tn3_mode(int mode);
int a3t_gemm_tn3_group(const a3t_gemm_desc* d, int n, void* stream);
int a3t_attn_split_mode(int mode);
int a3t_release_workspaces(void);

#ifdef __cplusplus
}
#endif
#endif
```

Baseline: 817,200 mel-frames/s.

## Fuse row-scale and pos-bias prologues into attention backward dV/dK GEMM B-loads

Adds a B-operand prologue variant of the bf16 TT GEMM kernel. In the dV product it multiplies dctx by per-row softmax scales streamed into LDS by a dedicated wave. In the dK product it adds the u positional bias to k on the fly. This removes the separate attn_scale_rows pass and the materialised qu buffer and its writes in attention backward. The cost is extra LDS, per-fragment bf16 unpack/repack ALU work in the GEMM inner loop, and one more rounding of the operand to bf16.

Result: no change. 819,900 mel-frames/s, median of 6 (+0.3%).

```diff
diff --git a/a3t_amd/_lib.py b/a3t_amd/_lib.py
--- a/a3t_amd/_lib.py
+++ b/a3t_amd/_lib.py
@@ -37,10 +37,16 @@
     ]
 
 
+class TTBPrologue(ctypes.Structure):
+    _fields_ = [("k_scale", c_void_p), ("ks_bs0", c_int64), ("ks_bs1", c_int64), ("n_bias", c_void_p), ("nb_bs1", c_int64)]
+
+
 _P = c_void_p
 _SIGS = {
     "a3t_gemm": [POINTER(GemmDesc), _P],
     "a3t_gemm_plan": [POINTER(GemmDesc), c_char_p, c_int],
+    "a3t_gemm_tt_bpro": [POINTER(GemmDesc), POINTER(TTBPrologue), _P],
+    "a3t_gemm_tt_bpro_plan": [POINTER(GemmDesc), POINTER(TTBPrologue), c_char_p, c_int],
     "a3t_layernorm_fwd": [_P, _P, _P, _P, c_int, _P, _P, c_int, c_int, c_float, _P],
     "a3t_layernorm_bwd": [_P, c_int, _P, _P, _P, _P, _P, _P, _P, _P, _P, _P, c_float, c_int, c_int, c_float,
                           ctypes.c_uint32, _P],
diff --git a/a3t_amd/conformer.py b/a3t_amd/conformer.py
--- a/a3t_amd/conformer.py
+++ b/a3t_amd/conformer.py
@@ -100,6 +100,8 @@
         self.fused_attn_train = self.bf16 and opt.fused_attn == "auto" and opt.fused_attn_train != 0
         self.fused_attn_train_min = 1 if opt.fused_attn_train == 2 else 64
         self._fused_now = self._fused_train_now = False
+        self.attn_bpro = os.environ.get("A3T_ATTN_BPRO", "1") != "0"
+        self._bpro_plans = {}
         self.attn_path, self.block_dims = {}, {}
         self._need_grad = training
         self._mode_tag = None
@@ -445,6 +447,21 @@
                  a_bs=(H * T * T, T * T), b_bs=(T * 3 * d, dk), c_bs=(T * d, dk), compute=cmp)
         return None if lens is not None else (probs, pdrop)
 
+    def _bpro_plan(self, B, T, signed):
+        key = (B, T, signed)
+        if key not in self._bpro_plans:
+            c = self.c
+            d, H, dk = c.adim, c.heads, c.dk
+            x = torch.empty(64, dtype=torch.bfloat16)
+            f = torch.empty(16, dtype=torch.float32)
+            kw = dict(batch=B * H, batch_inner=H, a_bs=(H * T * T, T * T), c_bs=(T * 3 * d, dk), compute=self.cmp, colsum=f,
+                      colsum_bs1=dk, colsum_slots=self.colsum_slots, colsum_ss=4 * d)
+            dv = ops.gemm_plan(x, x, x, T, dk, T, 1, T, 1, d, 3 * d, b_bs=(T * d, dk), a_signmask=signed, alpha=2.0 if signed else 1.0,
+                               b_kscale=(f, H * T, T), **kw)
+            dkp = ops.gemm_plan(x, x, x, T, dk, T, 1, T, 1, 3 * d, 3 * d, b_bs=(T * 3 * d, dk), b_nbias=(f, dk), **kw)
+            self._bpro_plans[key] = dv is not None and dkp is not None
+        return self._bpro_plans[key]
+
     def _mha_bwd(self, tag, pre, g, B, T, nb=None, nxt=None):
         p, gr, c = self.store.p, self.store.g, self.c
         d, H, dk = c.adim, c.heads, c.dk
@@ -465,10 +482,12 @@
         dvv = dqkv.view(-1)[2 * d:]
         sdt = torch.bfloat16 if self.bf16 else torch.float32
         rs = self.sv.get(tag + ".rs")
+        signed = bool(self.sv.get(tag + ".signed"))
+        tt = self.bf16 and ops.gemm_tt_supported(T, dk, T, B * H)
+        bpro = tt and self.attn_bpro and rs is not None and qu is None and self._bpro_plan(B, T, signed)
         dctx_v = dctx
-        if rs is not None:
+        if rs is not None and not bpro:
             dctx_v = self._act(self._t("tmp.dctxs"), (M, d))
-        signed = bool(self.sv.get(tag + ".signed"))
         adr = self._drop(c.attention_dropout_rate, tag + ".att") if (pdrop is not None or signed) else None
         regen = self.bf16 and adr is not None and T % 8 == 0 and T <= 2048
         ds_fused = (rs is not None and self.bf16 and self.opt.attn_bwd_ds and (adr is None or regen) and dk % 32 == 0 and dk <= 192
@@ -486,21 +505,21 @@
         csk = dict(colsum_bs1=dk, colsum_slots=S, colsum_ss=4 * d)
         make_q = qu is None
         if make_q:
-            qu = self._act("tmp.qu", (M, d))
+            qu = None if bpro else self._act("tmp.qu", (M, d))
             qv = self._act(self._t("tmp.qv"), (M, d))
 
         def dv_gemm():
-            if rs is not None:
+            if rs is not None and not bpro:
                 ops.attn_scale_rows(dctx, rs, dctx_v, B, H, T)
             ops.gemm(pdrop if pdrop is not None else probs, dctx_v, dvv, T, dk, T, 1, T, 1, d, 3 * d,
                      batch=B * H, batch_inner=H, a_bs=zb, b_bs=(T * d, dk), c_bs=(T * 3 * d, dk),
                      compute=cmp, colsum=sl[3 * d:] if fz else None, a_signmask=signed,
-                     alpha=1.0 / (1.0 - adr[0]) if signed else 1.0, **csk)
+                     alpha=1.0 / (1.0 - adr[0]) if signed else 1.0, b_kscale=(rs, H * T, T) if bpro else None, **csk)
             if make_q:
-                ops.add_pos_bias(qkv, p[pre + ".u"], p[pre + ".v"], qu, qv)
+                ops.add_pos_bias(qkv, None if bpro else p[pre + ".u"], p[pre + ".v"], qu, qv)
         qv_ready = self._side(dv_gemm, want_event=make_q, urgent=True)
         zbd = zb
-        dual = ds_fused and fz and self.opt.attn_dq_dual and ops.gemm_tt_supported(T, dk, T, B * H)
+        dual = ds_fused and fz and self.opt.attn_dq_dual and tt
         dview = ds_fused and fz and self.opt.attn_dbd_view
         if dview:
             bsv = T + T * T
@@ -542,9 +561,14 @@
         else:
             ops.gemm(ds, kk, dqu, T, dk, T, T, 1, 1, 3 * d, ldq, batch=B * H, batch_inner=H, a_bs=zbd,
                      b_bs=(T * 3 * d, dk), c_bs=cbq, compute=cmp, colsum=sl if fz else None, **csk)
-        dk_fn = lambda: ops.gemm(ds, qu, dkk, T, dk, T, 1, T, 1, d, 3 * d, batch=B * H, batch_inner=H,
-                                 a_bs=zbd, b_bs=(T * d, dk), c_bs=(T * 3 * d, dk), compute=cmp,
-                                 colsum=sl[2 * d:] if fz else None, **csk)
+        if bpro:
+            dk_fn = lambda: ops.gemm(ds, qkv, dkk, T, dk, T, 1, T, 1, 3 * d, 3 * d, batch=B * H, batch_inner=H,
+                                     a_bs=zbd, b_bs=(T * 3 * d, dk), c_bs=(T * 3 * d, dk), compute=cmp,
+                                     colsum=sl[2 * d:], b_nbias=(p[pre + ".u"], dk), **csk)
+        else:
+            dk_fn = lambda: ops.gemm(ds, qu, dkk, T, dk, T, 1, T, 1, d, 3 * d, batch=B * H, batch_inner=H,
+                                     a_bs=zbd, b_bs=(T * d, dk), c_bs=(T * 3 * d, dk), compute=cmp,
+                                     colsum=sl[2 * d:] if fz else None, **csk)
         if self.opt.attn_dk_main and dual and self.side is not None and make_q and qv_ready is not None:
             qv_ready.wait_on(torch.cuda.current_stream())
             dk_fn()
diff --git a/a3t_amd/csrc/convmod_attn.hip b/a3t_amd/csrc/convmod_attn.hip
--- a/a3t_amd/csrc/convmod_attn.hip
+++ b/a3t_amd/csrc/convmod_attn.hip
@@ -324,8 +324,8 @@
         int64_t m = i / d;
         int c = (int)(i - m * d);
         float q = ldx(qkv, dt, m * 3 * d + c);
-        stx(qu, dt, i, q + bu[c]);
-        stx(qv, dt, i, q + bv[c]);
+        if (qu) stx(qu, dt, i, q + bu[c]);
+        if (qv) stx(qv, dt, i, q + bv[c]);
     }
 }
 __device__ __forceinline__ void apb_unpack8(const uint4& u, float* f) {
@@ -346,22 +346,27 @@
         const int c = (int)(i - m * d8) * 8;
         float q[8], o[8];
         apb_unpack8(*(const uint4*)(qkv + m * 3 * d8 * 8 + c), q);
-        const float4 u0 = *(const float4*)(bu + c), u1 = *(const float4*)(bu + c + 4);
-        const float4 v0 = *(const float4*)(bv + c), v1 = *(const float4*)(bv + c + 4);
-        const float uu[8] = {u0.x, u0.y, u0.z, u0.w, u1.x, u1.y, u1.z, u1.w};
-        const float vv[8] = {v0.x, v0.y, v0.z, v0.w, v1.x, v1.y, v1.z, v1.w};
-#pragma unroll
-        for (int e = 0; e < 8; ++e) o[e] = q[e] + uu[e];
-        *(uint4*)(qu + i * 8) = apb_pack8(o);
-#pragma unroll
-        for (int e = 0; e < 8; ++e) o[e] = q[e] + vv[e];
-        *(uint4*)(qv + i * 8) = apb_pack8(o);
+        if (qu) {
+            const float4 u0 = *(const float4*)(bu + c), u1 = *(const float4*)(bu + c + 4);
+            const float uu[8] = {u0.x, u0.y, u0.z, u0.w, u1.x, u1.y, u1.z, u1.w};
+#pragma unroll
+            for (int e = 0; e < 8; ++e) o[e] = q[e] + uu[e];
+            *(uint4*)(qu + i * 8) = apb_pack8(o);
+        }
+        if (qv) {
+            const float4 v0 = *(const float4*)(bv + c), v1 = *(const float4*)(bv + c + 4);
+            const float vv[8] = {v0.x, v0.y, v0.z, v0.w, v1.x, v1.y, v1.z, v1.w};
+#pragma unroll
+            for (int e = 0; e < 8; ++e) o[e] = q[e] + vv[e];
+            *(uint4*)(qv + i * 8) = apb_pack8(o);
+        }
     }
 }
 static inline bool apb_al16(const void* p) { return ((uintptr_t)p & 15) == 0; }
 extern "C" int a3t_add_pos_bias(const void* qkv, const float* bias_u, const float* bias_v, void* qu, void* qv,
                                 int dtype, int M, int d, void* stream) {
     int64_t n = (int64_t)M * d;
+    if ((!qu && !qv) || (qu && !bias_u) || (qv && !bias_v)) return A3T_EINVAL;
     if (dtype == A3T_BF16 && d % 8 == 0 && apb_al16(qkv) && apb_al16(qu) && apb_al16(qv) && apb_al16(bias_u) &&
         apb_al16(bias_v)) {
         int64_t n8 = n / 8;
diff --git a/a3t_amd/csrc/gemm.hip b/a3t_amd/csrc/gemm.hip
--- a/a3t_amd/csrc/gemm.hip
+++ b/a3t_amd/csrc/gemm.hip
@@ -837,6 +837,33 @@
     return r;
 }
 
+static int bpro_plan(const a3t_gemm_desc* d, const a3t_tt_bprologue* b, GP* p, GemmPlan* pl) {
+    if (!b || (b->k_scale != nullptr) == (b->n_bias != nullptr) || !al(b->k_scale, 4) || !al(b->n_bias, 4)) return A3T_EINVAL;
+    const int rc = gemm_plan(d, p, pl);
+    if (rc) return rc;
+    if (pl->route != GR_TT || !pl->atn || pl->dual) return A3T_EINVAL;
+    tt_bpro_name(*pl, b->k_scale ? 1 : 2, pl->name, sizeof(pl->name));
+    return 0;
+}
+
+extern "C" int a3t_gemm_tt_bpro(const a3t_gemm_desc* d, const a3t_tt_bprologue* b, void* stream) {
+    GP p;
+    GemmPlan pl;
+    const int rc = bpro_plan(d, b, &p, &pl);
+    if (rc) return rc;
+    const int r = tt_bpro_launch(p, pl, *b, (hipStream_t)stream);
+    a3t_note_kernel(pl.name);
+    return r;
+}
+
+extern "C" int a3t_gemm_tt_bpro_plan(const a3t_gemm_desc* d, const a3t_tt_bprologue* b, char* name, int len) {
+    GP p;
+    GemmPlan pl;
+    const int rc = bpro_plan(d, b, &p, &pl);
+    if (!rc && name && len > 0) snprintf(name, (size_t)len, "%s", pl.name);
+    return rc;
+}
+
 extern "C" int a3t_gemm_plan(const a3t_gemm_desc* d, char* name, int len) {
     GP p;
     GemmPlan pl;
diff --git a/a3t_amd/csrc/gemm_bf16_tt.hip b/a3t_amd/csrc/gemm_bf16_tt.hip
--- a/a3t_amd/csrc/gemm_bf16_tt.hip
+++ b/a3t_amd/csrc/gemm_bf16_tt.hip
@@ -13,6 +13,27 @@
 constexpr int TT_MAX_ROWS = 320, TT_BK = 32, TT_STAGES = 4;
 constexpr int TT_A_BYTES = TT_MAX_ROWS * TT_BK * 2, TT_B_BYTES = 192 * TT_BK * 2, TT_STAGE = TT_A_BYTES + TT_B_BYTES;
 constexpr int TT_LDS = TT_STAGES * TT_STAGE;
+constexpr int TT_SC_STAGE = 256, TT_SC_BYTES = TT_STAGES * TT_SC_STAGE;
+
+struct TTBPro {
+    const float* k_scale;
+    int64_t ks_bs0, ks_bs1;
+    const float* n_bias;
+    int64_t nb_bs1;
+};
+
+template <int BPRO>
+__device__ __forceinline__ bf16x8 tt_bpro_apply(const bf16x8 v, const float* f) {
+    typedef unsigned u32x4 __attribute__((ext_vector_type(4)));
+    const u32x4 u = __builtin_bit_cast(u32x4, v);
+    u32x4 o;
+#pragma unroll
+    for (int e = 0; e < 4; ++e) {
+        const float lo = io_bf2f((unsigned short)(u[e] & 0xffff)), hi = io_bf2f((unsigned short)(u[e] >> 16));
+        o[e] = BPRO == 1 ? io_pack2(lo * f[2 * e], hi * f[2 * e + 1]) : io_pack2(lo + f[0], hi + f[0]);
+    }
+    return __builtin_bit_cast(bf16x8, o);
+}
 }
 
 #ifdef TT_TIMING
@@ -23,8 +44,9 @@
 #define TT_STAMP(k)
 #endif
 
-template <bool ATN, int NJ, bool ASGN = false, bool DUAL = false>
-__global__ __launch_bounds__(512, 2) void gemm_bf16_tt_kernel(GP p, int TR) {
+template <bool ATN, int NJ, bool ASGN, bool DUAL, int BPRO>
+__device__ __forceinline__ void tt_body(const GP& p, const int TR, const TTBPro& bp) {
+    static_assert(BPRO == 0 || (ATN && !DUAL), "the B prologue exists for the [k][m] products (dV, dK)");
     extern __shared__ __attribute__((aligned(16))) unsigned char smem[];
     const int tid = threadIdx.x, lane = tid & 63;
     const int w = __builtin_amdgcn_readfirstlane(tid >> 6);
@@ -37,6 +59,12 @@
     const u16* B = (const u16*)p.B + z0 * p.b_bs0 + z1 * p.b_bs1;
     const int64_t zoff = z0 * p.c_bs0 + z1 * p.c_bs1;
     const int m0 = tm * TR;
+    float nb[NJ];
+#pragma unroll
+    for (int j = 0; j < NJ; ++j) {
+        const int n = wc * (16 * NJ) + j * 16 + (lane & 15);
+        nb[j] = (BPRO == 2 && n < p.N) ? bp.n_bias[z1 * bp.nb_bs1 + n] : 0.f;
+    }
     const int HR = TR >> 1, nbi = HR >> 4;
     const int nkt = (p.K + TT_BK - 1) / TT_BK;
 
@@ -50,6 +78,9 @@
     const unsigned a2_ld = (DUAL && p.a2_rs) ? (unsigned)p.a2_rs * 2u : a_ld;
     const __amdgpu_buffer_rsrc_t rX2 = __builtin_amdgcn_make_buffer_rsrc((void*)X2, 0, (int)(is_a ? (unsigned)(p.M - 1) * a2_ld + (unsigned)p.K * 2u : (unsigned)(p.K - 1) * b2_ld + (unsigned)p.N * 2u), 0x00020000);
     const unsigned lds0 = __builtin_amdgcn_readfirstlane((unsigned)(uintptr_t)LDS_AS(smem));
+    const bool sc_wave = BPRO == 1 && w == 7;
+    const __amdgpu_buffer_rsrc_t rS = __builtin_amdgcn_make_buffer_rsrc(
+        (void*)(BPRO == 1 ? bp.k_scale + z0 * bp.ks_bs0 + z1 * bp.ks_bs1 : (const float*)nullptr), 0, BPRO == 1 ? p.K * 4 : 0, 0x00020000);
 
     unsigned voff[4];
     unsigned voff2[4];
@@ -80,6 +111,9 @@
     const unsigned dst0 = lds0 + (is_a ? (unsigned)(w * 4) * 1024u : (unsigned)TT_A_BYTES + (unsigned)((w - 5) * 4) * 1024u);
     auto issue = [&](const int kt) __attribute__((always_inline)) {
         const unsigned dst = dst0 + (unsigned)(kt & 3) * (unsigned)TT_STAGE;
+        if (sc_wave)
+            dma4(rS, lds0 + (unsigned)TT_LDS + (unsigned)(kt & 3) * (unsigned)TT_SC_STAGE,
+                 (lane < 32 && kt * TT_BK + lane < p.K) ? (unsigned)lane * 4u : OOB, (unsigned)kt * 128u);
         if (DUAL && kt >= nkt) {
             const int k2 = kt - nkt;
             const unsigned so = (unsigned)k2 * kstep2;
@@ -113,6 +147,10 @@
 #pragma unroll
         for (int j = 0; j < NJ; ++j) acc[i][j] = f32x4{0.f, 0.f, 0.f, 0.f};
 
+    if (BPRO == 2) {
+#pragma unroll
+        for (int j = 0; j < NJ; ++j) asm volatile("" : "+v"(nb[j]));
+    }
     issue(0), issue(1), issue(2);
     const int rb0 = wr * nbi;
     const int nkt_all = DUAL ? 2 * nkt : nkt;
@@ -122,7 +160,10 @@
 #pragma unroll
         for (int r = 0; r < 4; ++r) cs1[j][r] = 0.f;
     for (int kt = 0; kt < nkt_all; ++kt) {
-        WAIT_VM(8);
+        if (sc_wave)
+            WAIT_VM(10);
+        else
+            WAIT_VM(8);
         BAR();
 #ifdef TT_TIMING
         if (kt == 0) TT_STAMP(1);
@@ -130,6 +171,12 @@
         issue(kt + 3);
         const unsigned char* sA = smem + (kt & 3) * TT_STAGE;
         const unsigned char* sB = sA + TT_A_BYTES;
+        float sc[8];
+        if (BPRO == 1) {
+            const float4* s4 = (const float4*)(smem + TT_LDS + (kt & 3) * TT_SC_STAGE + g * 32);
+            const float4 s0 = s4[0], s1 = s4[1];
+            sc[0] = s0.x, sc[1] = s0.y, sc[2] = s0.z, sc[3] = s0.w, sc[4] = s1.x, sc[5] = s1.y, sc[6] = s1.z, sc[7] = s1.w;
+        }
         bf16x8 fb[NJ];
 #pragma unroll
         for (int j = 0; j < NJ; ++j) fb[j] = frag_rc(sB, wc * (16 * NJ) + j * 16);
@@ -140,6 +187,17 @@
                 fa[i] = ASGN ? a3t_sign_floor(frag_rc(sA, (rb0 + i) * 16), 0) : frag_rc(sA, (rb0 + i) * 16);
             else
                 fa[i] = *(const bf16x8*)(sA + (rb0 + i) * 1024 + offkc);
+        }
+        if (BPRO == 1) {
+#pragma unroll
+            for (int j = 0; j < NJ; ++j) fb[j] = tt_bpro_apply<1>(fb[j], sc);
+        } else if (BPRO == 2) {
+            const bool kin = kt * TT_BK + g * 8 < p.K;
+#pragma unroll
+            for (int j = 0; j < NJ; ++j) {
+                const float b = kin ? nb[j] : 0.f;
+                fb[j] = tt_bpro_apply<2>(fb[j], &b);
+            }
         }
         SB();
 #pragma unroll
@@ -218,9 +276,24 @@
 }
 
 template <bool ATN, int NJ, bool ASGN = false, bool DUAL = false>
+__global__ __launch_bounds__(512, 2) void gemm_bf16_tt_kernel(GP p, int TR) {
+    tt_body<ATN, NJ, ASGN, DUAL, 0>(p, TR, TTBPro{});
+}
+template <int NJ, bool ASGN, int BPRO>
+__global__ __launch_bounds__(512, 2) void gemm_bf16_tt_bpro_kernel(GP p, int TR, TTBPro bp) {
+    tt_body<true, NJ, ASGN, false, BPRO>(p, TR, bp);
+}
+
+template <bool ATN, int NJ, bool ASGN = false, bool DUAL = false>
 static void launch_tt(const GP& pv, int TR, int grid, hipStream_t stream) {
     (void)hipFuncSetAttribute((const void*)gemm_bf16_tt_kernel<ATN, NJ, ASGN, DUAL>, hipFuncAttributeMaxDynamicSharedMemorySize, TT_LDS);
     hipLaunchKernelGGL((gemm_bf16_tt_kernel<ATN, NJ, ASGN, DUAL>), dim3(grid), dim3(512), TT_LDS, stream, pv, TR);
+}
+template <int NJ, bool ASGN, int BPRO>
+static void launch_tt_bpro(const GP& pv, int TR, int grid, const TTBPro& bp, hipStream_t stream) {
+    constexpr int lds = TT_LDS + (BPRO == 1 ? TT_SC_BYTES : 0);
+    (void)hipFuncSetAttribute((const void*)gemm_bf16_tt_bpro_kernel<NJ, ASGN, BPRO>, hipFuncAttributeMaxDynamicSharedMemorySize, lds);
+    hipLaunchKernelGGL((gemm_bf16_tt_bpro_kernel<NJ, ASGN, BPRO>), dim3(grid), dim3(512), lds, stream, pv, TR, bp);
 }
 
 static bool tt_tiling(int M, int N, int K, int batch, int mode, int& tiles, int& TR) {
@@ -309,3 +382,34 @@
     }
     return (int)hipGetLastError();
 }
+
+void tt_bpro_name(const GemmPlan& pl, int bpro, char* name, size_t len) {
+    snprintf(name, len, "gemm_bf16_tt_bpro_kernel<%d, %s, %d>", pl.nj, tf(pl.asgn), bpro);
+}
+int tt_bpro_launch(const GP& p, const GemmPlan& pl, const a3t_tt_bprologue& b, hipStream_t stream) {
+    if (pl.route != GR_TT || !pl.atn || pl.dual || (b.k_scale != nullptr) == (b.n_bias != nullptr)) return A3T_EINVAL;
+    GP pv = p;
+    pv.ntiles = pl.ntiles;
+    const TTBPro bp = {b.k_scale, b.ks_bs0, b.ks_bs1, b.n_bias, b.nb_bs1};
+    const int TR = pl.TR, grid = (int)pl.grid.x;
+#define TT_BPRO(NJ, ASGN)                                            \
+    do {                                                             \
+        if (b.k_scale)                                               \
+            launch_tt_bpro<NJ, ASGN, 1>(pv, TR, grid, bp, stream);   \
+        else                                                         \
+            launch_tt_bpro<NJ, ASGN, 2>(pv, TR, grid, bp, stream);   \
+    } while (0)
+    if (pl.nj == 3) {
+        if (pl.asgn)
+            TT_BPRO(3, true);
+        else
+            TT_BPRO(3, false);
+    } else {
+        if (pl.asgn)
+            TT_BPRO(2, true);
+        else
+            TT_BPRO(2, false);
+    }
+#undef TT_BPRO
+    return (int)hipGetLastError();
+}
diff --git a/a3t_amd/csrc/gemm_common.h b/a3t_amd/csrc/gemm_common.h
--- a/a3t_amd/csrc/gemm_common.h
+++ b/a3t_amd/csrc/gemm_common.h
@@ -236,3 +236,5 @@
 int g8_tn_launch(const GP& p, const GemmPlan& pl, hipStream_t stream);
 bool tt_plan(const GP& p, int batch, int ly, GemmPlan* pl);
 int tt_launch(const GP& p, const GemmPlan& pl, hipStream_t stream);
+void tt_bpro_name(const GemmPlan& pl, int bpro, char* name, size_t len);
+int tt_bpro_launch(const GP& p, const GemmPlan& pl, const a3t_tt_bprologue& b, hipStream_t stream);
diff --git a/a3t_amd/csrc/mfma_kit.h b/a3t_amd/csrc/mfma_kit.h
--- a/a3t_amd/csrc/mfma_kit.h
+++ b/a3t_amd/csrc/mfma_kit.h
@@ -25,6 +25,10 @@
     asm volatile("s_mov_b32 m0, %0\n\ts_nop 0\n\tbuffer_load_dwordx4 %1, %2, %3 offen lds" ::"s"(lds_addr), "v"(voff), "s"(r), "s"(soff) : "memory");
 }
 
+__device__ __forceinline__ void dma4(const __amdgpu_buffer_rsrc_t& r, unsigned lds_addr, unsigned voff, unsigned soff) {
+    asm volatile("s_mov_b32 m0, %0\n\ts_nop 0\n\tbuffer_load_dword %1, %2, %3 offen lds" ::"s"(lds_addr), "v"(voff), "s"(r), "s"(soff) : "memory");
+}
+
 __device__ __forceinline__ float row16_sum(float v) {
     v += __builtin_bit_cast(float, __builtin_amdgcn_update_dpp(0, __builtin_bit_cast(int, v), 0xB1, 0xf, 0xf, true));
     v += __builtin_bit_cast(float, __builtin_amdgcn_update_dpp(0, __builtin_bit_cast(int, v), 0x4E, 0xf, 0xf, true));
diff --git a/a3t_amd/ops.py b/a3t_amd/ops.py
--- a/a3t_amd/ops.py
+++ b/a3t_amd/ops.py
@@ -71,23 +71,47 @@
     return d
 
 
-def gemm(*args, **kw):
+def _bprologue(b_kscale, b_nbias):
+    if b_kscale is None and b_nbias is None:
+        return None
+    b = L.TTBPrologue()
+    if b_kscale is not None:
+        t, b.ks_bs0, b.ks_bs1 = b_kscale
+        assert t.dtype == torch.float32
+        b.k_scale = t.data_ptr()
+    if b_nbias is not None:
+        t, b.nb_bs1 = b_nbias
+        assert t.dtype == torch.float32
+        b.n_bias = t.data_ptr()
+    return b
+
+
+def gemm(*args, b_kscale=None, b_nbias=None, **kw):
     lib = L.load()
     d = _gemm_desc(*args, **kw)
+    b = _bprologue(b_kscale, b_nbias)
+    if b is None:
+        what, launch = "a3t_gemm", lambda: lib.a3t_gemm(ctypes.byref(d), _stream())
+    else:
+        what, launch = "a3t_gemm_tt_bpro", lambda: lib.a3t_gemm_tt_bpro(ctypes.byref(d), ctypes.byref(b), _stream())
     if PROFILE is not None:
         e0, e1 = torch.cuda.Event(enable_timing=True), torch.cuda.Event(enable_timing=True)
         e0.record()
-        L.check(lib.a3t_gemm(ctypes.byref(d), _stream()), "a3t_gemm")
+        L.check(launch(), what)
         e1.record()
         PROFILE.append((lib.a3t_gemm_last_kernel().decode(), (4.0 if d.A2 else 2.0) * d.M * d.N * d.K * d.batch, e0, e1,
                         (d.M, d.N, d.K, d.batch, d.taps, d.splitk)))
         return
-    L.check(lib.a3t_gemm(ctypes.byref(d), _stream()), "a3t_gemm")
-
-
-def gemm_plan(*args, **kw):
+    L.check(launch(), what)
+
+
+def gemm_plan(*args, b_kscale=None, b_nbias=None, **kw):
     name = ctypes.create_string_buffer(128)
-    rc = L.load().a3t_gemm_plan(ctypes.byref(_gemm_desc(*args, **kw)), name, len(name))
+    b = _bprologue(b_kscale, b_nbias)
+    if b is None:
+        rc = L.load().a3t_gemm_plan(ctypes.byref(_gemm_desc(*args, **kw)), name, len(name))
+    else:
+        rc = L.load().a3t_gemm_tt_bpro_plan(ctypes.byref(_gemm_desc(*args, **kw)), ctypes.byref(b), name, len(name))
     return name.value.decode() if rc == 0 else None
 
 
@@ -296,7 +320,7 @@
 
 
 def add_pos_bias(qkv, u, v, qu, qv):
-    M, d = qu.shape
+    M, d = (qu if qu is not None else qv).shape
     L.check(L.load().a3t_add_pos_bias(_ptr(qkv), _ptr(u), _ptr(v), _ptr(qu), _ptr(qv), _dt(qkv), M, d, _stream()),
             "pos_bias")
 
diff --git a/include/a3t_hip.h b/include/a3t_hip.h
--- a/include/a3t_hip.h
+++ b/include/a3t_hip.h
@@ -69,6 +69,15 @@
 int a3t_gemm_pn_supported(int M, int N, int K, int taps, int flags);
 int a3t_gemm_tt_supported(int M, int N, int K, int batch);
 
+typedef struct a3t_tt_bprologue {
+    const float* k_scale;
+    int64_t ks_bs0, ks_bs1;
+    const float* n_bias;
+    int64_t nb_bs1;
+} a3t_tt_bprologue;
+int a3t_gemm_tt_bpro(const a3t_gemm_desc* d, const a3t_tt_bprologue* b, void* stream);
+int a3t_gemm_tt_bpro_plan(const a3t_gemm_desc* d, const a3t_tt_bprologue* b, char* name, int len);
+
 int a3t_layernorm_fwd(const float* x, const float* gamma, const float* beta, void* y, int y_dtype,
                       float* mean, float* rstd, int M, int D, float eps, void* stream);
 int a3t_layernorm_bwd(const void* dy, int dy_dtype, const float* x, const float* gamma, const float* mean,
```
